# juhotuho10/rust_GPU_raytracing

Hardware: AMD Instinct MI355X
Metric: Mray/s (primary+bounce) at 1920x1080, 8 bounces; 1/2/4/8-GPU scaling (higher is better)
Workload: dtype f32

## Files before the change

rust_gpu_raytracing_amd/csrc/pathtrace.hip:

```cpp
#include <hip/hip_runtime.h>
#include <stdint.h>

#include <algorithm>

#include "rt_launch.h"
#include "rt_path_common.h"
#include "rt_sphere_walk.h"
#include "rt_walk.h"

#ifdef RT_ISA_MARKS
#define RT_ISA_MARK(name) asm volatile("; RT_MARK " name)
#else
#define RT_ISA_MARK(name)
#endif

#pragma clang fp contract(off)

using namespace rtk;

typedef const __attribute__((address_space(4))) unsigned char* KernargPtr;
__device__ __forceinline__ KernargPtr kernarg_fresh(KernargPtr kp) {
    asm volatile("" : "+s"(kp));
    return kp;
}
#define RT_KERNARG(kp, field)                                                                        \
    (*reinterpret_cast<const __attribute__((address_space(4))) decltype(KernelArgs::field)*>(        \
        (kp) + __builtin_offsetof(KernelArgs, field)))
__device__ __forceinline__ ShadeArgs load_shade_args(KernargPtr kp) {
    return ShadeArgs{RT_KERNARG(kp, textures),        RT_KERNARG(kp, env),           RT_KERNARG(kp, texture_width),
                     RT_KERNARG(kp, texture_height),  RT_KERNARG(kp, env_map_width), RT_KERNARG(kp, env_map_height),
                     RT_KERNARG(kp, material_count),  RT_KERNARG(kp, tex_w),         RT_KERNARG(kp, tex_h),
                     RT_KERNARG(kp, tex_layers),      RT_KERNARG(kp, env_w),         RT_KERNARG(kp, env_h),
                     RT_KERNARG(kp, env_uniform),     RT_KERNARG(kp, bounces)};
}

constexpr uint32_t kPrimaryThreads = 1024;


__device__ __forceinline__ uint32_t* sched_orders(const KernelArgs& ka) { return ka.sched + 2u * ka.owned_tiles; }
__device__ __forceinline__ uint32_t* sched_flags(const KernelArgs& ka) { return ka.sched + 4u * ka.owned_tiles; }

__device__ __forceinline__ uint32_t xcc_id() {
    return __builtin_amdgcn_s_getreg((3 << 11) | (0 << 6) | 20);
}

struct TileQueue {
    uint32_t stripe;
    uint32_t empty;
};

__device__ __forceinline__ uint32_t claim_tile(const KernelArgs& ka, TileQueue& q) {
    const uint32_t n_str = ka.queue_stripes;
    const uint32_t lane = threadIdx.x & 63u;
    if (q.empty) return 0xffffffffu;
    uint32_t old = 0;
    if (lane == 0) old = atomicAdd(ka.queue + q.stripe * kQueueStride, 1u);
    uint64_t pos = (uint64_t)__builtin_amdgcn_readlane(old, 0) * n_str + q.stripe;
    if (pos < ka.queue_units) return (uint32_t)pos;
    while (true) {
        bool open = false;
        if (lane < n_str) {
            uint32_t st = q.stripe + 1u + lane;
            st = st >= n_str ? st - n_str : st;
            const uint32_t v = __hip_atomic_load(ka.queue + st * kQueueStride, __ATOMIC_RELAXED, __HIP_MEMORY_SCOPE_AGENT);
            open = (uint64_t)v * n_str + st < ka.queue_units;
        }
        const uint64_t m = __ballot(open);
        if (m == 0) {
            q.empty = 1u;
            return 0xffffffffu;
        }
        uint32_t st = q.stripe + 1u + (uint32_t)__builtin_ctzll(m);
        q.stripe = st >= n_str ? st - n_str : st;
        if (lane == 0) old = atomicAdd(ka.queue + q.stripe * kQueueStride, 1u);
        pos = (uint64_t)__builtin_amdgcn_readlane(old, 0) * n_str + q.stripe;
        if (pos < ka.queue_units) return (uint32_t)pos;
    }
}

template <bool kFramePar>
__device__ __forceinline__ uint32_t unit_tile(const KernelArgs& ka, uint32_t pos, uint32_t& frame) {
    if (pos == 0xffffffffu) return pos;
    uint32_t q;
    if (!kFramePar && !ka.frame_light) {
        frame = 0u;
        q = pos;
    } else if (ka.unit_tile_major) {
        q = pos / ka.frames;
        frame = pos - q * ka.frames;
    } else {
        frame = pos / ka.owned_tiles;
        q = pos - frame * ka.owned_tiles;
    }
    return ka.tile_order ? ka.tile_order[q] : q;
}

__device__ __forceinline__ void record_tile_cost(uint32_t* cost, bool fin, uint32_t tile, uint32_t n) {
    uint64_t m = __ballot(fin);
    while (m) {
        const uint32_t t = __builtin_amdgcn_readlane(tile, (uint32_t)__builtin_ctzll(m));
        const bool mine = fin && tile == t;
        uint32_t v = mine ? n : 0u;
        for (int o = 32; o > 0; o >>= 1) v += __shfl_xor(v, o);
        if ((threadIdx.x & 63u) == 0) atomicAdd(cost + t, v);
        m &= ~__ballot(mine);
    }
}


template <uint32_t kThreads>
__device__ void sort_tiles_by_cost(uint32_t* __restrict__ cost, uint32_t* __restrict__ order, uint32_t n,
                                   uint32_t* scratch) {
    constexpr uint32_t kWaves = kThreads / 64;
    static_assert(kWaves <= 16 && kOrderBuckets * kWaves <= kThreads, "scratch layout / one scan entry per thread");
    uint32_t* slots = scratch;
    uint32_t* max_cost = scratch + kOrderBuckets * 16;
    const uint32_t tid = threadIdx.x, wave = tid >> 6, lane = tid & 63u;
    if (tid == 0) *max_cost = 0;
    __syncthreads();
    uint32_t m = 0;
    for (uint32_t i = tid; i < n; i += kThreads) m = max(m, cost[i]);
    for (int o = 32; o > 0; o >>= 1) m = max(m, (uint32_t)__shfl_xor(m, o));
    if (lane == 0) atomicMax(max_cost, m);
    __syncthreads();
    const uint32_t mx = *max_cost;
    if (mx == 0) {
        for (uint32_t i = tid; i < n; i += kThreads) order[i] = i;
        return;
    }
    const uint64_t mc = (uint64_t)mx + 1u;
    const uint32_t span = ((n + kWaves - 1u) / kWaves + 63u) & ~63u;
    const uint32_t lo = min(n, wave * span), hi = min(n, lo + span);
    auto key = [&](uint32_t i) {
        return i < hi ? kOrderBuckets - 1u - (uint32_t)(((uint64_t)cost[i] * kOrderBuckets) / mc) : kOrderBuckets;
    };
    uint32_t cnt = 0;
    for (uint32_t base = lo; base < hi; base += 64u) {
        const uint32_t k = key(base + lane);
        for (uint32_t b = 0; b < kOrderBuckets; ++b) {
            const uint32_t c = (uint32_t)__popcll(__ballot(k == b));
            if (lane == b) cnt += c;
        }
    }
    if (lane < kOrderBuckets) slots[lane * kWaves + wave] = cnt;
    __syncthreads();
    constexpr uint32_t kEntries = kOrderBuckets * kWaves;
    uint32_t v = tid < kEntries ? slots[tid] : 0u;
    const uint32_t own = v;
    for (uint32_t off = 1; off < kEntries; off <<= 1) {
        __syncthreads();
        const uint32_t add = (tid < kEntries && tid >= off) ? slots[tid - off] : 0u;
        __syncthreads();
        v += add;
        if (tid < kEntries) slots[tid] = v;
    }
    __syncthreads();
    if (tid < kEntries) slots[tid] = v - own;
    __syncthreads();
    uint32_t next = lane < kOrderBuckets ? slots[lane * kWaves + wave] : 0u;
    for (uint32_t base = lo; base < hi; base += 64u) {
        const uint32_t i = base + lane;
        const uint32_t k = key(i);
        uint32_t pos = 0;
        for (uint32_t b = 0; b < kOrderBuckets; ++b) {
            const uint64_t mb = __ballot(k == b);
            const uint32_t first = __builtin_amdgcn_readlane(next, b);
            if (k == b) pos = first + __builtin_amdgcn_mbcnt_hi((uint32_t)(mb >> 32), __builtin_amdgcn_mbcnt_lo((uint32_t)mb, 0u));
            if (lane == b) next += (uint32_t)__popcll(mb);
        }
        if (i < hi) {
            order[pos] = i;
            cost[i] = 0;
        }
    }
}

#ifdef RT_DIAG_TAIL
__device__ __forceinline__ unsigned long long realtime() {
    unsigned long long t;
    asm volatile("s_memrealtime %0\n\ts_waitcnt lgkmcnt(0)" : "=s"(t)::"memory");
    return t;
}
#endif

#ifdef RT_DIAG
__device__ __forceinline__ unsigned long long stamp() {
    unsigned long long t;
    asm volatile("s_memtime %0\n\ts_waitcnt lgkmcnt(0)" : "=s"(t)::"memory");
    return t;
}
struct RootPassCount {
    unsigned long long* diag;
    __device__ __forceinline__ void operator()() const {
        const uint64_t pm = __ballot(true);
        if ((threadIdx.x & 63u) == (uint32_t)__builtin_ctzll(pm)) {
            atomicAdd(diag + 28, 1ull);
            atomicAdd(diag + 29, (unsigned long long)__popcll(pm));
        }
    }
};
struct WalkStepCount {
    unsigned long long* diag;
    __device__ __forceinline__ void operator()(bool walk, bool at_leaf, uint32_t) const {
        const uint64_t act = __ballot(walk), lf = __ballot(at_leaf);
        if (act && (threadIdx.x & 63u) == (uint32_t)__builtin_ctzll(__ballot(true))) {
            atomicAdd(diag + 22, 1ull);
            atomicAdd(diag + 23, (unsigned long long)__popcll(act));
            if (lf) {
                atomicAdd(diag + 24, 1ull);
                atomicAdd(diag + 25, (unsigned long long)__popcll(lf));
            }
        }
    }
};
#endif

template <int kMode, bool kTris>
constexpr bool kLinkedWalk = kBlockLeaves<kTris> && kMode >= 1;

__device__ __forceinline__ uint32_t lds_address(const void* p) {
    return (uint32_t)(uintptr_t)(const __attribute__((address_space(3))) void*)p;
}

template <int kMode, uint32_t kThreads, bool kTris, bool kFramePar>
__global__ void __launch_bounds__(kThreads, 1) rt_pathtrace_kernel(KernelArgs ka) {
    extern __shared__ __attribute__((aligned(16))) unsigned char lds[];
    __shared__ uint32_t block_rays;

    const uint32_t tid = threadIdx.x;
    const KernargPtr kernarg = (KernargPtr)__builtin_amdgcn_kernarg_segment_ptr();
    if (ka.launch_clock && tid == 0) atomicMax(ka.launch_clock, ~(unsigned long long)wall_clock64());
    float* l_srgb = reinterpret_cast<float*>(lds + ka.lds_srgb_offset);
    SceneView sv{ka.sphere_slots, ka.sphere_orig, ka.sphere_material, ka.sphere_bvh, ka.materials, nullptr,
                 ka.objects,      l_srgb,         ka.tri_bvh,     ka.tri_prims, kTris ? *ka.tri_extent : 0.0f,
                 ka.sub_objects};
    if constexpr (kTris && kMode <= 1) {
        if (ka.tri_qnodes) {
            const float4 g0 = ka.tri_qgrid[0], g1 = ka.tri_qgrid[1];
            if (g0.w != 0.0f) {
                sv.tri_q = ka.tri_qnodes;
                sv.qox = g0.x;
                sv.qoy = g0.y;
                sv.qoz = g0.z;
                sv.qsx = g1.x;
                sv.qsy = g1.y;
                sv.qsz = g1.z;
            }
        }
    }
    if (tid == 0) block_rays = 0;
    if constexpr (kMode >= 1) {
        float4* l_sph = reinterpret_cast<float4*>(lds);
        RtMaterial* l_mat = reinterpret_cast<RtMaterial*>(lds + ka.lds_mat_offset);
        RtObject* l_obj = reinterpret_cast<RtObject*>(lds + ka.lds_obj_offset);
        uint32_t* l_orig = reinterpret_cast<uint32_t*>(lds + ka.lds_orig_offset);
        uint32_t* l_smat = reinterpret_cast<uint32_t*>(lds + ka.lds_smat_offset);
        float4* l_nodes = reinterpret_cast<float4*>(lds + ka.lds_nodes_offset);
        for (uint32_t i = tid; i < ka.sphere_slot_count; i += kThreads) {
            l_sph[i] = ka.sphere_slots[i];
            l_orig[i] = ka.sphere_orig[i];
        }
        for (uint32_t i = tid; i < ka.sphere_count; i += kThreads) l_smat[i] = ka.sphere_material[i];
        if constexpr (kLinkedWalk<kMode, kTris>) {
            const uint32_t base = lds_address(l_nodes);
            for (uint32_t i = tid; i < 2u * ka.sphere_nodes; i += kThreads)
                l_nodes[i] = sphere_links_stage(ka.sphere_bvh[i], i, base, ka.sphere_nodes);
            if (tid < 2u) l_nodes[2u * ka.sphere_nodes + tid] = sphere_links_sentinel<float4>(tid, base, ka.sphere_nodes);
        } else {
            for (uint32_t i = tid; i < 2u * ka.sphere_nodes; i += kThreads) l_nodes[i] = ka.sphere_bvh[i];
        }
        float4* l_aux = reinterpret_cast<float4*>(lds + ka.lds_mat_aux_offset);
        for (uint32_t i = tid; i < ka.material_count; i += kThreads) {
            const RtMaterial m = ka.materials[i];
            l_mat[i] = m;
            const float ior_front = 1.0f / m.refraction_index;
            float r0f = (1.0f - ior_front) / (1.0f + ior_front);
            float r0b = (1.0f - m.refraction_index) / (1.0f + m.refraction_index);
            r0f = r0f * r0f;
            r0b = r0b * r0b;
            l_aux[2u * i] = make_float4(ior_front, r0f, r0b, div_const(m.roughness, 10.0f, kInv10));
            const f4 c = decode_texel(ka.textures[min(m.texture_index, ka.tex_layers - 1u)], ka.srgb);
            l_aux[2u * i + 1u] = make_float4(c.x, c.y, c.z, c.w);
        }
        sv.mat_aux = l_aux;
        if (ka.env_uniform & kEnvLineStaged) {
            float4* l_env = reinterpret_cast<float4*>(l_srgb) + kLdsTailBytes / sizeof(float4);
            const uint32_t n = env_line_texels(ka.env_uniform, ka.env_w, ka.env_h);
            const size_t stride = (ka.env_uniform & 2u) ? 1u : ka.env_w;
            for (uint32_t i = tid; i < n; i += kThreads) {
                const f4 c = decode_texel(ka.env[(size_t)i * stride], ka.srgb);
                l_env[i] = make_float4(c.x, c.y, c.z, c.w);
            }
        }
        if constexpr (kTris)
            for (uint32_t i = tid; i < ka.object_count; i += kThreads) l_obj[i] = ka.objects[i];
        sv.sph = l_sph;
        sv.orig = l_orig;
        sv.sph_mat = l_smat;
        sv.nodes = l_nodes;
        sv.mat = l_mat;
        sv.obj = l_obj;
    }
    if constexpr (kMode == 2) {
        float4* l_tn = reinterpret_cast<float4*>(lds + ka.lds_tri_nodes_offset);
        uint4* l_tp = reinterpret_cast<uint4*>(lds + ka.lds_tri_prims_offset);
        for (uint32_t i = tid; i < 2u * ka.tri_nodes; i += kThreads) l_tn[i] = ka.tri_bvh[i];
        for (uint32_t i = tid; i < ka.tri_prim_count; i += kThreads) l_tp[i] = ka.tri_prims[i];
        sv.tri_nodes = l_tn;
        sv.tri_prims = l_tp;
        if (ka.lds_sub_offset) {
            RtSubObject* l_sub = reinterpret_cast<RtSubObject*>(lds + ka.lds_sub_offset);
            for (uint32_t i = tid; i < ka.sub_object_count; i += kThreads) l_sub[i] = ka.sub_objects[i];
            sv.sub = l_sub;
        }
    }
    for (uint32_t i = tid; i < 256u; i += kThreads) l_srgb[i] = ka.srgb[i];
    float* l_cam = l_srgb + 256;
    if (tid < 16u) {
        l_cam[tid] = ka.inv_proj[tid];
        l_cam[16u + tid] = ka.inv_view[tid];
    }
    if (tid == 0) l_cam[32] = ka.aspect;
    __syncthreads();

    const bool accumulate = kFramePar || ka.accumulate == 1u;
    const uint32_t samples = accumulate ? ka.compute_per_frame : 1u;
    constexpr bool kLinked = kLinkedWalk<kMode, kTris>;
    const uint32_t walk_base = kLinked ? lds_address(lds + ka.lds_nodes_offset) : 0u;
    const uint32_t walk_end = kLinked ? sphere_links_addr(walk_base, ka.sphere_nodes) : ka.sphere_nodes;
    const auto walk_over = [&](uint32_t node) { return kLinked ? node == walk_end : node >= walk_end; };

    constexpr uint32_t kIdle = 0, kSetup = 1, kTrav = 2, kDone = 3, kPrimary = 4;
    uint32_t rays = 0;
    uint32_t lane_tile = 0;
    uint32_t lane_slot = 0;
    const bool frame_par = kFramePar || ka.frame_light != nullptr;
    uint32_t mode = kIdle;
    uint32_t index = 0, sample = 0, frame = 0;
    float4 pix = make_float4(0.f, 0.f, 0.f, 0.f);
    Path p;
    p.o = p.d = mk(0.f, 0.f, 0.f);
    p.light = p.contrib = f4{0.f, 0.f, 0.f, 0.f};
    p.seed = p.bounce = 0;
    TraceState ts;
    ts.inv = mk(0.f, 0.f, 0.f);
    ts.a4 = ts.a2 = 0.f;
    ts.node = 0;
    ts.phase = 2;
    ts.nan_hit = false;
    ts.sph = SphereHit{kF32Max, 0u, 0u};
    ts.tri = TriHit{kF32Max, 0u, 0u, 0u, false};

    auto random_index = [&]() { return ka.accumulation_index + (accumulate ? frame : 0u) + sample; };
    auto primary_start = [&]() -> uint32_t {
        return (kTris && ka.primary && p.bounce < ka.bounces) ? kPrimary : kSetup;
    };

    auto store_frame = [&]() {
        float r, g, b, a;
        if (accumulate) {
            const float div = (float)((ka.accumulation_index + frame) * ka.compute_per_frame);
            r = clamp01(pix.x / div);
            g = clamp01(pix.y / div);
            b = clamp01(pix.z / div);
            a = clamp01(pix.w / div);
        } else {
            r = clamp01(p.light.x);
            g = clamp01(p.light.y);
            b = clamp01(p.light.z);
            a = clamp01(p.light.w);
        }
        if (accumulate) ka.accum[index] = pix;
        ka.output[index] = pack_rgba8(r, g, b, a);
    };
    auto finish_sample_frame_par = [&]() {
        const size_t plane = kFramePar ? (size_t)ka.light_plane : (size_t)ka.owned_tiles * 64u;
        const size_t slot = (size_t)(frame * samples + sample) * plane + (size_t)lane_tile * 64u + lane_slot;
        ka.frame_light[slot] = make_float4(p.light.x, p.light.y, p.light.z, p.light.w);
        sample += 1;
        if (sample < samples) {
            start_sample(ka, index, random_index(), pixel_ray(ka, l_cam, index, index % ka.width, index / ka.width), p);
            mode = primary_start();
        } else {
            mode = kIdle;
        }
    };
    auto finish_sample = [&]() {
        if constexpr (kFramePar) {
            finish_sample_frame_par();
        } else {
            if (frame_par) {
                finish_sample_frame_par();
                return;
            }
            sample += 1;
            if (accumulate) {
                pix.x = pix.x + p.light.x;
                pix.y = pix.y + p.light.y;
                pix.z = pix.z + p.light.z;
                pix.w = pix.w + p.light.w;
            }
            if (sample == samples && frame + 1u < ka.frames) {
                store_frame();
                frame += 1;
                sample = 0;
            }
            if (sample < samples) {
                start_sample(ka, index, random_index(), pixel_ray(ka, l_cam, index, index % ka.width, index / ka.width),
                             p);
                mode = primary_start();
            } else {
                store_frame();
                mode = kIdle;
            }
        }
    };

#ifdef RT_DIAG_TAIL
    const unsigned long long wave_t0 = realtime();
    unsigned long long wave_dry = 0;
#endif
    static_assert(kThreads >= kQueueStripesMax, "one thread per stripe counter");
    if (blockIdx.x == 0 && threadIdx.x < kQueueStripesMax) ka.queue_next[threadIdx.x * kQueueStride] = 0u;
    TileQueue queue{(xcc_id() + 8u * (blockIdx.x >> 3)) % ka.queue_stripes, 0u};
    uint32_t tile_frame = 0;
    uint32_t tile = unit_tile<kFramePar>(ka, claim_tile(ka, queue), tile_frame);
    uint32_t next = 0;
#ifdef RT_DIAG
    unsigned long long iters = 0, trav_cyc = 0, steps = 0, step_lanes = 0, shade_cyc = 0, refill_cyc = 0,
                       setup_cyc = 0, leaf_cyc = 0, leaf_steps = 0;
    unsigned long long shade_passes = 0, shade_lanes = 0, miss_lanes = 0, glass_lanes = 0, spec_lanes = 0,
                       setup_passes = 0, setup_lanes = 0;
    const unsigned long long t_start = stamp();
#endif
    while (true) {
#ifdef RT_DIAG
        ++iters;
        const unsigned long long ts0 = stamp();
#endif
        bool fin = false;
        uint32_t fin_rays = 0;
        if (kTris && mode == kPrimary) {
            const uint4 r = ka.primary[(size_t)(frame * samples + sample) * ((size_t)ka.owned_tiles * 64u) +
                                       (size_t)lane_tile * 64u + lane_slot];
            primary_state(PrimaryRecord{__uint_as_float(r.x), r.y, r.z, r.w}, ts);
            mode = kDone;
        }
#ifdef RT_DIAG
        {
            const uint64_t dm = __ballot(mode == kDone);
            if (dm) {
                ++shade_passes;
                shade_lanes += (unsigned long long)__popcll(dm);
            }
        }
#endif
        if (mode == kDone) {
            const Hit h = trace_end<kTris>(sv, ka, p.o, p.d, ts);
#ifdef RT_DIAG
            {
                const bool miss = h.t == kF32Max;
                const RtMaterial dmat = sv.mat[min(h.material_index, ka.material_count - 1u)];
                miss_lanes += (unsigned long long)__popcll(__ballot(miss));
                glass_lanes += (unsigned long long)__popcll(__ballot(!miss && dmat.glass > 0.0f));
                spec_lanes += (unsigned long long)__popcll(__ballot(!miss && !(dmat.glass > 0.0f) && dmat.specular > 0.0f));
            }
#endif
            ++rays;
            RT_ISA_MARK("shade");
            bool ended;
            uint32_t bounce_limit;
            if constexpr (kFramePar) {
                const ShadeArgs sa = load_shade_args(kernarg_fresh(kernarg));
                ended = shade<(kMode >= 1), (kMode >= 1)>(sv, sa, p, h);
                bounce_limit = sa.bounces;
            } else {
                ended = shade<(kMode >= 1), (kMode >= 1)>(sv, ka, p, h);
                bounce_limit = ka.bounces;
            }
            if (ended) {
                fin = true;
                fin_rays = p.bounce + (p.bounce < bounce_limit ? 1u : 0u);
                finish_sample();
            } else {
                mode = kSetup;
            }
        }
        if (ka.tile_cost) record_tile_cost(ka.tile_cost, fin && (!frame_par || frame == 0u), lane_tile, fin_rays);
#ifdef RT_DIAG
        const unsigned long long ts1 = stamp();
        shade_cyc += ts1 - ts0;
#endif
        RT_ISA_MARK("refill");
        while (true) {
            const uint64_t need = __ballot(mode == kIdle);
            if (need == 0 || tile >= ka.owned_tiles) break;
            const uint32_t avail = 64u - next;
            if (mode == kIdle) {
                const uint32_t rank =
                    __builtin_amdgcn_mbcnt_hi((uint32_t)(need >> 32), __builtin_amdgcn_mbcnt_lo((uint32_t)need, 0u));
                if (rank < avail) {
                    const uint32_t slot = next + rank;
                    const uint32_t gt = tile * ka.world_size + ka.rank;
                    const uint32_t x = (gt % ka.tiles_x) * 8u + (slot & 7u);
                    const uint32_t y = (gt / ka.tiles_x) * 8u + (slot >> 3);
                    if (x < ka.width && y < ka.height) {
                        index = y * ka.width + x;
                        lane_tile = tile;
                        lane_slot = slot;
                        sample = 0;
                        frame = tile_frame;
                        mode = kSetup;
                        if (!kFramePar && accumulate && !frame_par) pix = ka.accum[index];
                        start_sample(ka, index, random_index(), pixel_ray(ka, l_cam, index, x, y), p);
                        mode = primary_start();
                    }
                }
            }
            next += min((uint32_t)__popcll(need), avail);
            if (next == 64u) {
                tile = unit_tile<kFramePar>(ka, claim_tile(ka, queue), tile_frame);
                next = 0;
            #ifdef RT_DIAG_TAIL
                if (tile >= ka.owned_tiles && wave_dry == 0) wave_dry = realtime();
#endif
            }
        }
#ifdef RT_DIAG
        const unsigned long long ts2 = stamp();
        refill_cyc += ts2 - ts1;
#endif
#ifdef RT_DIAG
        {
            const uint64_t sm = __ballot(mode == kSetup);
            if (sm) {
                ++setup_passes;
                setup_lanes += (unsigned long long)__popcll(sm);
            }
        }
#endif
        RT_ISA_MARK("setup");
        if (mode == kSetup) {
            if constexpr (!kFramePar)
                while (mode == kSetup && p.bounce >= ka.bounces) finish_sample();
            if (kFramePar || mode == kSetup) {
                trace_begin<kTris>(sv, ka, p.o, p.d, ts);
                if constexpr (kLinkedWalk<kMode, kTris>) ts.node = sphere_links_addr(walk_base, ts.node);
                mode = ts.phase == 2 ? kDone : kTrav;
            }
        }
#ifdef RT_DIAG
        setup_cyc += stamp() - ts2;
#endif
        if (__ballot(mode != kIdle) == 0 && tile >= ka.owned_tiles) break;
        const bool draining = tile >= ka.owned_tiles;
        uint32_t thresh = draining ? 0u : ka.trav_threshold;
        uint32_t n_active = 64u, min_steps = 0u;
        if constexpr (kDrainDecouple<kMode, kTris>) {
            if (draining) {
                thresh = ka.drain_threshold;
                n_active = (uint32_t)__popcll(__ballot(mode == kTrav || mode == kDone));
                min_steps = ka.drain_min_steps;
            }
        }
#ifdef RT_DIAG
        const unsigned long long t0 = stamp();
#endif
        while (true) {
            const uint64_t trav = __ballot(mode == kTrav);
            const uint32_t n_trav = (uint32_t)__popcll(trav);
            if constexpr (kDrainDecouple<kMode, kTris>) {
                if (trav == 0 || (n_trav <= thresh && n_trav < n_active && min_steps == 0)) break;
                min_steps -= min_steps != 0;
            } else {
                if (n_trav <= thresh || trav == 0) break;
            }
#ifdef RT_DIAG
            ++steps;
            step_lanes += (unsigned long long)n_trav;
#endif
            RT_ISA_MARK("traversal");
            bool leaves = false;
            if constexpr (kDeferLeaves<kTris> && !kFusedLeaves<kMode, kTris>) {
                const uint32_t n_pend = (uint32_t)__popcll(__ballot(mode == kTrav && ts.pending != kNoLeaf));
                leaves = 8u * n_pend >= ka.leaf_batch * n_trav;
            }
#ifdef RT_DIAG
            const unsigned long long tl0 = stamp();
#endif
            bool batched = false;
            if constexpr (kCoopLeaves<kMode, kTris>) {
                if (leaves && ka.tri_leaftris) {
                    RT_ISA_MARK("coop_leaf_batch");
                    const bool act = mode == kTrav && ts.pending != kNoLeaf;
                    coop_leaf_batch(sv, ka, p.o, p.d, ts, act, lds);
                    if (act) {
                        phase_end<kTris>(sv, ka, p.o, p.d, ts);
                        if (ts.phase == 2) mode = kDone;
                    }
                    batched = true;
                }
            }
            if constexpr (kBlockLeaves<kTris>) {
                if (mode == kTrav) {
                    RT_ISA_MARK("node_step");
                    RT_ISA_MARK("walk_block");
#ifdef RT_DIAG
                    const WalkStepCount hook{ka.diag};
#else
                    const SphereWalkNoHook hook{};
#endif
                    constexpr int kSteps = kTravUnroll<kMode, kTris>;
                    if constexpr (kLinkedWalk<kMode, kTris>) {
                        if (ka.sphere_boxes_ordered)
                            sphere_links_block<kSteps, true, float4>(lds, walk_end, ts.slab, ts.slack, ts.limit, ts.node,
                                                                     ts.pending, hook);
                        else
                            sphere_links_block<kSteps, false, float4>(lds, walk_end, ts.slab, ts.slack, ts.limit, ts.node,
                                                                      ts.pending, hook);
                    } else {
                        if (ka.sphere_boxes_ordered)
                            sphere_walk_block<kSteps, true>(sv.nodes, ka.sphere_nodes, ts.slab, ts.slack, ts.limit,
                                                            ts.node, ts.pending, hook);
                        else
                            sphere_walk_block<kSteps, false>(sv.nodes, ka.sphere_nodes, ts.slab, ts.slack, ts.limit,
                                                             ts.node, ts.pending, hook);
                    }
                    RT_ISA_MARK("walk_block_end");
                    if (ts.pending == kNoLeaf && walk_over(ts.node)) {
                        ts.phase = 2;
                        mode = kDone;
                    }
                    const uint32_t n_wait = (uint32_t)__popcll(__ballot(ts.pending != kNoLeaf));
                    const uint32_t n_tr = (uint32_t)__popcll(__ballot(true));
#ifdef RT_DIAG
                    if (8u * n_wait >= kBlockLeafShare * n_tr) {
                        const uint64_t gm = __ballot(mode == kTrav && ts.pending != kNoLeaf);
                        if (gm && (threadIdx.x & 63u) == (uint32_t)__builtin_ctzll(gm)) {
                            atomicAdd(ka.diag + 26, 1ull);
                            atomicAdd(ka.diag + 27, (unsigned long long)__popcll(gm));
                        }
                    }
#endif
                    if (8u * n_wait >= kBlockLeafShare * n_tr && mode == kTrav && ts.pending != kNoLeaf) {
                        RT_ISA_MARK("sphere_leaves");
#ifdef RT_DIAG
                        test_sphere_group<false>(sv, ts.pending, p.o, p.d, ts.a4, ts.a2, ts.sph, RootPassCount{ka.diag});
#else
                        test_sphere_group(sv, ts.pending, p.o, p.d, ts.a4, ts.a2, ts.sph);
#endif
                        ts.limit = prune_limit(ts);
                        ts.pending = kNoLeaf;
                        if (walk_over(ts.node)) {
                            ts.phase = 2;
                            mode = kDone;
                        }
                    }
                }
            } else if (!batched && mode == kTrav && (!leaves || ts.pending != kNoLeaf)) {
                if (kDeferLeaves<kTris> && leaves) {
                    RT_ISA_MARK("leaf_batch");
                    leaf_step<kTris, (kMode <= 1)>(sv, ka, p.o, p.d, ts);
                } else {
                    RT_ISA_MARK("node_step");
                    node_step<kTris, kCertWalk<kMode>>(sv, ka, p.o, p.d, ts);
                }
                phase_end<kTris>(sv, ka, p.o, p.d, ts);
                if (ts.phase == 2) mode = kDone;
                if (!(kDeferLeaves<kTris> && leaves)) {
#pragma unroll
                    for (int k = 1; k < kTravUnroll<kMode, kTris>; ++k) {
                        if (mode == kTrav) {
                            node_step<kTris, kCertWalk<kMode>>(sv, ka, p.o, p.d, ts);
                            phase_end<kTris>(sv, ka, p.o, p.d, ts);
                            if (ts.phase == 2) mode = kDone;
                        }
                    }
                }
                if constexpr (kFusedLeaves<kMode, kTris>) {
                    const uint64_t mt = __ballot(mode == kTrav && ts.pending != kNoLeaf && ts.phase == 0);
                    const uint64_t ms = __ballot(mode == kTrav && ts.pending != kNoLeaf && ts.phase != 0);
                    const uint32_t n_p = (uint32_t)__popcll(mt | ms);
                    const uint32_t n_t = (uint32_t)__popcll(__ballot(mode == kTrav));
                    const bool tri_first = __popcll(mt) >= __popcll(ms);
                    if (8u * n_p >= ka.leaf_batch * n_t && mode == kTrav && ts.pending != kNoLeaf &&
                        (ts.phase == 0) == tri_first) {
                        RT_ISA_MARK("leaf_batch");
                        leaf_step<kTris, (kMode <= 1)>(sv, ka, p.o, p.d, ts);
                        phase_end<kTris>(sv, ka, p.o, p.d, ts);
                        if (ts.phase == 2) mode = kDone;
                    }
                }
            }
#ifdef RT_DIAG
            if (leaves) {
                leaf_cyc += stamp() - tl0;
                ++leaf_steps;
            }
#endif
        }
#ifdef RT_DIAG
        trav_cyc += stamp() - t0;
#endif
    }
#ifdef RT_DIAG
    if ((threadIdx.x & 63u) == 0) {
        atomicAdd(ka.diag + 0, stamp() - t_start);
        atomicAdd(ka.diag + 1, trav_cyc);
        atomicAdd(ka.diag + 2, steps);
        atomicAdd(ka.diag + 3, iters);
        atomicAdd(ka.diag + 4, step_lanes);
        atomicAdd(ka.diag + 5, shade_cyc);
        atomicAdd(ka.diag + 6, refill_cyc);
        atomicAdd(ka.diag + 7, setup_cyc);
        atomicAdd(ka.diag + 8, leaf_cyc);
        atomicAdd(ka.diag + 9, leaf_steps);
        atomicAdd(ka.diag + 12, shade_passes);
        atomicAdd(ka.diag + 13, shade_lanes);
        atomicAdd(ka.diag + 14, miss_lanes);
        atomicAdd(ka.diag + 15, glass_lanes);
        atomicAdd(ka.diag + 16, spec_lanes);
        atomicAdd(ka.diag + 17, setup_passes);
        atomicAdd(ka.diag + 18, setup_lanes);
    }
#endif
#ifdef RT_DIAG_TAIL
    if ((threadIdx.x & 63u) == 0) {
        const unsigned long long wave_t1 = realtime();
        atomicAdd(ka.diag + 0, wave_t1);
        atomicMax(ka.diag + 1, wave_t1);
        atomicMax(ka.diag + 2, ~wave_t0);
        atomicAdd(ka.diag + 3, 1ull);
        atomicAdd(ka.diag + 4, wave_t0);
        atomicMax(ka.diag + 5, wave_t0);
        atomicMax(ka.diag + 7, wave_t1 - wave_t0);
        const uint32_t w = blockIdx.x * (kThreads / 64u) + (threadIdx.x >> 6);
        if (w < 65536u) {
            ka.diag[kDiagHeaderWords + 2 * w] = wave_dry ? wave_dry : wave_t1;
            ka.diag[kDiagHeaderWords + 2 * w + 1] = wave_t1;
        }
    }
#endif
    atomicAdd(&block_rays, rays);
    __syncthreads();
    if (tid == 0 && block_rays != 0) atomicAdd(ka.ray_counter, (unsigned long long)block_rays);
    if (ka.sched) {
        const uint32_t par = ka.sched_bits & 1u, n = ka.owned_tiles;
        __shared__ uint32_t sorter;
        if (tid == 0) {
            sorter = atomicAdd(sched_flags(ka) + par, 1u);
            if (blockIdx.x == 0) sched_flags(ka)[par ^ 1u] = 0u;
        }
        __syncthreads();
        if (sorter == 0)
            sort_tiles_by_cost<kThreads>(ka.sched + (par ^ 1u) * n, sched_orders(ka) + (par ^ 1u) * n, n,
                                         reinterpret_cast<uint32_t*>(lds + ka.lds_srgb_offset));
    }
    if (ka.launch_clock) {
        __syncthreads();
        if (tid == 0) atomicMax(ka.launch_clock + 1, (unsigned long long)wall_clock64());
    }
}

#define RT_FOR_EACH_SHAPE(X, FP)                                                                                \
    X(0, 256, true, FP) X(0, 512, true, FP) X(0, 1024, true, FP) X(1, 256, true, FP) X(1, 512, true, FP)       \
    X(1, 1024, true, FP) X(2, 256, true, FP) X(2, 512, true, FP) X(2, 1024, true, FP) X(0, 256, false, FP)     \
    X(0, 512, false, FP) X(0, 1024, false, FP) X(1, 256, false, FP) X(1, 512, false, FP) X(1, 1024, false, FP)
#define RT_FOR_EACH_CONFIG(X) RT_FOR_EACH_SHAPE(X, false) RT_FOR_EACH_SHAPE(X, true)

constexpr uint32_t kBruteThreads = 256;

__device__ __forceinline__ void brute_sub_triangles(const KernelArgs& ka, f3 o, f3 d, uint32_t first_tri,
                                                    uint32_t count, uint32_t oi, float& closest, TriHit& best) {
    for (uint32_t j = 0; j < count; ++j) {
        const uint32_t ti = min(first_tri + j, ka.triangle_count - 1u);
        const TriGeom g = load_tri(ka.triangles, ti);
        const float det = -dot(d, g.cn);
        const float inv_det = 1.0f / det;
        const f3 ao = o - g.a;
        const float dist = dot(ao, g.cn) * inv_det;
        if (dist < 0.0f || dist >= closest) continue;
        const f3 dao = cross(ao, d);
        const float v = -dot(g.ab, dao) * inv_det;
        if (v < 0.0f) continue;
        const float u = dot(g.ac, dao) * inv_det;
        if (u < 0.0f) continue;
        const float w = 1.0f - u - v;
        if (w < 0.0f) continue;
        closest = dist;
        best = TriHit{dist, 0u, ti, oi, det > 0.0f};
    }
}

constexpr uint32_t kBruteGroup = 4;
constexpr uint32_t kBruteWfTileSubs = 512;
constexpr uint32_t kBruteWfLoads = 2u * kBruteWfTileSubs / kBruteThreads;
static_assert(kBruteWfLoads * kBruteThreads == 2u * kBruteWfTileSubs, "tile = whole 16-B loads per thread");
static_assert(kBruteWfLoads == 4u, "the sweep's tile loads are written out for 4 per thread");
constexpr uint32_t kBruteRays = 1;
constexpr uint32_t kBruteChunk = kBruteRays * kBruteThreads;
constexpr uint32_t kBruteHits = 8;
static_assert(kBruteHits >= kBruteGroup, "a group's hits fit a drained list");
constexpr int kBruteWaves = 4, kBruteStreamWaves = 8;

struct BruteSlot {
    uint32_t s, index, x, y;
    bool valid;
};
__device__ __forceinline__ BruteSlot brute_slot(const KernelArgs& ka, const uint32_t* q_in, uint32_t level,
                                                uint32_t qi, uint32_t n_in) {
    BruteSlot r;
    const bool have = qi < n_in;
    r.s = have ? (level == 0u ? qi : q_in[qi]) : 0u;
    const uint32_t local_tile = r.s >> 6, lane_slot = r.s & 63u;
    const uint32_t gt = local_tile * ka.world_size + ka.rank;
    r.x = (gt % ka.tiles_x) * 8u + (lane_slot & 7u);
    r.y = (gt / ka.tiles_x) * 8u + (lane_slot >> 3);
    r.valid = have && local_tile < ka.owned_tiles && r.x < ka.width && r.y < ka.height;
    r.index = r.valid ? r.y * ka.width + r.x : 0u;
    return r;
}

__device__ __forceinline__ void brute_load_path(const float4* pl, uint32_t n_slots, uint32_t s, Path& p) {
    const float4 a = pl[s], b = pl[n_slots + s], l = pl[2u * n_slots + s], k = pl[3u * n_slots + s];
    p.o = mk(a.x, a.y, a.z);
    p.seed = __float_as_uint(a.w);
    p.d = mk(b.x, b.y, b.z);
    p.bounce = __float_as_uint(b.w);
    p.light = f4{l.x, l.y, l.z, l.w};
    p.contrib = f4{k.x, k.y, k.z, k.w};
}
__device__ __forceinline__ void brute_store_path(float4* pl, uint32_t n_slots, uint32_t s, const Path& p) {
    pl[s] = make_float4(p.o.x, p.o.y, p.o.z, __uint_as_float(p.seed));
    pl[n_slots + s] = make_float4(p.d.x, p.d.y, p.d.z, __uint_as_float(p.bounce));
    pl[2u * n_slots + s] = make_float4(p.light.x, p.light.y, p.light.z, p.light.w);
    pl[3u * n_slots + s] = make_float4(p.contrib.x, p.contrib.y, p.contrib.z, p.contrib.w);
}

template <bool kTris, bool kStream>
__global__ void __launch_bounds__(kBruteThreads, kStream ? kBruteStreamWaves : kBruteWaves)
    rt_brute_wf_kernel(KernelArgs ka) {
    extern __shared__ __attribute__((aligned(16))) unsigned char lds[];
    __shared__ uint32_t block_rays;
    const uint32_t tid = threadIdx.x;
    if (ka.launch_clock && tid == 0) atomicMax(ka.launch_clock, ~(unsigned long long)wall_clock64());
    const uint32_t n_slots = ka.owned_tiles * 64u;
    const uint32_t level = ka.brute_level;
    uint32_t* counts = ka.brute_counts + (size_t)ka.brute_pass * ka.brute_levels;
    const uint32_t n_in = level == 0u ? n_slots : counts[level];
    if (blockIdx.x * kBruteChunk >= n_in) {
        if (ka.launch_clock && tid == 0) atomicMax(ka.launch_clock + 1, (unsigned long long)wall_clock64());
        return;
    }
    float* l_cam;
    const SceneView sv = brute_stage<kTris, kBruteThreads>(ka, lds, tid, l_cam);
    uint4* l_tile = reinterpret_cast<uint4*>(lds + ka.lds_stack_offset);
    uint16_t* l_hits = reinterpret_cast<uint16_t*>(l_tile + 4u * kBruteWfTileSubs);
    if (tid == 0) block_rays = 0;
    __syncthreads();

    const bool accumulate = ka.accumulate == 1u;
    const uint32_t samples = accumulate ? ka.compute_per_frame : 1u;
    const uint32_t frame = ka.brute_pass / samples, sample = ka.brute_pass % samples;
    const bool last_pass = ka.brute_pass + 1u == ka.frames * samples;
    const uint32_t random_index = ka.accumulation_index + (accumulate ? frame : 0u) + sample;
    const uint32_t* q_in = ka.brute_queue + (size_t)(level & 1u) * n_slots;
    uint32_t* q_out = ka.brute_queue + (size_t)((level + 1u) & 1u) * n_slots;
    float4* pl = ka.brute_paths;
    uint32_t rays = 0;
    uint64_t streamed = 0;
    uint32_t chunks = 0;
    for (uint32_t c = blockIdx.x; c * kBruteChunk < n_in; c += gridDim.x) {
        ++chunks;
        f3 o[kBruteRays], d[kBruteRays], inv[kBruteRays];
        bool alive[kBruteRays];
        SphereHit sph[kBruteRays];
        TriHit tri[kBruteRays];
        float closest[kBruteRays];
#pragma unroll
        for (uint32_t k = 0; k < kBruteRays; ++k) {
            const BruteSlot bs = brute_slot(ka, q_in, level, c * kBruteChunk + k * kBruteThreads + tid, n_in);
            Path p;
            if (level == 0u) {
                if (bs.valid) {
                    start_sample(ka, bs.index, random_index, pixel_ray(ka, l_cam, bs.index, bs.x, bs.y), p);
                    brute_store_path(pl, n_slots, bs.s, p);
                }
            } else if (bs.valid) {
                brute_load_path(pl, n_slots, bs.s, p);
            }
            alive[k] = bs.valid && p.bounce < ka.bounces;
            o[k] = alive[k] ? p.o : mk(0.f, 0.f, 0.f);
            d[k] = alive[k] ? p.d : mk(0.f, 0.f, 1.f);
            inv[k] = mk(1.0f / d[k].x, 1.0f / d[k].y, 1.0f / d[k].z);
            sph[k] = SphereHit{kF32Max, 0u, 0u};
            tri[k] = TriHit{kF32Max, 0u, 0u, 0u, false};
            closest[k] = kF32Max;
            if (alive[k]) {
                const float a = dot(d[k], d[k]);
                for (uint32_t i = 0; i < ka.sphere_slot_count; i += 4u)
                    test_sphere_group<true>(sv, i, o[k], d[k], 4.0f * a, 2.0f * a, sph[k]);
            }
        }
        if constexpr (kTris && kStream) {
            static_assert(kBruteRays == 1, "the streamed sweep carries one ray per thread");
            uint32_t* l_hits32 = reinterpret_cast<uint32_t*>(l_tile);
            typedef float rt_v4 __attribute__((ext_vector_type(4)));
            typedef __attribute__((address_space(4))) const rt_v4 rt_cf4;
            auto ldc = [](rt_cf4* p_, uint32_t i_) {
                const rt_v4 v_ = p_[i_];
                return make_float4(v_.x, v_.y, v_.z, v_.w);
            };
            for (uint32_t oi = 0; oi < ka.object_count; ++oi) {
                const RtObject& ob = sv.obj[oi];
                const bool in_obj = alive[0] && ray_in_bounds(o[0], inv[0], ob.min_bounds, ob.max_bounds);
                if (__ballot(in_obj) == 0ull) continue;
                const uint32_t first = ob.first_sub_object_index, n_sub = ob.sub_object_count;
                const uint32_t last_sub = ka.sub_object_count - 1u;
                rt_cf4* recs = (rt_cf4*)(const void*)ka.sub_objects;
                if ((tid & 63u) == 0u) streamed += n_sub;
                uint32_t cnt = 0u;
                auto drain = [&]() {
                    for (uint32_t e = 0; __builtin_amdgcn_ballot_w64(e < cnt) != 0ull; ++e) {
                        if (e < cnt) {
                            const uint32_t si = l_hits32[e * kBruteThreads + tid];
                            const float4 lo = reinterpret_cast<const float4*>(ka.sub_objects)[2u * si];
                            const float4 hi = reinterpret_cast<const float4*>(ka.sub_objects)[2u * si + 1u];
                            brute_sub_triangles(ka, o[0], d[0], __float_as_uint(lo.w), __float_as_uint(hi.w), oi,
                                                closest[0], tri[0]);
                        }
                    }
                    cnt = 0u;
                };
                float4 l0, l1, l2, l3, h0, h1, h2, h3;
#define RT_BRUTE_SLOAD(j_)                                                                              \
    {                                                                                                   \
        const uint32_t s0_ = 2u * min(first + (j_), last_sub), s1_ = 2u * min(first + (j_) + 1u, last_sub); \
        const uint32_t s2_ = 2u * min(first + (j_) + 2u, last_sub), s3_ = 2u * min(first + (j_) + 3u, last_sub); \
        n0 = ldc(recs, s0_); m0 = ldc(recs, s0_ + 1u); n1 = ldc(recs, s1_); m1 = ldc(recs, s1_ + 1u);   \
        n2 = ldc(recs, s2_); m2 = ldc(recs, s2_ + 1u); n3 = ldc(recs, s3_); m3 = ldc(recs, s3_ + 1u);   \
    }
                {
                    float4 n0, n1, n2, n3, m0, m1, m2, m3;
                    RT_BRUTE_SLOAD(0u)
                    l0 = n0; l1 = n1; l2 = n2; l3 = n3; h0 = m0; h1 = m1; h2 = m2; h3 = m3;
                }
                uint32_t j0 = 0;
                for (; j0 + 4u <= n_sub; j0 += 4u) {
                    RT_ISA_MARK("brute_box");
                    float4 n0, n1, n2, n3, m0, m1, m2, m3;
                    RT_BRUTE_SLOAD(j0 + 4u)
                    uint32_t bits = 0u;
                    if (in_obj) {
                        bits |= ray_in_box4(o[0], inv[0], l0, h0) ? 1u : 0u;
                        bits |= ray_in_box4(o[0], inv[0], l1, h1) ? 2u : 0u;
                        bits |= ray_in_box4(o[0], inv[0], l2, h2) ? 4u : 0u;
                        bits |= ray_in_box4(o[0], inv[0], l3, h3) ? 8u : 0u;
                    }
                    if (__ballot(bits != 0u) != 0ull) {
                        while (bits) {
                            const uint32_t j = __builtin_ctz(bits);
                            bits &= bits - 1u;
                            l_hits32[cnt * kBruteThreads + tid] = first + j0 + j;
                            cnt += 1u;
                        }
                        if (__ballot(cnt + 4u > kBruteHits) != 0ull) drain();
                    }
                    l0 = n0; l1 = n1; l2 = n2; l3 = n3; h0 = m0; h1 = m1; h2 = m2; h3 = m3;
                }
#undef RT_BRUTE_SLOAD
                for (; j0 < n_sub; ++j0) {
                    const uint32_t si = min(first + j0, last_sub);
                    const float4 lo = ldc(recs, 2u * si), hi = ldc(recs, 2u * si + 1u);
                    if (in_obj && ray_in_box4(o[0], inv[0], lo, hi)) {
                        l_hits32[cnt * kBruteThreads + tid] = si;
                        cnt += 1u;
                    }
                    if (__ballot(cnt + 1u > kBruteHits) != 0ull) drain();
                }
                drain();
            }
        } else if constexpr (kTris) {
            for (uint32_t oi = 0; oi < ka.object_count; ++oi) {
                const RtObject& ob = sv.obj[oi];
                bool in_obj[kBruteRays];
                bool any_in = false;
#pragma unroll
                for (uint32_t k = 0; k < kBruteRays; ++k) {
                    in_obj[k] = alive[k] && ray_in_bounds(o[k], inv[k], ob.min_bounds, ob.max_bounds);
                    any_in |= in_obj[k];
                }
                if (!__syncthreads_or(any_in)) continue;
                const uint32_t first = ob.first_sub_object_index, n_sub = ob.sub_object_count;
                const uint32_t n_tiles = (n_sub + kBruteWfTileSubs - 1u) / kBruteWfTileSubs;
                const uint4* src = reinterpret_cast<const uint4*>(ka.sub_objects);
                const uint32_t last_sub = ka.sub_object_count - 1u;
                uint4 r0, r1, r2, r3;
#define RT_BRUTE_LOAD1(k_, rk)                                                                          \
    {                                                                                                   \
        const uint32_t q_ = tid + (k_) * kBruteThreads;                                                 \
        rk = src[2u * min(first + base_ + (min(q_, 2u * nt_ - 1u) >> 1), last_sub) + (q_ & 1u)];       \
    }
#define RT_BRUTE_LOAD_TILE(t)                                                                           \
    {                                                                                                   \
        const uint32_t base_ = (t) * kBruteWfTileSubs, nt_ = min(kBruteWfTileSubs, n_sub - base_);     \
        RT_BRUTE_LOAD1(0u, r0) RT_BRUTE_LOAD1(1u, r1) RT_BRUTE_LOAD1(2u, r2) RT_BRUTE_LOAD1(3u, r3)     \
    }
#define RT_BRUTE_STORE1(k_, rk)                                                                         \
    {                                                                                                   \
        const uint32_t q_ = tid + (k_) * kBruteThreads;                                                 \
        if (q_ < 2u * nt_) dst_[q_] = rk;                                                               \
    }
#define RT_BRUTE_STORE_TILE(t)                                                                          \
    {                                                                                                   \
        uint4* dst_ = l_tile + (size_t)((t) & 1u) * 2u * kBruteWfTileSubs;                             \
        const uint32_t nt_ = min(kBruteWfTileSubs, n_sub - (t) * kBruteWfTileSubs);                     \
        RT_BRUTE_STORE1(0u, r0) RT_BRUTE_STORE1(1u, r1) RT_BRUTE_STORE1(2u, r2) RT_BRUTE_STORE1(3u, r3) \
    }
                if (n_tiles) {
                    RT_BRUTE_LOAD_TILE(0u)
                    RT_BRUTE_STORE_TILE(0u)
                }
                for (uint32_t t = 0; t < n_tiles; ++t) {
                    __syncthreads();
                    const uint32_t nt = min(kBruteWfTileSubs, n_sub - t * kBruteWfTileSubs);
                    if (tid == 0) streamed += nt;
                    const bool more = t + 1u < n_tiles;
                    if (more) RT_BRUTE_LOAD_TILE(t + 1u)
                    if (any_in) {
                        const float4* tile = reinterpret_cast<const float4*>(l_tile + (size_t)(t & 1u) * 2u * kBruteWfTileSubs);
                        uint32_t cnt[kBruteRays];
#pragma unroll
                        for (uint32_t k = 0; k < kBruteRays; ++k) cnt[k] = 0u;
                        auto drain = [&]() {
#pragma unroll
                            for (uint32_t k = 0; k < kBruteRays; ++k) {
                                for (uint32_t e = 0; __builtin_amdgcn_ballot_w64(e < cnt[k]) != 0ull; ++e) {
                                    if (e < cnt[k]) {
                                        const uint32_t j = l_hits[(k * kBruteHits + e) * kBruteThreads + tid];
                                        const float4 lo = tile[2u * j], hi = tile[2u * j + 1u];
                                        brute_sub_triangles(ka, o[k], d[k], __float_as_uint(lo.w), __float_as_uint(hi.w),
                                                            oi, closest[k], tri[k]);
                                    }
                                }
                                cnt[k] = 0u;
                            }
                        };
                        uint32_t j0 = 0;
                        for (; j0 + kBruteGroup <= nt; j0 += kBruteGroup) {
                            RT_ISA_MARK("brute_box");
                            uint32_t bits[kBruteRays];
                            uint32_t any = 0u;
#pragma unroll
                            for (uint32_t k = 0; k < kBruteRays; ++k) bits[k] = 0u;
#pragma unroll
                            for (uint32_t j = 0; j < kBruteGroup; ++j) {
                                const float4 lo = tile[2u * (j0 + j)], hi = tile[2u * (j0 + j) + 1u];
#pragma unroll
                                for (uint32_t k = 0; k < kBruteRays; ++k)
                                    bits[k] |= (in_obj[k] & ray_in_box4(o[k], inv[k], lo, hi)) ? 1u << j : 0u;
                            }
#pragma unroll
                            for (uint32_t k = 0; k < kBruteRays; ++k) any |= bits[k];
                            if (any) {
                                bool full = false;
#pragma unroll
                                for (uint32_t k = 0; k < kBruteRays; ++k) {
                                    while (bits[k]) {
                                        const uint32_t j = __builtin_ctz(bits[k]);
                                        bits[k] &= bits[k] - 1u;
                                        l_hits[(k * kBruteHits + cnt[k]) * kBruteThreads + tid] = (uint16_t)(j0 + j);
                                        cnt[k] += 1u;
                                    }
                                    full |= cnt[k] + kBruteGroup > kBruteHits;
                                }
                                if (__builtin_amdgcn_ballot_w64(full) != 0ull) drain();
                            }
                        }
                        for (; j0 < nt; ++j0) {
                            const float4 lo = tile[2u * j0], hi = tile[2u * j0 + 1u];
#pragma unroll
                            for (uint32_t k = 0; k < kBruteRays; ++k) {
                                if (in_obj[k] && ray_in_box4(o[k], inv[k], lo, hi)) {
                                    l_hits[(k * kBruteHits + cnt[k]) * kBruteThreads + tid] = (uint16_t)j0;
                                    cnt[k] += 1u;
                                }
                            }
                            bool full = false;
#pragma unroll
                            for (uint32_t k = 0; k < kBruteRays; ++k) full |= cnt[k] + 1u > kBruteHits;
                            if (__builtin_amdgcn_ballot_w64(full) != 0ull) drain();
                        }
                        drain();
                    }
                    if (more) RT_BRUTE_STORE_TILE(t + 1u)
                }
#undef RT_BRUTE_LOAD1
#undef RT_BRUTE_LOAD_TILE
#undef RT_BRUTE_STORE1
#undef RT_BRUTE_STORE_TILE
            }
        }
#pragma unroll
        for (uint32_t k = 0; k < kBruteRays; ++k) {
            const BruteSlot bs = brute_slot(ka, q_in, level, c * kBruteChunk + k * kBruteThreads + tid, n_in);
            Path p;
            if (bs.valid) brute_load_path(pl, n_slots, bs.s, p);
            bool done = bs.valid && !alive[k];
            if (alive[k]) {
                ++rays;
                TraceState ts;
                ts.sph = sph[k];
                ts.tri = tri[k];
                const Hit h = trace_end<kTris>(sv, ka, o[k], d[k], ts);
                done = shade<true>(sv, ka, p, h);
            }
            const bool cont = alive[k] && !done;
            if (cont) brute_store_path(pl, n_slots, bs.s, p);
            const uint64_t m = __ballot(cont);
            if (m) {
                const uint32_t lane = __builtin_amdgcn_mbcnt_hi((uint32_t)(m >> 32), __builtin_amdgcn_mbcnt_lo((uint32_t)m, 0u));
                uint32_t base = 0u;
                if ((tid & 63u) == (uint32_t)__builtin_ctzll(m)) base = atomicAdd(counts + level + 1u, (uint32_t)__popcll(m));
                base = __builtin_amdgcn_readlane(base, (uint32_t)__builtin_ctzll(m));
                if (cont) q_out[base + lane] = bs.s;
            }
            if (done) {
                float r, g, b, al;
                if (accumulate) {
                    float4 pix = ka.accum[bs.index];
                    pix.x = pix.x + p.light.x;
                    pix.y = pix.y + p.light.y;
                    pix.z = pix.z + p.light.z;
                    pix.w = pix.w + p.light.w;
                    ka.accum[bs.index] = pix;
                    const float div = (float)((ka.accumulation_index + ka.frames - 1u) * ka.compute_per_frame);
                    r = clamp01(pix.x / div);
                    g = clamp01(pix.y / div);
                    b = clamp01(pix.z / div);
                    al = clamp01(pix.w / div);
                } else {
                    r = clamp01(p.light.x);
                    g = clamp01(p.light.y);
                    b = clamp01(p.light.z);
                    al = clamp01(p.light.w);
                }
                if (last_pass) ka.output[bs.index] = pack_rgba8(r, g, b, al);
            }
        }
    }
    atomicAdd(&block_rays, rays);
    __syncthreads();
    if (tid == 0 && block_rays) atomicAdd(ka.ray_counter, (unsigned long long)block_rays);
    if (tid == 0 && ka.stream_bytes && kTris && chunks) {
        uint64_t n_sub = 0;
        for (uint32_t oi = 0; oi < ka.object_count; ++oi) n_sub += sv.obj[oi].sub_object_count;
        atomicAdd(ka.stream_bytes, (unsigned long long)(chunks * n_sub * 32ull));
    }
    if (streamed && ka.l2_stream_bytes) atomicAdd(ka.l2_stream_bytes, (unsigned long long)streamed * 32ull);
    if (ka.launch_clock) {
        __syncthreads();
        if (tid == 0) atomicMax(ka.launch_clock + 1, (unsigned long long)wall_clock64());
    }
}

template <int kMode, bool kTris, uint32_t kThreads, uint32_t kMinWaves>
__global__ void __launch_bounds__(kThreads, kMinWaves) rt_primary_kernel(KernelArgs ka) {
    extern __shared__ __attribute__((aligned(16))) unsigned char lds[];
    const uint32_t tid = threadIdx.x;
    if (ka.launch_clock && tid == 0) atomicMax(ka.launch_clock, ~(unsigned long long)wall_clock64());
    float* l_srgb = reinterpret_cast<float*>(lds + ka.lds_srgb_offset);
    float* l_cam = l_srgb + 256;
    SceneView sv{ka.sphere_slots, ka.sphere_orig, ka.sphere_material, ka.sphere_bvh, ka.materials, nullptr,
                 ka.objects,      l_srgb,         ka.tri_bvh,     ka.tri_prims, kTris ? *ka.tri_extent : 0.0f,
                 ka.sub_objects};
    if constexpr (kMode >= 1) {
        float4* l_sph = reinterpret_cast<float4*>(lds);
        RtObject* l_obj = reinterpret_cast<RtObject*>(lds + ka.lds_obj_offset);
        uint32_t* l_orig = reinterpret_cast<uint32_t*>(lds + ka.lds_orig_offset);
        float4* l_nodes = reinterpret_cast<float4*>(lds + ka.lds_nodes_offset);
        for (uint32_t i = tid; i < ka.sphere_slot_count; i += kThreads) {
            l_sph[i] = ka.sphere_slots[i];
            l_orig[i] = ka.sphere_orig[i];
        }
        for (uint32_t i = tid; i < 2u * ka.sphere_nodes; i += kThreads) l_nodes[i] = ka.sphere_bvh[i];
        if constexpr (kTris)
            for (uint32_t i = tid; i < ka.object_count; i += kThreads) l_obj[i] = ka.objects[i];
        sv.sph = l_sph;
        sv.orig = l_orig;
        sv.nodes = l_nodes;
        sv.obj = l_obj;
    }
    if constexpr (kMode == 2) {
        float4* l_tn = reinterpret_cast<float4*>(lds + ka.lds_tri_nodes_offset);
        uint4* l_tp = reinterpret_cast<uint4*>(lds + ka.lds_tri_prims_offset);
        for (uint32_t i = tid; i < 2u * ka.tri_nodes; i += kThreads) l_tn[i] = ka.tri_bvh[i];
        for (uint32_t i = tid; i < ka.tri_prim_count; i += kThreads) l_tp[i] = ka.tri_prims[i];
        sv.tri_nodes = l_tn;
        sv.tri_prims = l_tp;
        if (ka.lds_sub_offset) {
            RtSubObject* l_sub = reinterpret_cast<RtSubObject*>(lds + ka.lds_sub_offset);
            for (uint32_t i = tid; i < ka.sub_object_count; i += kThreads) l_sub[i] = ka.sub_objects[i];
            sv.sub = l_sub;
        }
    }
    if (tid < 16u) {
        l_cam[tid] = ka.inv_proj[tid];
        l_cam[16u + tid] = ka.inv_view[tid];
    }
    if (tid == 0) l_cam[32] = ka.aspect;
    __syncthreads();

    const uint32_t unit = __builtin_amdgcn_readfirstlane(blockIdx.x * (kThreads / 64u) + (tid >> 6));
    if (unit >= ka.queue_units) return;
    const uint32_t n_frames = ka.queue_units / ka.owned_tiles;
    const uint32_t frame = ka.primary_tile_major ? unit % n_frames : unit / ka.owned_tiles;
    const uint32_t local_tile = ka.primary_tile_major ? unit / n_frames : unit - frame * ka.owned_tiles;
    const uint32_t slot = tid & 63u;
    const uint32_t gt = local_tile * ka.world_size + ka.rank;
    const uint32_t x = (gt % ka.tiles_x) * 8u + (slot & 7u);
    const uint32_t y = (gt / ka.tiles_x) * 8u + (slot >> 3);
    const bool valid = x < ka.width && y < ka.height;
    const uint32_t index = valid ? y * ka.width + x : 0u;
    const bool accumulate = ka.accumulate == 1u;
    const uint32_t samples = accumulate ? ka.compute_per_frame : 1u;
    const size_t owned_px = (size_t)ka.owned_tiles * 64u;
    const f3 cam = pixel_ray(ka, l_cam, index, x, y);
    for (uint32_t sample = 0; sample < samples; ++sample) {
        Path p;
        start_sample(ka, index, ka.accumulation_index + (accumulate ? frame : 0u) + sample, cam, p);
        const f3 o = p.o, d = p.d;
        TraceState ts;
        trace_begin<kTris>(sv, ka, o, d, ts);
        if constexpr (kTris) {
            if (ts.phase == 0) {
                uint32_t node = __builtin_amdgcn_readfirstlane(ts.node);
                while (node < ka.tri_nodes) {
                    const float4 lo = sv.tri_nodes[2u * node], hi = sv.tri_nodes[2u * node + 1u];
                    float near_t, far_t;
                    slab_hit(ts.slab, lo.x, lo.y, lo.z, hi.x, hi.y, hi.z, near_t, far_t);
                    bool hit = valid && near_t <= far_t && far_t >= 0.0f && near_t <= ts.limit;
                    const uint32_t leaf = __float_as_uint(hi.w);
                    uint32_t skip = 0u;
                    if (kCertWalk<kMode> && hit && leaf != 0xffffffffu && ka.tri_leafcert && near_t > ts.tri.t &&
                        ts.tri.t != kF32Max) {
                        skip = tri_leaf_skips(ka, leaf & 0xffffffu, ts.slab, o, d, ts.tri.t, lo, hi);
                        if (skip == kLeafCertAll) hit = false;
                    }
                    const bool any = __ballot(hit) != 0;
                    if (any && leaf != 0xffffffffu && hit) {
                        tri_leaf<(kMode <= 1)>(sv, ka, o, d, ts, leaf & 0xffffffu);
                        ts.limit = tri_limit(sv, ka, o, ts);
                    }
                    node = (any && leaf == 0xffffffffu) ? node + 1u : __float_as_uint(lo.w);
                }
                if (ts.nan_hit) ts.tri = sweep_triangles(sv, ka, o, d);
                ts.phase = ka.sphere_nodes != 0 ? 1u : 2u;
                ts.node = 0;
                if (ts.phase == 1) phase_setup<kTris>(sv, ka, o, ts.a2 * 0.5f, 1, ts);
            }
        }
        if (ts.phase == 1) {
            const uint32_t n0 = ka.sphere_octant_stride ? ka.sphere_octant_stride : ka.sphere_nodes;
            SlabRay sr = slab_ray(o.x, o.y, o.z, ts.inv.x, ts.inv.y, ts.inv.z, 0.0f);
            {
                const float r = sqrt_up(dot(o, o));
                float m, slack;
                sphere_cull_bounds(r, ka.sphere_extent, ka.sphere_rmin, ka.sphere_rmax,
                                   __builtin_amdgcn_rsqf(ts.a2 * 0.5f), m, slack);
                sr = slab_ray(o.x, o.y, o.z, ts.inv.x, ts.inv.y, ts.inv.z, m);
                ts.slack = slack;
                ts.limit = prune_limit(ts);
            }
            uint32_t node = 0;
            while (node < n0) {
                const float4 lo = sv.nodes[2u * node], hi = sv.nodes[2u * node + 1u];
                float near_t, far_t;
                slab_hit(sr, lo.x, lo.y, lo.z, hi.x, hi.y, hi.z, near_t, far_t);
                const bool hit = valid && near_t <= far_t && far_t >= -ts.slack && near_t <= ts.limit;
                const bool any = __ballot(hit) != 0;
                const uint32_t leaf = __float_as_uint(hi.w);
                if (any && leaf != 0xffffffffu && hit) {
                    test_sphere_group(sv, leaf & 0xffffffu, o, d, ts.a4, ts.a2, ts.sph);
                    ts.limit = prune_limit(ts);
                }
                node = (any && leaf == 0xffffffffu) ? node + 1u : __float_as_uint(lo.w);
            }
        }
        if (valid)
            reinterpret_cast<uint4*>(ka.primary)[(size_t)(frame * samples + sample) * owned_px +
                                                 (size_t)local_tile * 64u + slot] = [&] {
                const PrimaryRecord r = primary_record<kTris>(ts);
                return make_uint4(__float_as_uint(r.t), r.id, r.meta, r.orig);
            }();
    }
}

namespace {
hipError_t allow_big_lds(const void* fn) {
    int dev = 0, max_optin = 0;
    hipError_t e = hipGetDevice(&dev);
    if (e != hipSuccess) return e;
    e = hipDeviceGetAttribute(&max_optin, hipDeviceAttributeSharedMemPerBlockOptin, dev);
    if (e != hipSuccess || max_optin <= 0) return hipSuccess;
    return hipFuncSetAttribute(fn, hipFuncAttributeMaxDynamicSharedMemorySize, max_optin - 256);
}
}

hipError_t rt_launch_pathtrace(const KernelArgs& ka, int mode, bool tris, bool frame_par, uint32_t threads,
                               size_t lds_bytes, uint32_t blocks, hipStream_t stream) {
    if (frame_par && (!ka.frame_light || ka.accumulate != 1u || ka.bounces == 0)) return hipErrorInvalidValue;
#define RT_LAUNCH(M, T, TR, FP)                                                                                \
    if (mode == M && threads == T && tris == TR && frame_par == FP) {                                         \
        hipLaunchKernelGGL((rt_pathtrace_kernel<M, T, TR, FP>), dim3(blocks), dim3(T), lds_bytes, stream, ka); \
        return hipGetLastError();                                                                             \
    }
    RT_FOR_EACH_CONFIG(RT_LAUNCH)
#undef RT_LAUNCH
    return hipErrorInvalidValue;
}

size_t rt_brute_wf_tile_bytes(bool stream) {
    if (stream) return (size_t)kBruteThreads * kBruteHits * 4u;
    return 2u * (size_t)kBruteWfTileSubs * sizeof(RtSubObject) + (size_t)kBruteThreads * kBruteRays * kBruteHits * 2u;
}

uint32_t rt_brute_wf_chunk() { return kBruteChunk; }

hipError_t rt_launch_brute_wf(const KernelArgs& ka, bool tris, bool scalar_stream, size_t lds_bytes, uint32_t blocks,
                              hipStream_t stream) {
    if (blocks == 0) return hipSuccess;
    const void* fn = tris ? (scalar_stream ? reinterpret_cast<const void*>(&rt_brute_wf_kernel<true, true>)
                                           : reinterpret_cast<const void*>(&rt_brute_wf_kernel<true, false>))
                          : reinterpret_cast<const void*>(&rt_brute_wf_kernel<false, false>);
    if (lds_bytes > 64u * 1024u) {
        hipError_t e = hipFuncSetAttribute(fn, hipFuncAttributeMaxDynamicSharedMemorySize, (int)lds_bytes);
        if (e != hipSuccess) return hipErrorInvalidConfiguration;
    }
    if (tris && scalar_stream)
        hipLaunchKernelGGL((rt_brute_wf_kernel<true, true>), dim3(blocks), dim3(kBruteThreads), lds_bytes, stream, ka);
    else if (tris)
        hipLaunchKernelGGL((rt_brute_wf_kernel<true, false>), dim3(blocks), dim3(kBruteThreads), lds_bytes, stream, ka);
    else
        hipLaunchKernelGGL((rt_brute_wf_kernel<false, false>), dim3(blocks), dim3(kBruteThreads), lds_bytes, stream, ka);
    return hipGetLastError();
}

hipError_t rt_launch_primary(const KernelArgs& ka, int mode, bool tris, size_t lds_bytes, uint32_t threads,
                             uint32_t min_waves, hipStream_t stream) {
    if (threads == 0) threads = kPrimaryThreads;
    const uint32_t per = threads / 64u;
    const uint32_t blocks = (ka.queue_units + per - 1u) / per;
    if (blocks == 0) return hipSuccess;
#define RT_PRIMARY(M, TR, T, W)                                                                                \
    if (mode == M && tris == TR && threads == T && min_waves == W) {                                           \
        if (lds_bytes > 64u * 1024u) {                                                                         \
            hipError_t e = allow_big_lds(reinterpret_cast<const void*>(&rt_primary_kernel<M, TR, T, W>));     \
            if (e != hipSuccess) return e;                                                                     \
        }                                                                                                      \
        hipLaunchKernelGGL((rt_primary_kernel<M, TR, T, W>), dim3(blocks), dim3(T), lds_bytes, stream, ka);   \
        return hipGetLastError();                                                                              \
    }
    RT_PRIMARY(1, true, 64, 0) RT_PRIMARY(1, true, 128, 0) RT_PRIMARY(1, true, 256, 0) RT_PRIMARY(1, true, 256, 8)
    RT_PRIMARY(1, true, 512, 0) RT_PRIMARY(1, true, 1024, 0) RT_PRIMARY(2, true, 1024, 0)
#undef RT_PRIMARY
    return hipErrorInvalidValue;
}

constexpr int kDefaultWavesPerCu = 16;

hipError_t rt_pathtrace_pick_config(int mode, bool tris, bool frame_par, size_t lds_bytes,
                                    size_t lds_bytes_per_thread, uint32_t force_threads, uint32_t waves_cap,
                                    uint32_t* threads, int* blocks_per_cu) {
    const int kTargetWavesPerCu = waves_cap ? (int)waves_cap : kDefaultWavesPerCu;
    int best_waves = -1;
#define RT_OCC(M, T, TR, FP)                                                                              \
    if (mode == M && tris == TR && frame_par == FP) {                                                     \
        int n = 0;                                                                                        \
        hipError_t e = allow_big_lds(reinterpret_cast<const void*>(&rt_pathtrace_kernel<M, T, TR, FP>)); \
        if (e != hipSuccess) return e;                                                                    \
        e = hipOccupancyMaxActiveBlocksPerMultiprocessor(&n, rt_pathtrace_kernel<M, T, TR, FP>, T,       \
                                                         lds_bytes + (size_t)T * lds_bytes_per_thread);  \
        if (e != hipSuccess) return e;                                                                    \
        const int waves = std::min(n * (int)(T / 64), kTargetWavesPerCu);                                 \
        if (n > 0 && (force_threads ? force_threads == T : waves > best_waves)) {                         \
            best_waves = waves;                                                                           \
            *threads = T;                                                                                 \
            *blocks_per_cu = force_threads ? n : std::max(1, std::min(n, kTargetWavesPerCu / (int)(T / 64))); \
        }                                                                                                 \
    }
    RT_FOR_EACH_CONFIG(RT_OCC)
#undef RT_OCC
    if (best_waves <= 0) return hipErrorInvalidConfiguration;
    return hipSuccess;
}

extern "C" __global__ void __launch_bounds__(256) rt_pack_tiles_kernel(const float4* __restrict__ accum,
                                                                      float4* __restrict__ dst, uint32_t width,
                                                                      uint32_t height, uint32_t tiles_x,
                                                                      uint32_t owned_tiles, uint32_t rank,
                                                                      uint32_t world) {
    const uint64_t gid = (uint64_t)blockIdx.x * blockDim.x + threadIdx.x;
    const uint64_t local_tile = gid >> 6;
    if (local_tile >= owned_tiles) return;
    const uint32_t lane = (uint32_t)(gid & 63u);
    const uint32_t tile = (uint32_t)local_tile * world + rank;
    const uint32_t x = (tile % tiles_x) * 8u + (lane & 7u);
    const uint32_t y = (tile / tiles_x) * 8u + (lane >> 3);
    float4 v = make_float4(0.f, 0.f, 0.f, 0.f);
    if (x < width && y < height) v = accum[(size_t)y * width + x];
    dst[gid] = v;
}

__device__ __forceinline__ uint32_t owned_tiles_of(uint32_t n_tiles, uint32_t rank, uint32_t world) {
    return rank < n_tiles ? (n_tiles - rank + world - 1u) / world : 0u;
}

extern "C" __global__ void __launch_bounds__(256) rt_unpack_tiles_kernel(
    const float4* __restrict__ src, float4* __restrict__ accum, uint32_t* __restrict__ output, uint32_t width,
    uint32_t height, uint32_t tiles_x, uint32_t n_tiles, uint32_t first_rank, uint32_t world, uint64_t stride_px,
    uint32_t skip_rank, float divisor) {
    const uint32_t rank = first_rank + blockIdx.y;
    if (rank == skip_rank) return;
    src += (uint64_t)blockIdx.y * stride_px;
    const uint64_t gid = (uint64_t)blockIdx.x * blockDim.x + threadIdx.x;
    const uint64_t local_tile = gid >> 6;
    if (local_tile >= owned_tiles_of(n_tiles, rank, world)) return;
    const uint32_t lane = (uint32_t)(gid & 63u);
    const uint32_t tile = (uint32_t)local_tile * world + rank;
    const uint32_t x = (tile % tiles_x) * 8u + (lane & 7u);
    const uint32_t y = (tile / tiles_x) * 8u + (lane >> 3);
    if (x >= width || y >= height) return;
    const float4 v = src[gid];
    const size_t idx = (size_t)y * width + x;
    accum[idx] = v;
    output[idx] = pack_rgba8(clamp01(v.x / divisor), clamp01(v.y / divisor), clamp01(v.z / divisor),
                             clamp01(v.w / divisor));
}

typedef float StreamF4 __attribute__((ext_vector_type(4)));
__device__ __forceinline__ float4 ld_stream(const float4* p) {
    const StreamF4 v = __builtin_nontemporal_load(reinterpret_cast<const StreamF4*>(p));
    return make_float4(v.x, v.y, v.z, v.w);
}

__device__ __forceinline__ void resolve_pixel(float4* __restrict__ accum, uint32_t* __restrict__ output,
                                              const float4* __restrict__ light, uint32_t width, uint32_t height,
                                              uint32_t tiles_x, uint32_t owned_tiles, uint32_t rank, uint32_t world,
                                              uint32_t k0, uint32_t samples, uint32_t frames) {
    const uint64_t gid = (uint64_t)blockIdx.x * blockDim.x + threadIdx.x;
    const uint64_t owned_px = (uint64_t)owned_tiles * 64u;
    if (gid >= owned_px) return;
    const uint32_t lane = (uint32_t)(gid & 63u);
    const uint32_t tile = (uint32_t)(gid >> 6) * world + rank;
    const uint32_t x = (tile % tiles_x) * 8u + (lane & 7u);
    const uint32_t y = (tile / tiles_x) * 8u + (lane >> 3);
    if (x >= width || y >= height) return;
    const size_t idx = (size_t)y * width + x;
    float4 pix = accum[idx];
    const uint32_t n = frames * samples;
    constexpr uint32_t kGroup = 8;
    const float4* src = light + gid;
    uint32_t i = 0;
    for (; i + kGroup <= n; i += kGroup) {
        float4 l[kGroup];
#pragma unroll
        for (uint32_t k = 0; k < kGroup; k++) l[k] = ld_stream(src + (size_t)(i + k) * owned_px);
#pragma unroll
        for (uint32_t k = 0; k < kGroup; k++) {
            pix.x = pix.x + l[k].x;
            pix.y = pix.y + l[k].y;
            pix.z = pix.z + l[k].z;
            pix.w = pix.w + l[k].w;
        }
    }
    for (; i < n; i++) {
        const float4 l = ld_stream(src + (size_t)i * owned_px);
        pix.x = pix.x + l.x;
        pix.y = pix.y + l.y;
        pix.z = pix.z + l.z;
        pix.w = pix.w + l.w;
    }
    accum[idx] = pix;
    const float div = (float)((k0 + frames - 1u) * samples);
    output[idx] = pack_rgba8(clamp01(pix.x / div), clamp01(pix.y / div), clamp01(pix.z / div), clamp01(pix.w / div));
}

extern "C" __global__ void __launch_bounds__(256) rt_resolve_frames_kernel(
    float4* __restrict__ accum, uint32_t* __restrict__ output, const float4* __restrict__ light, uint32_t width,
    uint32_t height, uint32_t tiles_x, uint32_t owned_tiles, uint32_t rank, uint32_t world, uint32_t k0,
    uint32_t samples, uint32_t frames, unsigned long long* __restrict__ clock) {
    constexpr uint32_t kResolveStampBlocks = 64;
    const bool first = blockIdx.x < kResolveStampBlocks;
    const bool last = blockIdx.x + kResolveStampBlocks >= gridDim.x;
    if (clock && first && threadIdx.x == 0) atomicMax(clock, ~(unsigned long long)wall_clock64());
    resolve_pixel(accum, output, light, width, height, tiles_x, owned_tiles, rank, world, k0, samples, frames);
    if (clock && last) {
        __syncthreads();
        if (threadIdx.x == 0) atomicMax(clock + 1, (unsigned long long)wall_clock64());
    }
}

hipError_t rt_launch_resolve(float4* accum, uint32_t* output, const float4* light, uint32_t width, uint32_t height,
                             uint32_t tiles_x, uint32_t owned_tiles, uint32_t rank, uint32_t world, uint32_t k0,
                             uint32_t samples, uint32_t frames, unsigned long long* clock, hipStream_t stream) {
    const uint64_t threads = (uint64_t)owned_tiles * 64u;
    const uint32_t blocks = (uint32_t)((threads + 255u) / 256u);
    hipLaunchKernelGGL(rt_resolve_frames_kernel, dim3(blocks), dim3(256), 0, stream, accum, output, light, width,
                       height, tiles_x, owned_tiles, rank, world, k0, samples, frames, clock);
    return hipGetLastError();
}

extern "C" __global__ void __launch_bounds__(256) rt_pack_output_kernel(
    const uint32_t* __restrict__ output, uint32_t* __restrict__ dst, uint32_t width, uint32_t height,
    uint32_t tiles_x, uint32_t n_tiles, uint32_t first_rank, uint32_t world, uint64_t stride_px, uint32_t skip_rank,
    uint32_t unpack) {
    const uint32_t rank = first_rank + blockIdx.y;
    if (rank == skip_rank) return;
    dst += (uint64_t)blockIdx.y * stride_px;
    const uint64_t gid = (uint64_t)blockIdx.x * blockDim.x + threadIdx.x;
    const uint64_t local_tile = gid >> 6;
    if (local_tile >= owned_tiles_of(n_tiles, rank, world)) return;
    const uint32_t lane = (uint32_t)(gid & 63u);
    const uint32_t tile = (uint32_t)local_tile * world + rank;
    const uint32_t x = (tile % tiles_x) * 8u + (lane & 7u);
    const uint32_t y = (tile / tiles_x) * 8u + (lane >> 3);
    const bool inside = x < width && y < height;
    const size_t idx = (size_t)y * width + x;
    uint32_t* out = const_cast<uint32_t*>(output);
    if (unpack) {
        if (inside) out[idx] = dst[gid];
    } else {
        dst[gid] = inside ? output[idx] : 0u;
    }
}

static uint32_t owned_tiles_host(uint32_t n_tiles, uint32_t rank, uint32_t world) {
    return rank < n_tiles ? (n_tiles - rank + world - 1u) / world : 0u;
}

hipError_t rt_launch_pack_output(uint32_t* output, uint32_t* packed, uint32_t width, uint32_t height, uint32_t tiles_x,
                                 uint32_t n_tiles, uint32_t first_rank, uint32_t ranks, uint32_t world,
                                 uint64_t stride_px, uint32_t skip_rank, bool unpack, hipStream_t stream) {
    const uint64_t threads = (uint64_t)owned_tiles_host(n_tiles, first_rank, world) * 64u;
    const uint32_t blocks = (uint32_t)((threads + 255u) / 256u);
    if (blocks == 0 || ranks == 0) return hipSuccess;
    hipLaunchKernelGGL(rt_pack_output_kernel, dim3(blocks, ranks), dim3(256), 0, stream, output, packed, width, height,
                       tiles_x, n_tiles, first_rank, world, stride_px, skip_rank, unpack ? 1u : 0u);
    return hipGetLastError();
}

hipError_t rt_launch_pack(const float4* accum, float4* dst, uint32_t width, uint32_t height, uint32_t tiles_x,
                          uint32_t owned_tiles, uint32_t rank, uint32_t world, hipStream_t stream) {
    const uint64_t threads = (uint64_t)owned_tiles * 64u;
    const uint32_t blocks = (uint32_t)((threads + 255u) / 256u);
    hipLaunchKernelGGL(rt_pack_tiles_kernel, dim3(blocks), dim3(256), 0, stream, accum, dst, width, height, tiles_x,
                       owned_tiles, rank, world);
    return hipGetLastError();
}

hipError_t rt_launch_unpack(const float4* src, float4* accum, uint32_t* output, uint32_t width, uint32_t height,
                            uint32_t tiles_x, uint32_t n_tiles, uint32_t first_rank, uint32_t ranks, uint32_t world,
                            uint64_t stride_px, uint32_t skip_rank, float divisor, hipStream_t stream) {
    const uint64_t threads = (uint64_t)owned_tiles_host(n_tiles, first_rank, world) * 64u;
    const uint32_t blocks = (uint32_t)((threads + 255u) / 256u);
    if (blocks == 0 || ranks == 0) return hipSuccess;
    hipLaunchKernelGGL(rt_unpack_tiles_kernel, dim3(blocks, ranks), dim3(256), 0, stream, src, accum, output, width,
                       height, tiles_x, n_tiles, first_rank, world, stride_px, skip_rank, divisor);
    return hipGetLastError();
}

extern "C" __global__ void __launch_bounds__(256) rt_math_selftest_kernel(uint32_t which,
                                                                         unsigned long long* mismatches,
                                                                         uint32_t* first_bad) {
    unsigned long long bad = 0;
    const uint64_t stride = (uint64_t)gridDim.x * blockDim.x;
    for (uint64_t i = (uint64_t)blockIdx.x * blockDim.x + threadIdx.x; i < (1ull << 32); i += stride) {
        const uint32_t bits = (uint32_t)i;
        const float x = __uint_as_float(bits);
        float got, want;
        if (which == 0) {
            const float ax = __builtin_fabsf(x);
            if (ax != 0.0f && ax < 0x1p-96f) continue;
            got = sqrt_rn_nrm(x);
            want = __builtin_sqrtf(x);
        } else if (which == 1) {
            got = div_const(x, kTwoPiWgsl, kInvTwoPiWgsl);
            want = x / kTwoPiWgsl;
        } else if (which == 2) {
            got = div_const(x, kWgslPi, kInvWgslPi);
            want = x / kWgslPi;
        } else if (which == 3) {
            got = div_const(x, 255.0f, kInv255);
            want = x / 255.0f;
        } else if (which == 4) {
            got = div_const(x, 10.0f, kInv10);
            want = x / 10.0f;
        } else {
            const float u = (float)bits / 4294967296.0f;
            if (which == 5) {
                got = logf_u01(u);
                want = logf_c(u);
            } else {
                const float theta = kBoxMullerTwoPi * u;
                got = cosf_box(theta);
                want = cosf_c(theta);
            }
        }
        const bool same = __float_as_uint(got) == __float_as_uint(want) || (got != got && want != want);
        if (!same) {
            ++bad;
            atomicMin(first_bad, bits);
        }
    }
    if (bad) atomicAdd(mismatches, bad);
}

hipError_t rt_launch_math_selftest(uint32_t which, unsigned long long* mismatches, uint32_t* first_bad,
                                   hipStream_t stream) {
    hipLaunchKernelGGL(rt_math_selftest_kernel, dim3(8192), dim3(256), 0, stream, which, mismatches, first_bad);
    return hipGetLastError();
}
```

rust_gpu_raytracing_amd/csrc/rt_frames.cpp:

```cpp
#include <algorithm>

#include "rt_ctx.h"
#include "rt_launch.h"

namespace {

constexpr size_t kLdsSceneBudget = 64 * 1024;
constexpr size_t kLdsAccelBudget = 150 * 1024;
constexpr float kTriPruneRho = 1.0f / 64.0f;
uint32_t trav_threshold_for(int lds_mode, bool tris, bool certified) {
    if (!tris) return 12;
    return lds_mode == 2 ? 24 : certified ? 56 : 48;
}
uint32_t leaf_batch_for(int lds_mode, bool certified) { return lds_mode == 2 ? 6 : certified ? 4 : 5; }
constexpr uint64_t kSchedMinTilesPerWave = 4;
constexpr uint32_t kMaxFrameBatch = 64;
constexpr uint32_t kMaxParallelLights = 64;

}


void rth::scene_base_args(rt_ctx* ctx, KernelArgs& ka) {
    const rt_params& p = ctx->params;
    ka.sphere_slots = ctx->d_slot_sph;
    ka.sphere_orig = ctx->d_slot_orig;
    ka.sphere_material = ctx->d_sph_mat;
    ka.sphere_bvh = reinterpret_cast<const float4*>(ctx->d_bvh);
    ka.sphere_always = ctx->n_always;
    ka.sphere_nodes = ctx->n_nodes;
    ka.sphere_extent = ctx->sphere_extent;
    ka.sphere_rmin = ctx->sphere_rmin;
    ka.sphere_rmax = ctx->sphere_rmax;
    ka.tri_accel = (ctx->use_tri_bvh && p.object_count != 0) ? 1u : 0u;
    ka.tri_nodes = ka.tri_accel ? ctx->tri_nodes : 0u;
    ka.tri_prim_count = ka.tri_accel ? ctx->tri_prim_count : 0u;
    ka.tri_extent = ctx->d_tri_extent;
    ka.tri_bvh = reinterpret_cast<const float4*>(ctx->d_tri_bvh);
    ka.tri_prims = reinterpret_cast<const uint4*>(ctx->d_tri_prims);
    ka.materials = ctx->d_mat;
    ka.objects = ctx->d_obj;
    ka.sub_objects = ctx->d_sub;
    ka.triangles = ctx->d_tri;
    ka.textures = ctx->d_tex;
    ka.env = ctx->d_env;
    ka.srgb = ctx->d_srgb;
    ka.camera_origin[0] = ctx->camera.origin[0];
    ka.camera_origin[1] = ctx->camera.origin[1];
    ka.camera_origin[2] = ctx->camera.origin[2];
    ka.width = ctx->width;
    ka.accumulation_index = p.accumulation_index;
    ka.accumulate = p.accumulate;
    ka.sphere_count = p.sphere_count;
    ka.sphere_slot_count = ctx->n_slots;
    ka.object_count = p.object_count;
    ka.compute_per_frame = p.compute_per_frame;
    ka.texture_width = p.texture_width;
    ka.texture_height = p.texture_height;
    ka.env_map_width = p.env_map_width;
    ka.env_map_height = p.env_map_height;
    ka.material_count = ctx->n_mat_dev;
    ka.sub_object_count = ctx->n_sub_dev;
    ka.triangle_count = ctx->n_tri_dev;
    ka.tex_w = ctx->tex_w;
    ka.tex_h = ctx->tex_h;
    ka.tex_layers = ctx->tex_layers;
    ka.env_w = ctx->env_w;
    ka.env_h = ctx->env_h;
    ka.env_uniform = ctx->env_uniform;
    ka.height = ctx->height;
    ka.gen_rays = ctx->gen_rays ? 1u : 0u;
    ka.aspect = (float)ctx->width / (float)ctx->height;
    std::memcpy(ka.inv_proj, ctx->inv_proj, sizeof(ka.inv_proj));
    std::memcpy(ka.inv_view, ctx->inv_view, sizeof(ka.inv_view));
}

static int scene_carve_layouts(rt_ctx* ctx, KernelArgs& ka, uint32_t layouts, size_t mode1_budget, int max_mode,
                               SceneLaunch& sl) {
    const rt_params& p = ctx->params;
    size_t off = al16((size_t)ctx->n_slots * 16);
    ka.lds_mat_offset = (uint32_t)off;
    off = al16(off + (size_t)ctx->n_mat_dev * sizeof(RtMaterial));
    ka.lds_mat_aux_offset = (uint32_t)off;
    off = al16(off + (size_t)ctx->n_mat_dev * 32);
    ka.lds_obj_offset = (uint32_t)off;
    off = al16(off + (size_t)p.object_count * sizeof(RtObject));
    ka.lds_orig_offset = (uint32_t)off;
    off = al16(off + (size_t)ctx->n_slots * 4);
    ka.lds_smat_offset = (uint32_t)off;
    off = al16(off + (size_t)p.sphere_count * 4);
    ka.lds_nodes_offset = (uint32_t)off;
    off = al16(off + (size_t)layouts * ctx->n_nodes * sizeof(SphereBvhNode));
    if (p.object_count == 0) off += sizeof(SphereBvhNode);
    sl.mode1_bytes = off + kLdsTailBytes;
    ka.lds_tri_nodes_offset = (uint32_t)off;
    off = al16(off + (size_t)ka.tri_nodes * sizeof(SphereBvhNode));
    ka.lds_tri_prims_offset = (uint32_t)off;
    off = al16(off + (size_t)ka.tri_prim_count * sizeof(SubObjectPrim));
    ka.lds_sub_offset = 0;
    if (ctx->stage_subs && ka.sub_object_count != 0) {
        const size_t with = al16(off + (size_t)ka.sub_object_count * sizeof(RtSubObject));
        if (with + kLdsTailBytes <= kLdsAccelBudget) {
            ka.lds_sub_offset = (uint32_t)off;
            off = with;
        }
    }
    sl.mode2_bytes = off + kLdsTailBytes;
    if (ka.tri_accel && ka.tri_nodes != 0 && sl.mode2_bytes <= kLdsAccelBudget && max_mode >= 2)
        return 2;
    if (sl.mode1_bytes <= mode1_budget && max_mode >= 1) return 1;
    return 0;
}

void rth::scene_carve(rt_ctx* ctx, KernelArgs& ka, int max_mode, SceneLaunch& sl) {
    sl.tris = ctx->params.object_count != 0;
    sl.mode = scene_carve_layouts(ctx, ka, 1, kLdsSceneBudget, max_mode, sl);
    sl.layouts = 1;
    if (ctx->sphere_octants && ctx->n_nodes != 0) {
        if (scene_carve_layouts(ctx, ka, 8, kLdsAccelBudget, max_mode, sl) == sl.mode)
            sl.layouts = 8;
        else
            scene_carve_layouts(ctx, ka, 1, kLdsSceneBudget, max_mode, sl);
    }
}

int rth::scene_accel_args(rt_ctx* ctx, KernelArgs& ka, SceneLaunch& sl) {
    ka.sphere_nodes = sl.layouts * ctx->n_nodes;
    ka.sphere_octant_stride = sl.layouts == 8 ? ctx->n_nodes : 0u;
    ka.sphere_boxes_ordered = (sl.layouts == 8 && ctx->sphere_boxes_ordered && !sl.tris) ? 1u : 0u;
    const bool certified = sl.tris && sl.mode <= 1 && ka.tri_accel && ctx->tri_prune_mode == 1;
    ka.trav_threshold = ctx->trav_threshold ? ctx->trav_threshold : trav_threshold_for(sl.mode, sl.tris, certified);
    ka.leaf_batch = ctx->leaf_batch ? ctx->leaf_batch : leaf_batch_for(sl.mode, certified);
    ka.tri_qnodes = nullptr;
    ka.tri_qgrid = nullptr;
    ka.tri_octant_stride = 0;
    const bool global_walk = sl.tris && sl.mode <= 1 && ka.tri_accel && ka.tri_nodes != 0;
    const bool octants = global_walk && ctx->tri_octants_built;
    const bool qnodes = global_walk && ctx->use_qnodes;
    int rc;
    if (octants || qnodes) {
        const uint32_t n_out = octants ? 8u * ka.tri_nodes : ka.tri_nodes;
        if (qnodes && (rc = grow_buffer(ctx, "quantized triangle nodes", &ctx->d_tri_qnodes, &ctx->qnodes_cap,
                                        (size_t)n_out * sizeof(uint4), &ctx->qnodes_dirty)))
            return rc;
        if (!ctx->d_tri_qgrid) RT_HIP(ctx, hipMalloc(reinterpret_cast<void**>(&ctx->d_tri_qgrid), 2 * sizeof(float4)));
        if (ctx->qnodes_dirty || ctx->derived_octants != octants || ctx->derived_qnodes != qnodes) {
            RT_HIP(ctx, rt_launch_quantize_tri_nodes(reinterpret_cast<const SphereBvhNode*>(ctx->d_tri_bvh),
                                                     ka.tri_nodes, octants ? ctx->d_tri_src8 : nullptr,
                                                     octants ? ctx->d_tri_skip8 : nullptr, n_out,
                                                     octants ? ctx->d_tri_bvh8 : nullptr,
                                                     qnodes ? ctx->d_tri_qnodes : nullptr, ctx->d_tri_qgrid,
                                                     ctx->stream));
            ctx->qnodes_dirty = false;
            ctx->derived_octants = octants;
            ctx->derived_qnodes = qnodes;
            ctx->primary_dirty = true;
        }
        if (qnodes) {
            ka.tri_qnodes = ctx->d_tri_qnodes;
            ka.tri_qgrid = ctx->d_tri_qgrid;
        }
        if (octants) {
            ka.tri_bvh = reinterpret_cast<const float4*>(ctx->d_tri_bvh8);
            ka.tri_octant_stride = ka.tri_nodes;
            ka.tri_nodes = n_out;
        }
    }
    ka.tri_prune_mode = (sl.tris && ka.tri_accel && ka.tri_nodes != 0) ? (uint32_t)ctx->tri_prune_mode : 0u;
    ka.tri_prune = ka.tri_prune_mode == 2u ? kTriPruneRho : 0.0f;
    ka.tri_leafcert = nullptr;
    if (ka.tri_prune_mode == 1u && ka.tri_prim_count != 0 && sl.mode <= 1) {
        if ((rc = grow_buffer(ctx, "leaf certificates", &ctx->d_tri_lcert, &ctx->tri_lcert_cap,
                              (size_t)ka.tri_prim_count * sizeof(TriLeafCert), &ctx->cones_dirty)))
            return rc;
        if (ctx->cones_dirty) {
            RT_HIP(ctx, rt_launch_tri_leafcert(ctx->d_tri_prims, ka.tri_prim_count, ctx->d_sub, ctx->d_tri,
                                               ctx->n_tri_dev, ctx->d_tri_lcert, ctx->stream));
            ctx->cones_dirty = false;
            ctx->primary_dirty = true;
        }
        ka.tri_leafcert = ctx->d_tri_lcert;
    }
    ka.tri_leaftris = nullptr;
    sl.coop = sl.tris && sl.mode <= 1 && ka.tri_accel && ka.tri_nodes != 0 && ka.tri_prim_count != 0 &&
                      ctx->use_coop_leaves;
    if (sl.coop) {
        if ((rc = grow_buffer(ctx, "leaf triangle blocks", &ctx->d_tri_ltris, &ctx->tri_ltris_cap,
                              (size_t)ka.tri_prim_count * kLeafTriWords * sizeof(uint4), &ctx->ltris_dirty)))
            return rc;
        if (ctx->ltris_dirty) {
            RT_HIP(ctx, rt_launch_tri_leaftris(ctx->d_tri_prims, ka.tri_prim_count, ctx->d_tri, ctx->n_tri_dev,
                                               ctx->d_tri_ltris, ctx->stream));
            ctx->ltris_dirty = false;
            ctx->primary_dirty = true;
        }
        ka.tri_leaftris = ctx->d_tri_ltris;
    }
    if (sl.mode == 2) {
        ka.lds_srgb_offset = (uint32_t)(sl.mode2_bytes - kLdsTailBytes);
        sl.lds_bytes = sl.mode2_bytes;
    } else if (sl.mode == 1) {
        ka.lds_srgb_offset = (uint32_t)(sl.mode1_bytes - kLdsTailBytes);
        sl.lds_bytes = sl.mode1_bytes;
    } else {
        ka.lds_srgb_offset = 0;
        sl.lds_bytes = kLdsTailBytes;
    }
    return RT_OK;
}

static bool rt_path_frame_par_instance(bool frame_par_batch, uint32_t accumulate, uint32_t bounces, bool enabled) {
    return enabled && frame_par_batch && accumulate == 1u && bounces >= 1u;
}


struct BatchLaunch {
    uint32_t bounces = 0, frames = 0;
    uint64_t owned_px = 0;
    bool frame_par = false;
    bool fp_instance = false;
    SceneLaunch sl;
    const rt_ctx::OccEntry* occ = nullptr;
    size_t lds_bytes = 0;
    uint32_t blocks = 0;
    bool sched = false;
    int si = 0;
    hipStream_t S = nullptr;
    bool primary = false;
};

static void batch_base_args(rt_ctx* ctx, const BatchLaunch& b, KernelArgs& ka) {
    ka.camera_rays = ctx->d_rays;
    ka.accum = ctx->d_accum;
    ka.output = ctx->d_out;
    ka.ray_counter = ctx->d_counter;
    ka.diag = ctx->d_counter + 1;
    ka.queue_stripes = ctx->queue_stripes;
    scene_base_args(ctx, ka);
    ka.bounces = b.bounces;
    ka.tiles_x = ctx->tiles_x;
    ka.owned_tiles = ctx->owned_tiles;
    ka.rank = ctx->rank;
    ka.world_size = ctx->world;
    ka.drain_threshold = ctx->drain_threshold;
    ka.drain_min_steps = ctx->drain_min_steps;
    ka.frames = b.frames;
}

static int plan_batch(rt_ctx* ctx, BatchLaunch& b, KernelArgs& ka) {
    const rt_params& p = ctx->params;
    b.owned_px = (uint64_t)ctx->owned_tiles * 64u;
    b.frame_par = b.frames > 1 && p.accumulate == 1u && ctx->frame_parallel &&
                  (uint64_t)b.frames * p.compute_per_frame <= kMaxParallelLights && p.compute_per_frame > 0;
    ka.frame_light = nullptr;
    ka.queue_units = ctx->owned_tiles;
    if (b.frame_par) {
        const size_t need = (size_t)b.owned_px * b.frames * p.compute_per_frame;
        if (need * sizeof(float4) > ctx->frame_light_cap) {
            const size_t want = std::max<size_t>(
                need, std::min<size_t>(ctx->batch_budget / (2 * sizeof(float4)),
                                       (size_t)b.owned_px * std::min<uint64_t>((uint64_t)ctx->frame_batch *
                                                                                   p.compute_per_frame,
                                                                               kMaxParallelLights)));
            const int rc = grow_buffer(ctx, "frame lights", ctx->d_frame_light, &ctx->frame_light_cap,
                                       want * sizeof(float4), nullptr, 2);
            if (rc) return rc;
        }
        ka.queue_units = ctx->owned_tiles * b.frames;
        ka.unit_tile_major = ctx->unit_tile_major ? 1u : 0u;
        ka.light_plane = (uint32_t)b.owned_px;
    }
    b.fp_instance = rt_path_frame_par_instance(b.frame_par, p.accumulate, b.bounces, ctx->frame_par_instance);
    return RT_OK;
}

static int launch_brute(rt_ctx* ctx, BatchLaunch& b, KernelArgs& ka) {
    SceneLaunch& sl = b.sl;
    scene_carve_layouts(ctx, ka, 1, kLdsSceneBudget, ctx->force_global_scene ? 0 : ctx->max_lds_mode, sl);
    ka.lds_srgb_offset = (uint32_t)(sl.mode1_bytes - kLdsTailBytes);
    ka.lds_stack_offset = (uint32_t)al16(sl.mode1_bytes);
    const uint32_t samples = ka.accumulate == 1u ? ka.compute_per_frame : 1u;
    const uint64_t passes = (uint64_t)b.frames * samples;
    const bool scalar_stream = sl.tris && ctx->brute == 2;
    const size_t lds = ka.lds_stack_offset + rt_brute_wf_tile_bytes(scalar_stream);
    int dev = 0, max_optin = 0;
    RT_HIP(ctx, hipGetDevice(&dev));
    RT_HIP(ctx, hipDeviceGetAttribute(&max_optin, hipDeviceAttributeSharedMemPerBlockOptin, dev));
    if (lds > (size_t)max_optin - 256)
        return fail(ctx, RT_E_CAPACITY, "brute-force mode: spheres, materials and objects must fit in LDS");
    ka.sphere_octant_stride = 0;
    ka.sphere_boxes_ordered = 0;
    ka.stream_bytes = ctx->d_stream;
    ka.l2_stream_bytes = ctx->d_stream + 1;
    ka.frame_light = nullptr;
    RT_HIP(ctx, join_aux(ctx));
    int rc = claim_clock_slot(ctx, ctx->stream, ka);
    if (rc) return rc;
    const size_t n_slots = (size_t)ctx->owned_tiles * 64u;
    ka.brute_levels = std::max(1u, b.bounces) + 1u;
    const size_t n_counts = (size_t)passes * ka.brute_levels;
    if ((rc = grow_buffer(ctx, "brute-force paths", &ctx->d_brute_paths, &ctx->brute_paths_cap,
                          4 * n_slots * sizeof(float4))) ||
        (rc = grow_buffer(ctx, "brute-force queue", &ctx->d_brute_queue, &ctx->brute_queue_cap,
                          2 * n_slots * sizeof(uint32_t))) ||
        (rc = grow_buffer(ctx, "brute-force counters", &ctx->d_brute_counts, &ctx->brute_counts_cap,
                          n_counts * sizeof(uint32_t))))
        return rc;
    RT_HIP(ctx, hipMemsetAsync(ctx->d_brute_counts, 0, n_counts * sizeof(uint32_t), ctx->stream));
    ka.brute_paths = ctx->d_brute_paths;
    ka.brute_queue = ctx->d_brute_queue;
    ka.brute_counts = ctx->d_brute_counts;
    const uint32_t chunks = (uint32_t)((n_slots + rt_brute_wf_chunk() - 1u) / rt_brute_wf_chunk());
    const uint32_t blocks = std::min<uint32_t>(chunks, 16u * (uint32_t)std::max<int>(1, (int)ctx->n_cu));
    for (uint64_t pass = 0; pass < passes; ++pass)
        for (uint32_t level = 0; level < std::max(1u, b.bounces); ++level) {
            ka.brute_pass = (uint32_t)pass;
            ka.brute_level = level;
            RT_HIP(ctx, rt_launch_brute_wf(ka, sl.tris, scalar_stream, lds, blocks, ctx->stream));
        }
    ctx->last_blocks = blocks;
    ctx->last_passes = RT_PASS_BRUTE | (scalar_stream ? RT_PASS_BRUTE_STREAM : 0u);
    ctx->last_lds = (uint32_t)lds;
    ctx->last_threads = 256;
    ctx->primary_dirty = true;
    return RT_OK;
}

static int path_occupancy(rt_ctx* ctx, BatchLaunch& b, KernelArgs& ka) {
    const SceneLaunch& sl = b.sl;
    const size_t lane_pt = sl.coop ? (size_t)kLeafBatchWaveBytes / 64u : 0u;
    size_t line_bytes = 0;
    if (sl.mode >= 1) {
        const uint32_t n = env_line_texels(ka.env_uniform, ka.env_w, ka.env_h);
        if (n != 0 && n <= kEnvLineMax) line_bytes = (size_t)n * sizeof(float4);
    }
    const rt_ctx::OccKey key{sl.lds_bytes, lane_pt, line_bytes, sl.mode, sl.tris ? 1u : 0u, ctx->force_threads,
                             ctx->waves_cap};
    rt_ctx::OccEntry& oc = ctx->occ_cache[b.fp_instance ? 1 : 0];
    if (oc.blocks_per_cu == 0 || !same_key(oc.key, key)) {
        int per_cu = 0;
        uint32_t threads = 0;
        hipError_t oe = rt_pathtrace_pick_config(sl.mode, sl.tris, b.fp_instance, sl.lds_bytes, lane_pt,
                                                 ctx->force_threads, ctx->waves_cap, &threads, &per_cu);
        if (oe != hipSuccess) return hip_fail(ctx, "rt_pathtrace_pick_config (occupancy query)", oe);
        oc.env_line = false;
        if (line_bytes != 0) {
            int per_cu_line = 0;
            uint32_t threads_line = 0;
            oe = rt_pathtrace_pick_config(sl.mode, sl.tris, b.fp_instance, sl.lds_bytes + line_bytes, lane_pt,
                                          ctx->force_threads, ctx->waves_cap, &threads_line, &per_cu_line);
            if (oe != hipSuccess) (void)hipGetLastError();
            oc.env_line = oe == hipSuccess && threads_line == threads && per_cu_line == per_cu;
        }
        oc.key = key;
        oc.blocks_per_cu = per_cu;
        oc.threads = threads;
    }
    b.occ = &oc;
    ctx->last_threads = oc.threads;
    ctx->last_mode = sl.mode;
    b.lds_bytes = sl.lds_bytes;
    if (oc.env_line) {
        ka.env_uniform |= kEnvLineStaged;
        b.lds_bytes += line_bytes;
    }
    ka.lds_leafbatch_offset = (uint32_t)al16(b.lds_bytes);
    if (sl.coop) b.lds_bytes = ka.lds_leafbatch_offset + (size_t)oc.threads * lane_pt;
    const uint32_t waves_per_block = oc.threads / 64;
    const uint64_t resident = (uint64_t)oc.blocks_per_cu * (uint64_t)(ctx->n_cu > 0 ? ctx->n_cu : 1);
    const uint64_t wanted = ((uint64_t)ka.queue_units + waves_per_block - 1) / waves_per_block;
    b.blocks = (uint32_t)(wanted < resident ? wanted : resident);
    return RT_OK;
}

static int select_stream(rt_ctx* ctx, BatchLaunch& b, KernelArgs& ka) {
    b.si = (b.frame_par && ctx->batch_overlap) ? (int)(ctx->batches & 1u) : 0;
    b.S = b.si ? ctx->aux_stream : ctx->stream;
    if (!b.frame_par) RT_HIP(ctx, join_aux(ctx));
    if (b.si && ctx->primary_dirty) {
        RT_HIP(ctx, follow_primary(ctx, b.S));
        ctx->primary_dirty = false;
    }
    const uint32_t parity = ctx->queue_parity[b.si];
    ka.queue = ctx->d_queue + (size_t)(2 * b.si + parity) * kQueueStripesMax * kQueueStride;
    ka.queue_next = ctx->d_queue + (size_t)(2 * b.si + (parity ^ 1u)) * kQueueStripesMax * kQueueStride;
    if (b.frame_par) ka.frame_light = ctx->d_frame_light[ctx->batches & 1u];
    return RT_OK;
}

static int schedule_state(rt_ctx* ctx, BatchLaunch& b, KernelArgs& ka) {
    const uint32_t waves_per_block = b.occ->threads / 64;
    b.sched = ctx->tile_schedule && (!b.frame_par || ctx->batch_schedule) &&
              (uint64_t)ka.queue_units >= kSchedMinTilesPerWave * b.blocks * waves_per_block;
    if (!b.sched) return RT_OK;
    const size_t n = ctx->owned_tiles;
    uint32_t*& state = ctx->d_tile_sched[b.si];
    if (!state) {
        int rc = dev_alloc(ctx, &state, 4 * n + 2);
        if (rc) return rc;
        RT_HIP(ctx, hipMemsetAsync(state, 0, (4 * n + 2) * 4, ctx->stream));
        ctx->primary_dirty = true;
        RT_HIP(ctx, follow_primary(ctx, b.S));
        ctx->sched_launches[b.si] = 0;
    }
    ka.sched = state;
    ka.sched_bits = (uint32_t)(ctx->sched_launches[b.si] & 1u);
    ka.tile_cost = ka.sched + ka.sched_bits * (size_t)n;
    ka.tile_order = ctx->sched_launches[b.si] ? ka.sched + (2u + ka.sched_bits) * (size_t)n : nullptr;
    return RT_OK;
}

static int primary_prepass(rt_ctx* ctx, BatchLaunch& b, KernelArgs& ka) {
    const rt_params& p = ctx->params;
    const SceneLaunch& sl = b.sl;
    const size_t need =
        (size_t)b.owned_px * b.frames * std::max<uint32_t>(1u, p.accumulate == 1u ? p.compute_per_frame : 1u);
    b.primary = b.bounces > 0 && sl.mode >= 1 && sl.tris && ka.compute_per_frame > 0 &&
                (ctx->primary_pass == 1 || (ctx->primary_pass == -1 && sl.mode == 1)) &&
                2 * need * sizeof(uint4) <= ctx->batch_budget;
    ka.primary = nullptr;
    if (!b.primary) return RT_OK;
    if (need * sizeof(uint4) > ctx->primary_cap) {
        const size_t want = std::max<size_t>(
            need, std::min<size_t>(ctx->batch_budget / (2 * sizeof(uint4)), (size_t)b.owned_px * ctx->frame_batch));
        const int rc = grow_buffer(ctx, "primary records", ctx->d_primary, &ctx->primary_cap, want * sizeof(uint4),
                                   nullptr, 2);
        if (rc) return rc;
    }
    KernelArgs pka = ka;
    pka.primary = ctx->d_primary[ctx->batches & 1u];
    pka.queue_units = ctx->owned_tiles * b.frames;
    pka.primary_tile_major = ctx->primary_tile_major ? 1u : 0u;
    const size_t image = sl.mode == 2 ? sl.mode2_bytes : sl.mode1_bytes;
    const uint32_t min_waves = (sl.mode == 2 || ctx->primary_threads != 256u) ? 0u : ctx->primary_min_waves;
    RT_HIP(ctx, rt_launch_primary(pka, sl.mode, sl.tris, image, sl.mode == 2 ? 1024u : ctx->primary_threads, min_waves,
                                  b.S));
    ka.primary = pka.primary;
    return RT_OK;
}

static int launch_path_and_resolve(rt_ctx* ctx, const BatchLaunch& b, const KernelArgs& ka) {
    const rt_params& p = ctx->params;
    hipError_t e = rt_launch_pathtrace(ka, b.sl.mode, b.sl.tris, b.fp_instance, b.occ->threads, b.lds_bytes, b.blocks,
                                       b.S);
    ctx->last_blocks = b.blocks;
    ctx->last_passes = RT_PASS_PATH | (b.primary ? RT_PASS_PRIMARY : 0u) | (b.frame_par ? RT_PASS_RESOLVE : 0u) |
                       (b.fp_instance ? RT_PASS_PATH_FRAME_PAR : 0u);
    ctx->last_lds = (uint32_t)b.lds_bytes;
    if (e != hipSuccess) return hip_fail(ctx, "rt_pathtrace_kernel launch", e);
    if (b.frame_par) {
        if (ctx->batches > 0) RT_HIP(ctx, hipStreamWaitEvent(b.S, ctx->ev_resolved[(ctx->batches - 1) & 1u], 0));
        e = rt_launch_resolve(ctx->d_accum, ctx->d_out, ka.frame_light, ctx->width, ctx->height, ctx->tiles_x,
                              ctx->owned_tiles, ctx->rank, ctx->world, p.accumulation_index, p.compute_per_frame,
                              b.frames, ka.launch_clock ? ka.launch_clock + 2 : nullptr, b.S);
        if (e != hipSuccess) return hip_fail(ctx, "rt_resolve_frames_kernel launch", e);
        RT_HIP(ctx, hipEventRecord(ctx->ev_resolved[ctx->batches & 1u], b.S));
        ctx->batches += 1;
    }
    ctx->queue_parity[b.si] ^= 1u;
    if (b.si) {
        RT_HIP(ctx, hipEventRecord(ctx->ev_aux_done, b.S));
        ctx->aux_outstanding = true;
    }
    if (!b.frame_par) ctx->primary_dirty = true;
    if (b.sched) ++ctx->sched_launches[b.si];
    return RT_OK;
}

static int dispatch_batch(rt_ctx* ctx, uint32_t bounces, uint32_t frames) {
    const rt_params& p = ctx->params;
    int rc;
    if ((rc = refresh_sphere_slots(ctx, p.sphere_count, p.object_count == 0)) ||
        (rc = refresh_tri_accel(ctx, p.object_count)))
        return rc;
    KernelArgs ka{};
    BatchLaunch b;
    b.bounces = bounces;
    b.frames = frames;
    batch_base_args(ctx, b, ka);
    if ((rc = plan_batch(ctx, b, ka))) return rc;
    scene_carve(ctx, ka, ctx->force_global_scene ? 0 : ctx->max_lds_mode, b.sl);
    if (ctx->brute) return launch_brute(ctx, b, ka);
    if ((rc = scene_accel_args(ctx, ka, b.sl)) || (rc = path_occupancy(ctx, b, ka))) return rc;
    if (b.blocks == 0) return RT_OK;
    if ((rc = select_stream(ctx, b, ka)) || (rc = schedule_state(ctx, b, ka)) ||
        (rc = claim_clock_slot(ctx, b.S, ka)) || (rc = primary_prepass(ctx, b, ka)))
        return rc;
    return launch_path_and_resolve(ctx, b, ka);
}

static int dispatch_frames(rt_ctx* ctx, uint32_t bounces, uint32_t frames) {
    const rt_params& p = ctx->params;
    const uint64_t samples = std::max<uint32_t>(1u, p.accumulate == 1u ? p.compute_per_frame : 1u);
    const uint64_t per_frame = (uint64_t)ctx->owned_tiles * 64u * samples * 2u * 2u * sizeof(float4);
    const uint64_t fit = std::max<uint64_t>(1u, ctx->batch_budget / std::max<uint64_t>(1u, per_frame));
    if (frames <= fit) return dispatch_batch(ctx, bounces, frames);
    const uint32_t k0 = ctx->params.accumulation_index;
    int rc = RT_OK;
    for (uint32_t done = 0; done < frames && rc == RT_OK;) {
        const uint32_t n = (uint32_t)std::min<uint64_t>(fit, frames - done);
        if (p.accumulate == 1u) ctx->params.accumulation_index = k0 + done;
        rc = dispatch_batch(ctx, bounces, n);
        done += n;
    }
    ctx->params.accumulation_index = k0;
    return rc;
}

int rth::flush_frames(rt_ctx* ctx) {
    if (ctx->pending_frames == 0) return RT_OK;
    const uint32_t n = ctx->pending_frames;
    ctx->pending_frames = 0;
    return dispatch_frames(ctx, ctx->pending_bounces, n);
}

int rt_dispatch(rt_ctx* ctx, uint32_t bounces) {
    RT_ENTER(ctx);
    return dispatch_frames(ctx, bounces, 1);
}

int rt_compute_frame(rt_ctx* ctx, uint32_t bounces) {
    if (!ctx || ctx->frame_batch <= 1) return rt_compute_frames(ctx, bounces, 1);
    if (ctx->pending_frames && bounces != ctx->pending_bounces) {
        RT_ENTER_NOFLUSH(ctx);
        const int rc = flush_frames(ctx);
        if (rc) return rc;
    }
    if (ctx->pending_frames == 0) {
        ctx->pending_bounces = bounces;
        if (ctx->params.accumulate) ctx->params.accumulation_index = ctx->k;
    }
    if (ctx->params.accumulate) ctx->k += 1;
    ctx->pending_frames += 1;
    if (ctx->pending_frames < ctx->frame_batch) return RT_OK;
    RT_ENTER_NOFLUSH(ctx);
    return flush_frames(ctx);
}

int rt_submit_frames(rt_ctx* ctx, uint32_t bounces, uint32_t count) {
    if (!ctx) return RT_E_INVALID;
    for (uint32_t i = 0; i < count; i++) {
        const int rc = rt_compute_frame(ctx, bounces);
        if (rc) return rc;
    }
    return RT_OK;
}

int rt_set_frame_batch(rt_ctx* ctx, uint32_t max_frames) {
    RT_ENTER(ctx);
    if (max_frames == 0 || max_frames > kMaxFrameBatch)
        return fail(ctx, RT_E_INVALID, "frame batch must be in [1, " + std::to_string(kMaxFrameBatch) + "]");
    ctx->frame_batch = max_frames;
    return RT_OK;
}

int rt_frame_batch(const rt_ctx* ctx, uint32_t* max_frames, uint32_t* pending) {
    if (!ctx || !max_frames || !pending) return RT_E_INVALID;
    *max_frames = ctx->frame_batch;
    *pending = ctx->pending_frames;
    return RT_OK;
}

int rt_flush(rt_ctx* ctx) {
    RT_ENTER(ctx);
    return RT_OK;
}

int rt_compute_frames(rt_ctx* ctx, uint32_t bounces, uint32_t frames) {
    RT_ENTER(ctx);
    if (frames == 0) return fail(ctx, RT_E_INVALID, "frames must be >= 1");
    if (ctx->params.accumulate) {
        ctx->params.accumulation_index = ctx->k;
        ctx->k += frames;
    }
    return dispatch_frames(ctx, bounces, frames);
}

int rt_synchronize(rt_ctx* ctx) {
    RT_ENTER(ctx);
    RT_HIP(ctx, hipStreamSynchronize(ctx->stream));
    return RT_OK;
}

int rth::copy_plane_to_device(rt_ctx* ctx, const char* entry, const uint32_t* src, const char* missing,
                         void* dst_device, uint32_t bytes_per_row) {
    if (dst_device && missing) return fail(ctx, RT_E_INVALID, std::string(entry) + ": " + missing);
    const int rc = check_device_ptrs(ctx, entry, {{dst_device, "dst_device", 1, false}});
    if (rc) return rc;
    if ((uint64_t)bytes_per_row < 4ull * ctx->width)
        return fail(ctx, RT_E_INVALID, std::string(entry) + ": bytes_per_row < 4 * width");
    RT_HIP(ctx, hipMemcpy2DAsync(dst_device, bytes_per_row, src, 4u * (size_t)ctx->width, 4u * (size_t)ctx->width,
                                 ctx->height, hipMemcpyDeviceToDevice, ctx->stream));
    return RT_OK;
}

int rt_copy_output_to_device(rt_ctx* ctx, void* dst_device, uint32_t bytes_per_row) {
    RT_ENTER(ctx);
    return copy_plane_to_device(ctx, "rt_copy_output_to_device", ctx->d_out,
                                ctx->world > 1 ? "a rank context (world_size > 1) has no full frame" : nullptr,
                                dst_device, bytes_per_row);
}

int rt_owned_pixel_count(const rt_ctx* ctx, uint32_t rank, uint32_t world_size, uint64_t* out) {
    if (!ctx || !out || world_size == 0 || rank >= world_size) return RT_E_INVALID;
    *out = (uint64_t)owned_tile_count(ctx->tiles_x * ctx->tiles_y, rank, world_size) * 64u;
    return RT_OK;
}

int rt_pack_owned_accumulation(rt_ctx* ctx, void* dst_device) {
    RT_ENTER(ctx);
    if (!dst_device) return fail(ctx, RT_E_INVALID, "dst is NULL");
    if (ctx->owned_tiles == 0) return RT_OK;
    hipError_t e = rt_launch_pack(ctx->d_accum, static_cast<float4*>(dst_device), ctx->width, ctx->height,
                                  ctx->tiles_x, ctx->owned_tiles, ctx->rank, ctx->world, ctx->stream);
    if (e != hipSuccess) return hip_fail(ctx, "rt_pack_tiles_kernel launch", e);
    return RT_OK;
}

int rt_unpack_accumulation(rt_ctx* ctx, const void* src_device, uint32_t src_rank, uint32_t world_size,
                           uint32_t divisor) {
    RT_ENTER(ctx);
    if (!src_device || world_size == 0 || src_rank >= world_size || divisor == 0)
        return fail(ctx, RT_E_INVALID, "unpack: bad arguments");
    hipError_t e = rt_launch_unpack(static_cast<const float4*>(src_device), ctx->d_accum, ctx->d_out, ctx->width,
                                    ctx->height, ctx->tiles_x, ctx->tiles_x * ctx->tiles_y, src_rank, 1, world_size,
                                    0, 0xffffffffu, (float)divisor, ctx->stream);
    if (e != hipSuccess) return hip_fail(ctx, "rt_unpack_tiles_kernel launch", e);
    return RT_OK;
}

int rt_unpack_accumulation_ranks(rt_ctx* ctx, const void* src_device, uint64_t stride_px, uint32_t world_size,
                                 uint32_t skip_rank, uint32_t divisor) {
    RT_ENTER(ctx);
    const uint64_t cap = (uint64_t)owned_tile_count(ctx->tiles_x * ctx->tiles_y, 0, world_size ? world_size : 1) * 64u;
    if (!src_device || world_size == 0 || divisor == 0 || stride_px < cap)
        return fail(ctx, RT_E_INVALID, "unpack: bad arguments (stride below the largest rank's block?)");
    hipError_t e = rt_launch_unpack(static_cast<const float4*>(src_device), ctx->d_accum, ctx->d_out, ctx->width,
                                    ctx->height, ctx->tiles_x, ctx->tiles_x * ctx->tiles_y, 0, world_size, world_size,
                                    stride_px, skip_rank, (float)divisor, ctx->stream);
    if (e != hipSuccess) return hip_fail(ctx, "rt_unpack_tiles_kernel launch", e);
    return RT_OK;
}

int rt_pack_owned_output(rt_ctx* ctx, void* dst_device) {
    RT_ENTER(ctx);
    if (!dst_device) return fail(ctx, RT_E_INVALID, "dst is NULL");
    if (ctx->owned_tiles == 0) return RT_OK;
    hipError_t e = rt_launch_pack_output(ctx->d_out, static_cast<uint32_t*>(dst_device), ctx->width, ctx->height,
                                         ctx->tiles_x, ctx->tiles_x * ctx->tiles_y, ctx->rank, 1, ctx->world, 0,
                                         0xffffffffu, false, ctx->stream);
    if (e != hipSuccess) return hip_fail(ctx, "rt_pack_output_kernel launch", e);
    return RT_OK;
}

int rt_unpack_output(rt_ctx* ctx, const void* src_device, uint32_t src_rank, uint32_t world_size) {
    RT_ENTER(ctx);
    if (!src_device || world_size == 0 || src_rank >= world_size) return fail(ctx, RT_E_INVALID, "unpack: bad arguments");
    hipError_t e = rt_launch_pack_output(ctx->d_out, const_cast<uint32_t*>(static_cast<const uint32_t*>(src_device)),
                                         ctx->width, ctx->height, ctx->tiles_x, ctx->tiles_x * ctx->tiles_y, src_rank, 1,
                                         world_size, 0, 0xffffffffu, true, ctx->stream);
    if (e != hipSuccess) return hip_fail(ctx, "rt_pack_output_kernel launch", e);
    return RT_OK;
}

int rt_unpack_output_ranks(rt_ctx* ctx, const void* src_device, uint64_t stride_px, uint32_t world_size,
                           uint32_t skip_rank) {
    RT_ENTER(ctx);
    const uint64_t cap = (uint64_t)owned_tile_count(ctx->tiles_x * ctx->tiles_y, 0, world_size ? world_size : 1) * 64u;
    if (!src_device || world_size == 0 || stride_px < cap)
        return fail(ctx, RT_E_INVALID, "unpack: bad arguments (stride below the largest rank's block?)");
    hipError_t e = rt_launch_pack_output(ctx->d_out, const_cast<uint32_t*>(static_cast<const uint32_t*>(src_device)),
                                         ctx->width, ctx->height, ctx->tiles_x, ctx->tiles_x * ctx->tiles_y, 0,
                                         world_size, world_size, stride_px, skip_rank, true, ctx->stream);
    if (e != hipSuccess) return hip_fail(ctx, "rt_pack_output_kernel launch", e);
    return RT_OK;
}
```

rust_gpu_raytracing_amd/csrc/rt_kernel_args.h:

```cpp
#pragma once
#include <hip/hip_runtime.h>
#include <stdint.h>

#include "tri_cone.h"

struct RtSphere {
    float position[3];
    float radius;
    uint32_t material_index;
    uint32_t _pad[3];
};

struct RtMaterial {
    uint32_t texture_index;
    float roughness;
    float emission_power;
    float specular;
    float specular_scatter;
    float glass;
    float refraction_index;
    uint32_t _pad;
};

struct RtObject {
    float min_bounds[3];
    uint32_t first_sub_object_index;
    float max_bounds[3];
    uint32_t sub_object_count;
    uint32_t material_index;
    uint32_t _pad[3];
};

struct RtSubObject {
    float min_bounds[3];
    uint32_t first_triangle_index;
    float max_bounds[3];
    uint32_t triangle_count;
};

struct RtTriangleHot {
    float4 p0;
    float4 p1;
    float4 p2;
    float4 fn;
};

__host__ __device__ inline RtTriangleHot pack_triangle(const float* a, const float* ab, const float* ac,
                                                       const float* cn, const float* fn) {
    RtTriangleHot h;
    h.p0 = make_float4(a[0], a[1], a[2], ab[0]);
    h.p1 = make_float4(ab[1], ab[2], ac[0], ac[1]);
    h.p2 = make_float4(ac[2], cn[0], cn[1], cn[2]);
    h.fn = make_float4(fn[0], fn[1], fn[2], 0.f);
    return h;
}

__host__ __device__ inline void unpack_triangle(const RtTriangleHot& h, float* a, float* ab, float* ac, float* cn,
                                                float* fn) {
    a[0] = h.p0.x, a[1] = h.p0.y, a[2] = h.p0.z;
    ab[0] = h.p0.w, ab[1] = h.p1.x, ab[2] = h.p1.y;
    ac[0] = h.p1.z, ac[1] = h.p1.w, ac[2] = h.p2.x;
    cn[0] = h.p2.y, cn[1] = h.p2.z, cn[2] = h.p2.w;
    fn[0] = h.fn.x, fn[1] = h.fn.y, fn[2] = h.fn.z;
}

static_assert(sizeof(RtSphere) == 32, "SceneSphere layout");
static_assert(sizeof(RtMaterial) == 32, "SceneMaterial layout");
static_assert(sizeof(RtObject) == 48, "ObjectInfo layout");
static_assert(sizeof(RtSubObject) == 32, "SubObjectInfo layout");
static_assert(sizeof(RtTriangleHot) == 64, "hot triangle layout");

#ifndef RT_ORDER_BUCKETS
#define RT_ORDER_BUCKETS 16
#endif
constexpr uint32_t kOrderBuckets = RT_ORDER_BUCKETS;
constexpr size_t kLdsTailBytes = 1024 + 160;
static_assert(kLdsTailBytes >= (kOrderBuckets * 16 + 1) * 4, "sort scratch fits the LDS tail");

constexpr uint32_t kEnvLineMax = 512;
constexpr uint32_t kEnvLineStaged = 4u;
static_assert(kLdsTailBytes % 16 == 0, "the environment line after the tail is 16-byte aligned");
__host__ __device__ inline uint32_t env_line_texels(uint32_t env_uniform, uint32_t env_w, uint32_t env_h) {
    switch (env_uniform & 3u) {
        case 3u: return 1u;
        case 1u: return env_h;
        case 2u: return env_w;
        default: return 0u;
    }
}

constexpr uint32_t kLeafTriSlots = 8;
constexpr uint32_t kLeafTriWords = 3 * kLeafTriSlots;
constexpr uint32_t kLeafBatchWaveBytes = 64 * 48;

constexpr uint32_t kQueueStripesMax = 64;
constexpr uint32_t kQueueStride = 64;

constexpr uint32_t kDiagHeaderWords = 32;

struct KernelArgs {
    const float4* __restrict__ camera_rays;
    float4* __restrict__ accum;
    uint32_t* __restrict__ output;
    unsigned long long* __restrict__ ray_counter;
    unsigned long long* __restrict__ diag;
    uint32_t* __restrict__ queue;
    uint32_t* __restrict__ queue_next;
    uint32_t* __restrict__ sched;
    const uint32_t* __restrict__ tile_order;
    uint32_t* __restrict__ tile_cost;
    const float4* __restrict__ sphere_slots;
    const uint32_t* __restrict__ sphere_orig;
    const uint32_t* __restrict__ sphere_material;
    const float4* __restrict__ sphere_bvh;
    const RtMaterial* __restrict__ materials;
    const RtObject* __restrict__ objects;
    const RtSubObject* __restrict__ sub_objects;
    const RtTriangleHot* __restrict__ triangles;
    const float4* __restrict__ tri_bvh;
    const uint4* __restrict__ tri_prims;
    const uint4* __restrict__ tri_qnodes;
    const float4* __restrict__ tri_qgrid;
    const uint32_t* __restrict__ textures;
    const uint32_t* __restrict__ env;
    const float* __restrict__ srgb;
    float camera_origin[3];
    float inv_proj[16];
    float inv_view[16];
    float aspect;
    uint32_t gen_rays;
    uint32_t width;
    uint32_t accumulation_index;
    uint32_t accumulate;
    uint32_t sphere_count;
    uint32_t object_count;
    uint32_t sphere_slot_count;
    uint32_t sphere_always;
    uint32_t sphere_nodes;
    uint32_t sphere_octant_stride;
    uint32_t sphere_boxes_ordered;
    float sphere_extent;
    float sphere_rmin, sphere_rmax;
    uint32_t tri_nodes;
    uint32_t tri_prim_count;
    uint32_t tri_accel;
    const float* __restrict__ tri_extent;
    uint32_t tri_octant_stride;
    uint32_t tri_prune_mode;
    float tri_prune;
    const TriLeafCert* __restrict__ tri_leafcert;
    const uint4* __restrict__ tri_leaftris;
    uint32_t lds_leafbatch_offset;
    uint32_t compute_per_frame;
    uint32_t frames;
    float4* __restrict__ frame_light;
    uint32_t queue_units;
    uint32_t unit_tile_major;
    unsigned long long* __restrict__ launch_clock;
    uint4* __restrict__ primary;
    uint32_t primary_tile_major;
    unsigned long long* __restrict__ stream_bytes;
    unsigned long long* __restrict__ l2_stream_bytes;
    float4* __restrict__ brute_paths;
    uint32_t* __restrict__ brute_queue;
    uint32_t* __restrict__ brute_counts;
    uint32_t brute_levels;
    uint32_t brute_pass;
    uint32_t brute_level;
    uint32_t texture_width;
    uint32_t texture_height;
    uint32_t env_map_width;
    uint32_t env_map_height;
    uint32_t material_count;
    uint32_t sub_object_count;
    uint32_t triangle_count;
    uint32_t tex_w, tex_h, tex_layers;
    uint32_t env_w, env_h;
    uint32_t env_uniform;
    uint32_t height;
    uint32_t bounces;
    uint32_t tiles_x;
    uint32_t owned_tiles;
    uint32_t rank;
    uint32_t world_size;
    uint32_t trav_threshold;
    uint32_t drain_threshold;
    uint32_t drain_min_steps;
    uint32_t leaf_batch;
    uint32_t queue_stripes;
    uint32_t sched_bits;
    uint32_t lds_mat_offset;
    uint32_t lds_mat_aux_offset;
    uint32_t lds_obj_offset;
    uint32_t lds_orig_offset;
    uint32_t lds_smat_offset;
    uint32_t lds_nodes_offset;
    uint32_t lds_tri_nodes_offset;
    uint32_t lds_tri_prims_offset;
    uint32_t lds_sub_offset;
    uint32_t lds_stack_offset;
    uint32_t lds_srgb_offset;
    uint32_t light_plane;
};
```

rust_gpu_raytracing_amd/csrc/rt_path_common.h:

```cpp
#pragma once
#include <hip/hip_runtime.h>
#include <stdint.h>

#include "rt_bvh_slab.h"
#include "rt_device_math.h"
#include "rt_kernel_args.h"
#include "rt_sphere_roots.h"
#include "tri_qnode.h"

#pragma clang fp contract(off)

using namespace rtk;

namespace {

struct Hit {
    float t;
    f3 p;
    f3 n;
    uint32_t material_index;
    bool front_face;
    float u, v;
};

struct SceneView {
    const float4* sph;
    const uint32_t* orig;
    const uint32_t* sph_mat;
    const float4* nodes;
    const RtMaterial* mat;
    const float4* mat_aux;
    const RtObject* obj;
    const float* srgb;
    const float4* tri_nodes;
    const uint4* tri_prims;
    float tri_extent;
    const RtSubObject* sub;
    const uint4* tri_q;
    float qox, qoy, qoz, qsx, qsy, qsz;
};

__device__ __forceinline__ f3 ld3(const float4& v) { return mk(v.x, v.y, v.z); }

__device__ __forceinline__ int texel_coord(float c, uint32_t size) {
    if (!(c >= 0.0f)) return 0;
    if (c >= (float)size) return (int)size - 1;
    const int i = (int)c;
    return i > (int)size - 1 ? (int)size - 1 : i;
}

__device__ __forceinline__ f4 decode_texel(uint32_t texel, const float* srgb) {
    return f4{srgb[texel & 0xffu], srgb[(texel >> 8) & 0xffu], srgb[(texel >> 16) & 0xffu],
              div_const((float)(texel >> 24), 255.0f, kInv255)};
}


__device__ __forceinline__ float sphere_disc(const float4 s, f3 o, f3 d, float four_a, float& b) {
    const f3 oc = o - ld3(s);
    b = 2.0f * dot(d, oc);
    const float c = dot(oc, oc) - s.w;
    return b * b - four_a * c;
}

template <bool kBySlot = false, class PassHook = SphereRootsNoHook>
__device__ __forceinline__ void test_sphere_group(const SceneView& sv, uint32_t slot, f3 o, f3 d, float four_a,
                                                  float two_a, SphereHit& best, PassHook pass = PassHook{}) {
    const float4 s0 = sv.sph[slot], s1 = sv.sph[slot + 1u], s2 = sv.sph[slot + 2u], s3 = sv.sph[slot + 3u];
    const uint4 og = *reinterpret_cast<const uint4*>(sv.orig + slot);
    float b[4], disc[4];
    disc[0] = sphere_disc(s0, o, d, four_a, b[0]);
    disc[1] = sphere_disc(s1, o, d, four_a, b[1]);
    disc[2] = sphere_disc(s2, o, d, four_a, b[2]);
    disc[3] = sphere_disc(s3, o, d, four_a, b[3]);
    const uint32_t orig[4] = {og.x, og.y, og.z, og.w};
    if constexpr (kBySlot)
        sphere_group_roots_by_slot(disc, b, orig, slot, two_a, best);
    else
        sphere_group_roots(disc, b, orig, slot, two_a, best, pass);
}

constexpr float kTriMarginScale = 1.0e-5f;

__device__ __forceinline__ bool ray_in_bounds(f3 o, f3 inv, const float* mn, const float* mx) {
    const float tminx = (mn[0] - o.x) * inv.x, tmaxx = (mx[0] - o.x) * inv.x;
    const float tminy = (mn[1] - o.y) * inv.y, tmaxy = (mx[1] - o.y) * inv.y;
    const float tminz = (mn[2] - o.z) * inv.z, tmaxz = (mx[2] - o.z) * inv.z;
    const float near_t = fmax_nn(fmax_nn(fmin_nn(tminx, tmaxx), fmin_nn(tminy, tmaxy)), fmin_nn(tminz, tmaxz));
    const float far_t = fmin_nn(fmin_nn(fmax_nn(tminx, tmaxx), fmax_nn(tminy, tmaxy)), fmax_nn(tminz, tmaxz));
    return near_t <= far_t && far_t >= 0.0f;
}

__device__ __forceinline__ bool ray_in_box4(f3 o, f3 inv, float4 lo, float4 hi) {
    const float mn[3] = {lo.x, lo.y, lo.z}, mx[3] = {hi.x, hi.y, hi.z};
    return ray_in_bounds(o, inv, mn, mx);
}

struct TriHit {
    float t;
    uint32_t seq, tri, obj;
    bool front;
};

struct TriGeom {
    f3 a, ab, ac, cn;
};
__device__ __forceinline__ TriGeom load_tri(const RtTriangleHot* __restrict__ t, uint32_t i) {
    const float4 p0 = t[i].p0, p1 = t[i].p1, p2 = t[i].p2;
    return TriGeom{mk(p0.x, p0.y, p0.z), mk(p0.w, p1.x, p1.y), mk(p1.z, p1.w, p2.x), mk(p2.y, p2.z, p2.w)};
}


__device__ __forceinline__ TriHit sweep_triangles(const SceneView& sv, const KernelArgs& ka, f3 o, f3 d) {
    TriHit th{kF32Max, 0u, 0u, 0u, false};
    float closest = kF32Max;
    const f3 inv = mk(1.0f / d.x, 1.0f / d.y, 1.0f / d.z);
    const uint32_t n_obj = ka.object_count;
    for (uint32_t oi = 0; oi < n_obj; ++oi) {
        const RtObject& ob = sv.obj[oi];
        if (!ray_in_bounds(o, inv, ob.min_bounds, ob.max_bounds)) continue;
        const uint32_t first_sub = ob.first_sub_object_index;
        const uint32_t n_sub = ob.sub_object_count;
        for (uint32_t i = 0; i < n_sub; ++i) {
            const uint32_t si = min(first_sub + i, ka.sub_object_count - 1u);
            const RtSubObject sub = sv.sub[si];
            if (!ray_in_bounds(o, inv, sub.min_bounds, sub.max_bounds)) continue;
            for (uint32_t j = 0; j < sub.triangle_count; ++j) {
                const uint32_t ti = min(sub.first_triangle_index + j, ka.triangle_count - 1u);
                const TriGeom g = load_tri(ka.triangles, ti);
                const float det = -dot(d, g.cn);
                const float inv_det = 1.0f / det;
                const f3 ao = o - g.a;
                const float dist = dot(ao, g.cn) * inv_det;
                if (dist < 0.0f || dist >= closest) continue;
                const f3 dao = cross(ao, d);
                const float v = -dot(g.ab, dao) * inv_det;
                if (v < 0.0f) continue;
                const float u = dot(g.ac, dao) * inv_det;
                if (u < 0.0f) continue;
                const float w = 1.0f - u - v;
                if (w < 0.0f) continue;
                closest = dist;
                th.t = dist;
                th.tri = ti;
                th.obj = oi;
                th.front = det > 0.0f;
            }
        }
    }
    return th;
}

constexpr uint32_t kNoLeaf = 0xffffffffu;

struct TraceState {
    f3 inv;
    float a4, a2;
    SlabRay slab;
    float slack;
    float limit;
    uint32_t node;
    uint32_t phase;
    uint32_t pending;
    float cert_gap;
    bool nan_hit;
    SphereHit sph;
    TriHit tri;
};

__device__ __forceinline__ float prune_limit(const TraceState& ts) {
    return fmin_nn(ts.sph.t, ts.tri.t) * 1.00001f + ts.slack;
}

constexpr float kTriPruneAbs = 0x1p-10f;
__device__ __forceinline__ float tri_limit(const SceneView& sv, const KernelArgs& ka, f3 o, const TraceState& ts) {
    if (ka.tri_prune == 0.0f || ts.tri.t == kF32Max) return __builtin_inff();
    const float r = sqrt_up(dot(o, o));
    const float sig = kTriPruneAbs * (r + sv.tri_extent) * (__builtin_amdgcn_rsqf(ts.a2 * 0.5f) * 1.001f);
    return ts.tri.t * (1.0f + ka.tri_prune) + sig;
}

__device__ __forceinline__ uint32_t tri_leaf_skips(const KernelArgs& ka, uint32_t prim, const SlabRay& sr, f3 o, f3 d,
                                                   float tb, float4 lo, float4 hi) {
    const uint4* rec = reinterpret_cast<const uint4*>(ka.tri_leafcert + prim);
    const uint4 c0 = rec[0], c1 = rec[1];
    const uint32_t w[8] = {c0.x, c0.y, c0.z, c0.w, c1.x, c1.y, c1.z, c1.w};
    const float t1x = fminf(fmaf(lo.x, sr.ix, sr.lx), fmaf(hi.x, sr.ix, sr.hx));
    const float t1y = fminf(fmaf(lo.y, sr.iy, sr.ly), fmaf(hi.y, sr.iy, sr.hy));
    const float t1z = fminf(fmaf(lo.z, sr.iz, sr.lz), fmaf(hi.z, sr.iz, sr.hz));
    return tri_leafcert_skips(w, tri_cone_ray(o.x, o.y, o.z, d.x, d.y, d.z), tb, t1x, t1y, t1z, fabsf(sr.ix),
                              fabsf(sr.iy), fabsf(sr.iz));
}


template <bool kLazySub = false>
__device__ __forceinline__ void tri_leaf(const SceneView& sv, const KernelArgs& ka, f3 o, f3 d, TraceState& ts,
                                         uint32_t pending) {
    const uint32_t prim = pending & 0xffffffu;
    uint32_t skip = 0u;
    if ((pending >> 24) & 1u) {
        const uint4* rec = reinterpret_cast<const uint4*>(ka.tri_leafcert + prim);
        const uint4 c0 = rec[0], c1 = rec[1];
        const uint32_t w[8] = {c0.x, c0.y, c0.z, c0.w, c1.x, c1.y, c1.z, c1.w};
        skip = tri_leafcert_skips_gap(w, tri_cone_ray(o.x, o.y, o.z, d.x, d.y, d.z), ts.tri.t, ts.cert_gap);
        if (skip == kLeafCertAll) return;
    }
    const uint4 pr = sv.tri_prims[prim];
    const RtObject& ob = sv.obj[pr.x];
    if (!ray_in_bounds(o, ts.inv, ob.min_bounds, ob.max_bounds)) return;
    uint32_t first, count;
    int sub_state;
    if (kLazySub && pr.w != 0xffffffffu) {
        first = pr.w & ((1u << 27) - 1u);
        count = pr.w >> 27;
        sub_state = 0;
    } else {
        const RtSubObject sub = sv.sub[pr.y];
        if (!ray_in_bounds(o, ts.inv, sub.min_bounds, sub.max_bounds)) return;
        first = sub.first_triangle_index;
        count = sub.triangle_count;
        sub_state = 1;
    }
    for (uint32_t j = 0; j < count; ++j) {
        if ((skip >> j) & 1u) continue;
        const uint32_t ti = min(first + j, ka.triangle_count - 1u);
        const uint32_t seq = pr.z + j;
        const TriGeom g = load_tri(ka.triangles, ti);
        const float det = -dot(d, g.cn);
        const float inv_det = 1.0f / det;
        const f3 ao = o - g.a;
        const float dist = dot(ao, g.cn) * inv_det;
        const bool nan_dist = dist != dist;
        if (dist < 0.0f) continue;
        if (!nan_dist && !(dist < ts.tri.t || (dist == ts.tri.t && seq < ts.tri.seq))) continue;
        const f3 dao = cross(ao, d);
        const float v = -dot(g.ab, dao) * inv_det;
        if (v < 0.0f) continue;
        const float u = dot(g.ac, dao) * inv_det;
        if (u < 0.0f) continue;
        const float w = 1.0f - u - v;
        if (w < 0.0f) continue;
        if (kLazySub && sub_state == 0) {
            const RtSubObject sub = sv.sub[pr.y];
            if (!ray_in_bounds(o, ts.inv, sub.min_bounds, sub.max_bounds)) return;
            sub_state = 1;
        }
        if (nan_dist) {
            ts.nan_hit = true;
            continue;
        }
        ts.tri = TriHit{dist, seq, ti, pr.x, det > 0.0f};
    }
}

template <bool kTris, bool kAlwaysUv = false>
__device__ __forceinline__ Hit trace_end(const SceneView& sv, const KernelArgs& ka, f3 o, f3 d, const TraceState& ts) {
    Hit h;
    h.t = kF32Max;
    h.p = mk(0.f, 0.f, 0.f);
    h.n = mk(0.f, 0.f, 0.f);
    h.material_index = 0;
    h.front_face = false;
    h.u = 0.f;
    h.v = 0.f;
    if (kTris && ts.tri.t != kF32Max) {
        const RtObject& ob = sv.obj[ts.tri.obj];
        const f3 fn = ld3(ka.triangles[ts.tri.tri].fn);
        h.front_face = ts.tri.front;
        h.n = ts.tri.front ? fn : -fn;
        h.t = ts.tri.t;
        h.p = o + d * ts.tri.t;
        if (kAlwaysUv || ka.tex_w != 1u || ka.tex_h != 1u) {
            h.u = (h.p.x - ob.min_bounds[0]) / (ob.max_bounds[0] - ob.min_bounds[0]);
            h.v = (h.p.z - ob.min_bounds[2]) / (ob.max_bounds[2] - ob.min_bounds[2]);
        }
        h.material_index = ob.material_index;
    }
    if (ts.sph.t < h.t) {
        const float4 s = sv.sph[ts.sph.slot];
        const float t = ts.sph.t;
        const f3 p = o + d * t;
        const f3 outward = normalize(p - ld3(s));
        h.t = t;
        h.p = p;
        if (kAlwaysUv || ka.tex_w != 1u || ka.tex_h != 1u) {
            const float theta = acosf_c(-outward.y);
            const float phi = atan2f_c(-outward.z, outward.x) + kWgslPi;
            h.u = div_const(phi, kTwoPiWgsl, kInvTwoPiWgsl);
            h.v = div_const(theta, kWgslPi, kInvWgslPi);
        }
        h.front_face = dot(d, outward) < 0.0f;
        h.n = h.front_face ? outward : -outward;
        h.material_index = sv.sph_mat[ts.sph.orig];
    }
    return h;
}

struct HitId {
    uint32_t kind, index, triangle;
};
template <bool kTris>
__device__ __forceinline__ HitId trace_end_id(const TraceState& ts) {
    const float tt = (kTris && ts.tri.t != kF32Max) ? ts.tri.t : kF32Max;
    if (ts.sph.t < tt) return HitId{1u, ts.sph.orig, 0u};
    if (kTris && ts.tri.t != kF32Max) return HitId{2u, ts.tri.obj, ts.tri.tri};
    return HitId{0u, 0u, 0u};
}

struct ShadeArgs {
    const uint32_t* __restrict__ textures;
    const uint32_t* __restrict__ env;
    uint32_t texture_width, texture_height, env_map_width, env_map_height, material_count;
    uint32_t tex_w, tex_h, tex_layers, env_w, env_h, env_uniform;
    uint32_t bounces;
};

template <class KA>
__device__ __forceinline__ uint32_t fetch_texture(const KA& ka, uint32_t layer, float u, float v) {
    const int x = texel_coord(u * (float)(int32_t)ka.texture_width, ka.tex_w);
    const int y = texel_coord(v * (float)(int32_t)ka.texture_height, ka.tex_h);
    const uint32_t l = min(layer, ka.tex_layers - 1u);
    const size_t off = ((size_t)l * ka.tex_h + (size_t)y) * ka.tex_w + (size_t)x;
    return ka.textures[off];
}

template <bool kLine = false, class KA>
__device__ __forceinline__ f4 sample_env(const KA& ka, const float* srgb, f3 d) {
    int x = 0, y = 0;
    if (!(ka.env_uniform & 1u)) {
        const float u = 0.5f + div_const(atan2f_c(d.z, d.x), kTwoPiWgsl, kInvTwoPiWgsl);
        x = texel_coord(u * (float)(int32_t)ka.env_map_width, ka.env_w);
    }
    if (!(ka.env_uniform & 2u)) {
        const float v = 0.5f + div_const(asinf_c(d.y), kWgslPi, kInvWgslPi);
        y = texel_coord(v * (float)(int32_t)ka.env_map_height, ka.env_h);
    }
    if (kLine && (ka.env_uniform & kEnvLineStaged)) {
        const float4 c = (reinterpret_cast<const float4*>(srgb) + kLdsTailBytes / sizeof(float4))[x + y];
        return f4{c.x, c.y, c.z, c.w};
    }
    return decode_texel(ka.env[(size_t)y * ka.env_w + (size_t)x], srgb);
}

struct Path {
    f3 o, d;
    f4 light, contrib;
    uint32_t seed;
    uint32_t bounce;
};

__device__ __forceinline__ f3 mat4_mul_xyz(const float* m, float x, float y, float z, float w, float& out_w) {
    const float r0 = ((m[0] * x + m[4] * y) + m[8] * z) + m[12] * w;
    const float r1 = ((m[1] * x + m[5] * y) + m[9] * z) + m[13] * w;
    const float r2 = ((m[2] * x + m[6] * y) + m[10] * z) + m[14] * w;
    out_w = ((m[3] * x + m[7] * y) + m[11] * z) + m[15] * w;
    return mk(r0, r1, r2);
}

__device__ __forceinline__ f3 camera_ray(const KernelArgs& ka, const float* cam, uint32_t x, uint32_t y) {
    const float xc = (float)x / (float)ka.width;
    const float yc = (float)y / (float)ka.height;
    const float nx = xc * 2.0f - 1.0f;
    const float ny = yc * 2.0f - 1.0f;
    const float ax = nx * cam[32];
    float tw;
    const f3 t = mat4_mul_xyz(cam, ax, ny, 1.0f, 1.0f, tw);
    const f3 ws = normalize(mk(t.x / tw, t.y / tw, t.z / tw));
    float unused;
    return mat4_mul_xyz(cam + 16, ws.x, ws.y, ws.z, 0.0f, unused);
}

__device__ __forceinline__ f3 pixel_ray(const KernelArgs& ka, const float* cam, uint32_t index, uint32_t x,
                                        uint32_t y) {
    if (ka.gen_rays) return camera_ray(ka, cam, x, y);
    const float4 cr = ka.camera_rays[index];
    return mk(cr.x, cr.y, cr.z);
}

__device__ __forceinline__ void start_sample(const KernelArgs& ka, uint32_t index, uint32_t random_index, f3 cam,
                                             Path& p) {
    p.o = mk(ka.camera_origin[0], ka.camera_origin[1], ka.camera_origin[2]);
    p.d = cam;
    p.seed = index * random_index * 326624u;
    const float rx = random01(p.seed), ry = random01(p.seed), rz = random01(p.seed);
    const f3 jit = mk(rx * 2.0f - 1.0f, ry * 2.0f - 1.0f, rz * 2.0f - 1.0f);
    p.d = p.d + jit * 0.0005f;
    p.contrib = f4{1.0f, 1.0f, 1.0f, 1.0f};
    p.light = f4{0.0f, 0.0f, 0.0f, 0.0f};
    p.bounce = 0;
}

__device__ __forceinline__ void start_sample_at(f3 origin, uint32_t stream, uint32_t random_index, f3 dir, Path& p) {
    p.o = origin;
    p.d = dir;
    p.seed = stream * random_index * 326624u;
    const float rx = random01(p.seed), ry = random01(p.seed), rz = random01(p.seed);
    const f3 jit = mk(rx * 2.0f - 1.0f, ry * 2.0f - 1.0f, rz * 2.0f - 1.0f);
    p.d = p.d + jit * 0.0005f;
    p.contrib = f4{1.0f, 1.0f, 1.0f, 1.0f};
    p.light = f4{0.0f, 0.0f, 0.0f, 0.0f};
    p.bounce = 0;
}

template <bool kAux, bool kEnvLine = false, class KA>
__device__ __forceinline__ bool shade(const SceneView& sv, const KA& ka, Path& p, const Hit& h) {
    if (h.t == kF32Max) {
        const f4 c = sample_env<kEnvLine>(ka, sv.srgb, p.d);
        p.light.x = p.light.x + c.x * p.contrib.x;
        p.light.y = p.light.y + c.y * p.contrib.y;
        p.light.z = p.light.z + c.z * p.contrib.z;
        p.light.w = p.light.w + c.w * p.contrib.w;
        return true;
    }
    const uint32_t mi = min(h.material_index, ka.material_count - 1u);
    const RtMaterial m = sv.mat[mi];
    const bool tex1 = kAux && ka.tex_w == 1u && ka.tex_h == 1u;
    uint32_t texel = 0;
    if (!tex1) texel = fetch_texture(ka, m.texture_index, h.u, h.v);
    const float gx = normal01(p.seed);
    const float gy = normal01(p.seed);
    const float gz = normal01(p.seed);
    const f3 diffuse = normalize(h.n + mk(gx, gy, gz));
    const f3 specular = p.d - h.n * (2.0f * dot(h.n, p.d));
    f4 color;
    if (tex1) {
        const float4 c = sv.mat_aux[2u * mi + 1u];
        color = f4{c.x, c.y, c.z, c.w};
    } else {
        color = decode_texel(texel, sv.srgb);
    }
    const float e = m.emission_power;
    p.light.x = p.light.x + (color.x * e) * p.contrib.x;
    p.light.y = p.light.y + (color.y * e) * p.contrib.y;
    p.light.z = p.light.z + (color.z * e) * p.contrib.z;
    p.light.w = p.light.w + (color.w * e) * p.contrib.w;
    const bool is_glass = m.glass > random01(p.seed);
    bool tint;
    if (is_glass) {
        float ior, r0, rough10;
        if constexpr (kAux) {
            const float4 ax = sv.mat_aux[2u * mi];
            ior = h.front_face ? ax.x : m.refraction_index;
            r0 = h.front_face ? ax.y : ax.z;
            rough10 = ax.w;
        } else {
            ior = m.refraction_index;
            if (h.front_face) ior = 1.0f / ior;
            r0 = (1.0f - ior) / (1.0f + ior);
            r0 = r0 * r0;
            rough10 = div_const(m.roughness, 10.0f, kInv10);
        }
        const float cos_t = fmin_nn(dot(-p.d, h.n), 1.0f);
        const float sin_t = sqrt_rn_nrm(1.0f - cos_t * cos_t);
        const bool reflects = ior * sin_t > 1.0f;
        const float sp = r0 + (1.0f - r0) * pow5(1.0f - cos_t);
        const bool is_spec = (m.specular * sp) > random01(p.seed);
        if (reflects || is_spec) {
            p.d = lerp(specular, diffuse, m.specular_scatter);
            p.o = h.p + h.n * 0.0001f;
            tint = false;
        } else {
            const f3 perp = (p.d + h.n * cos_t) * ior;
            const float len = sqrt_rn_any(dot(perp, perp));
            const float len_sq = len * len;
            const f3 refr = perp + h.n * (-sqrt_rn_nrm(__builtin_fabsf(1.0f - len_sq)));
            p.d = lerp(refr, diffuse, rough10);
            p.o = h.p - h.n * 0.0001f;
            tint = true;
        }
    } else {
        const bool is_spec = m.specular > random01(p.seed);
        if (is_spec) {
            p.d = lerp(specular, diffuse, m.specular_scatter);
            tint = false;
        } else {
            p.d = lerp(specular, diffuse, m.roughness);
            tint = true;
        }
        p.o = h.p + h.n * 0.0001f;
    }
    if (tint) {
        p.contrib.x = p.contrib.x * color.x;
        p.contrib.y = p.contrib.y * color.y;
        p.contrib.z = p.contrib.z * color.z;
        p.contrib.w = p.contrib.w * color.w;
    }
    p.bounce += 1;
    return p.bounce >= ka.bounces;
}

__device__ __forceinline__ float clamp01(float x) { return fmin_nn(fmax_nn(x, 0.0f), 1.0f); }

__device__ __forceinline__ uint32_t pack_rgba8(float r, float g, float b, float a) {
    const uint32_t br = (uint32_t)(r * 255.0f) & 0xffu;
    const uint32_t bg = (uint32_t)(g * 255.0f) & 0xffu;
    const uint32_t bb = (uint32_t)(b * 255.0f) & 0xffu;
    const uint32_t ba = (uint32_t)(a * 255.0f) & 0xffu;
    return br | (bg << 8) | (bb << 16) | (ba << 24);
}


struct PrimaryRecord {
    float t;
    uint32_t id;
    uint32_t meta;
    uint32_t orig;
};

template <bool kTris>
__device__ __forceinline__ PrimaryRecord primary_record(const TraceState& ts) {
    const float tt = kTris ? ts.tri.t : kF32Max;
    if (ts.sph.t < (tt != kF32Max ? tt : kF32Max))
        return PrimaryRecord{ts.sph.t, ts.sph.slot, 1u << 30, ts.sph.orig};
    return PrimaryRecord{tt, ts.tri.tri, (ts.tri.obj & 0x3fffffffu) | (ts.tri.front ? 0x80000000u : 0u), 0u};
}

__device__ __forceinline__ void primary_state(const PrimaryRecord& r, TraceState& ts) {
    ts.sph = SphereHit{kF32Max, 0u, 0u};
    ts.tri = TriHit{kF32Max, 0u, 0u, 0u, false};
    if (r.meta & (1u << 30)) {
        ts.sph = SphereHit{r.t, r.orig, r.id};
    } else {
        ts.tri = TriHit{r.t, 0u, r.id, r.meta & 0x3fffffffu, (r.meta & 0x80000000u) != 0u};
    }
}

template <bool kTris, uint32_t kThreads>
__device__ __forceinline__ SceneView brute_stage(const KernelArgs& ka, unsigned char* lds, uint32_t tid, float*& l_cam) {
    float4* l_sph = reinterpret_cast<float4*>(lds);
    RtMaterial* l_mat = reinterpret_cast<RtMaterial*>(lds + ka.lds_mat_offset);
    float4* l_aux = reinterpret_cast<float4*>(lds + ka.lds_mat_aux_offset);
    RtObject* l_obj = reinterpret_cast<RtObject*>(lds + ka.lds_obj_offset);
    uint32_t* l_orig = reinterpret_cast<uint32_t*>(lds + ka.lds_orig_offset);
    uint32_t* l_smat = reinterpret_cast<uint32_t*>(lds + ka.lds_smat_offset);
    float* l_srgb = reinterpret_cast<float*>(lds + ka.lds_srgb_offset);
    for (uint32_t i = tid; i < ka.sphere_slot_count; i += kThreads) {
        l_sph[i] = ka.sphere_slots[i];
        l_orig[i] = ka.sphere_orig[i];
    }
    for (uint32_t i = tid; i < ka.sphere_count; i += kThreads) l_smat[i] = ka.sphere_material[i];
    for (uint32_t i = tid; i < ka.material_count; i += kThreads) {
        const RtMaterial m = ka.materials[i];
        l_mat[i] = m;
        const float ior_front = 1.0f / m.refraction_index;
        float r0f = (1.0f - ior_front) / (1.0f + ior_front);
        float r0b = (1.0f - m.refraction_index) / (1.0f + m.refraction_index);
        r0f = r0f * r0f;
        r0b = r0b * r0b;
        l_aux[2u * i] = make_float4(ior_front, r0f, r0b, div_const(m.roughness, 10.0f, kInv10));
        const f4 c = decode_texel(ka.textures[min(m.texture_index, ka.tex_layers - 1u)], ka.srgb);
        l_aux[2u * i + 1u] = make_float4(c.x, c.y, c.z, c.w);
    }
    if constexpr (kTris)
        for (uint32_t i = tid; i < ka.object_count; i += kThreads) l_obj[i] = ka.objects[i];
    for (uint32_t i = tid; i < 256u; i += kThreads) l_srgb[i] = ka.srgb[i];
    l_cam = l_srgb + 256;
    if (tid < 16u) {
        l_cam[tid] = ka.inv_proj[tid];
        l_cam[16u + tid] = ka.inv_view[tid];
    }
    if (tid == 0) l_cam[32] = ka.aspect;
    return SceneView{l_sph, l_orig, l_smat, nullptr, l_mat, l_aux, l_obj, l_srgb, nullptr, nullptr, 0.0f,
                     ka.sub_objects};
}

}
```

rust_gpu_raytracing_amd/csrc/rt_walk.h:

```cpp
#pragma once
#include <hip/hip_runtime.h>
#include <stdint.h>

#include "rt_path_common.h"

#pragma clang fp contract(off)

using namespace rtk;

namespace {

template <bool kTris>
__device__ __forceinline__ void phase_setup(const SceneView& sv, const KernelArgs& ka, f3 o, float a, uint32_t phase,
                                            TraceState& ts) {
    const float r = sqrt_up(dot(o, o));
    float m;
    if (phase == 0) {
        m = kTriMarginScale * (r + sv.tri_extent) + 1.0e-30f;
        ts.slack = 0.0f;
    } else {
        sphere_cull_bounds(r, ka.sphere_extent, ka.sphere_rmin, ka.sphere_rmax, __builtin_amdgcn_rsqf(a), m,
                           ts.slack);
    }
    ts.slab = slab_ray(o.x, o.y, o.z, ts.inv.x, ts.inv.y, ts.inv.z, m);
    ts.limit = phase == 0 ? __builtin_inff() : prune_limit(ts);
    if (kTris && phase == 0) {
        const uint32_t oct = (__float_as_uint(ts.inv.x) >> 31) | ((__float_as_uint(ts.inv.y) >> 31) << 1) |
                             ((__float_as_uint(ts.inv.z) >> 31) << 2);
        ts.node = oct * ka.tri_octant_stride;
    }
    if (phase == 1) {
        const uint32_t oct = (__float_as_uint(ts.inv.x) >> 31) | ((__float_as_uint(ts.inv.y) >> 31) << 1) |
                             ((__float_as_uint(ts.inv.z) >> 31) << 2);
        ts.node = oct * ka.sphere_octant_stride;
        if constexpr (!kTris)
            if (ka.sphere_boxes_ordered) slab_pair_by_octant(ts.slab);
    }
}

template <bool kTris>
__device__ __forceinline__ void trace_begin(const SceneView& sv, const KernelArgs& ka, f3 o, f3 d, TraceState& ts) {
    if constexpr (kTris) {
        ts.inv = mk(1.0f / d.x, 1.0f / d.y, 1.0f / d.z);
    } else {
        ts.inv = mk(__builtin_amdgcn_rcpf(d.x), __builtin_amdgcn_rcpf(d.y), __builtin_amdgcn_rcpf(d.z));
    }
    const float a = dot(d, d);
    ts.a4 = 4.0f * a;
    ts.a2 = 2.0f * a;
    ts.sph = SphereHit{kF32Max, 0u, 0u};
    ts.tri = TriHit{kF32Max, 0u, 0u, 0u, false};
    ts.nan_hit = false;
    ts.node = 0;
    ts.pending = kNoLeaf;
    uint32_t i = 0;
    for (; i + 4u <= ka.sphere_always; i += 4u) test_sphere_group<true>(sv, i, o, d, ts.a4, ts.a2, ts.sph);
    if (ka.sphere_always - i >= 2u) {
        test_sphere_group<true>(sv, i, o, d, ts.a4, ts.a2, ts.sph);
    } else if (ka.sphere_always - i == 1u) {
        float b;
        const float disc = sphere_disc(sv.sph[i], o, d, ts.a4, b);
        sphere_candidate(disc, b, ts.a2, sv.orig[i], i, ts.sph);
    }
    if constexpr (!kTris) {
        ts.phase = 1;
    } else if (!ka.tri_accel) {
        ts.tri = sweep_triangles(sv, ka, o, d);
        ts.phase = 1;
    } else {
        ts.phase = ka.tri_nodes != 0 ? 0u : 1u;
    }
    if (ts.phase == 1 && ka.sphere_nodes == 0) ts.phase = 2;
    phase_setup<kTris>(sv, ka, o, a, ts.phase, ts);
}

__device__ __forceinline__ uint32_t lane_id_here() {
    uint32_t l;
    asm volatile("v_mbcnt_lo_u32_b32 %0, -1, 0\n\tv_mbcnt_hi_u32_b32 %0, -1, %0" : "=v"(l));
    return l;
}

template <bool kTris>
__device__ __forceinline__ void phase_end(const SceneView& sv, const KernelArgs& ka, f3 o, f3 d, TraceState& ts) {
    if (ts.pending != kNoLeaf) return;
    if (kTris && ts.phase == 0) {
        if (ts.node < ka.tri_nodes) return;
#ifdef RT_DIAG_TAIL
        if (ts.nan_hit) atomicAdd(ka.diag + 6, 1ull);
#endif
        if (ts.nan_hit) ts.tri = sweep_triangles(sv, ka, o, d);
        ts.node = 0;
        ts.phase = ka.sphere_nodes != 0 ? 1u : 2u;
        phase_setup<kTris>(sv, ka, o, ts.a2 * 0.5f, 1, ts);
    } else if (ts.node >= ka.sphere_nodes) {
        ts.phase = 2;
    }
}

template <bool kTris>
constexpr bool kDeferLeaves = kTris;
template <bool kTris>
constexpr bool kBlockLeaves = !kTris;
#ifndef RT_BLOCK_LEAF_SHARE
#define RT_BLOCK_LEAF_SHARE 3
#endif
constexpr uint32_t kBlockLeafShare = RT_BLOCK_LEAF_SHARE;
#ifndef RT_SPHERE_TRAV_UNROLL
#define RT_SPHERE_TRAV_UNROLL 4
#endif
template <int kMode, bool kTris>
constexpr int kTravUnroll = !kTris ? RT_SPHERE_TRAV_UNROLL : kMode <= 1 ? 5 : 3;
template <int kMode, bool kTris>
constexpr bool kFusedLeaves = kTris && kMode == 2;

template <int kMode, bool kTris>
constexpr bool kDrainDecouple = kTris && kMode < 2;

template <int kMode>
constexpr bool kCertWalk = kMode <= 1;

__device__ __forceinline__ void qnode_decode(const SceneView& sv, uint4 q, uint32_t node, float4& lo, float4& hi) {
    lo = make_float4(fmaf((float)(q.x & 0xffffu), sv.qsx, sv.qox), fmaf((float)(q.x >> 16), sv.qsy, sv.qoy),
                     fmaf((float)(q.y & 0xffffu), sv.qsz, sv.qoz), 0.0f);
    hi = make_float4(fmaf((float)(q.y >> 16), sv.qsx, sv.qox), fmaf((float)(q.z & 0xffffu), sv.qsy, sv.qoy),
                     fmaf((float)(q.z >> 16), sv.qsz, sv.qoz), 0.0f);
    const bool is_leaf = (q.w & 0x80000000u) != 0u;
    lo.w = __uint_as_float(is_leaf ? ((q.w & kTriQLastLeaf) ? kTriWalkEnd : node + 1u) : q.w);
    hi.w = __uint_as_float(is_leaf ? (q.w & 0xffffffu) : 0xffffffffu);
}

template <bool kTris, bool kCert>
__device__ __forceinline__ void node_visit(const SceneView& sv, const KernelArgs& ka, f3 o, f3 d, TraceState& ts,
                                           bool tri, float4 lo, float4 hi) {
    float near_t, far_t;
    if (!kTris && ka.sphere_boxes_ordered)
        slab_hit_ordered(ts.slab, lo.x, lo.y, lo.z, hi.x, hi.y, hi.z, near_t, far_t);
    else
        slab_hit(ts.slab, lo.x, lo.y, lo.z, hi.x, hi.y, hi.z, near_t, far_t);
    const bool hit = near_t <= far_t && far_t >= -ts.slack && near_t <= ts.limit;
    const uint32_t leaf = __float_as_uint(hi.w);
    uint32_t skip = 0u;
    if constexpr (kTris && kCert) {
        if (tri && hit && leaf != 0xffffffffu && ka.tri_leafcert && near_t > ts.tri.t && ts.tri.t != kF32Max &&
            ts.pending == kNoLeaf) {
            const float tbs = ts.tri.t * (1.0f + 0x1p-20f);
            const SlabRay& sr = ts.slab;
            const float gx = (fminf(fmaf(lo.x, sr.ix, sr.lx), fmaf(hi.x, sr.ix, sr.hx)) - tbs) * fabsf(d.x);
            const float gy = (fminf(fmaf(lo.y, sr.iy, sr.ly), fmaf(hi.y, sr.iy, sr.hy)) - tbs) * fabsf(d.y);
            const float gz = (fminf(fmaf(lo.z, sr.iz, sr.lz), fmaf(hi.z, sr.iz, sr.hz)) - tbs) * fabsf(d.z);
            ts.cert_gap = fmaxf(fmaxf(gx, gy), gz) * (1.0f - 0x1p-20f);
            skip = ts.cert_gap > 0.0f ? 1u : 0u;
        }
    }
    const bool at_leaf = hit && leaf != 0xffffffffu;
#ifdef RT_DIAG
    if constexpr (!kDeferLeaves<kTris>) {
        const uint64_t act = __ballot(true), lf = __ballot(at_leaf);
        if ((threadIdx.x & 63u) == (uint32_t)__builtin_ctzll(act)) {
            atomicAdd(ka.diag + 22, 1ull);
            atomicAdd(ka.diag + 23, (unsigned long long)__popcll(act));
            if (lf) {
                atomicAdd(ka.diag + 24, 1ull);
                atomicAdd(ka.diag + 25, (unsigned long long)__popcll(lf));
            }
        }
    }
#endif
    if (at_leaf && !kDeferLeaves<kTris> && !kBlockLeaves<kTris>) {
        test_sphere_group(sv, leaf & 0xffffffu, o, d, ts.a4, ts.a2, ts.sph);
        ts.limit = prune_limit(ts);
    } else if (at_leaf) {
        if (ts.pending != kNoLeaf) return;
        ts.pending = (leaf & 0xffffffu) | (skip << 24);
    }
    ts.node = (hit && !at_leaf) ? ts.node + 1u : __float_as_uint(lo.w);
}

template <bool kTris, bool kCert = true>
__device__ __forceinline__ void node_step(const SceneView& sv, const KernelArgs& ka, f3 o, f3 d, TraceState& ts) {
    const bool tri = kTris && ts.phase == 0;
    if (kDeferLeaves<kTris> && ts.node >= (tri ? ka.tri_nodes : ka.sphere_nodes))
        return;
    if (kBlockLeaves<kTris> && ts.pending != kNoLeaf) return;
    float4 lo, hi;
    if (kTris && tri && sv.tri_q) {
        qnode_decode(sv, sv.tri_q[ts.node], ts.node, lo, hi);
    } else {
        const float4* nodes = tri ? sv.tri_nodes : sv.nodes;
        lo = nodes[2u * ts.node];
        hi = nodes[2u * ts.node + 1u];
    }
    node_visit<kTris, kCert>(sv, ka, o, d, ts, tri, lo, hi);
}

template <bool kTris, bool kLazySub = false>
__device__ __forceinline__ void leaf_step(const SceneView& sv, const KernelArgs& ka, f3 o, f3 d, TraceState& ts) {
    if (kTris && ts.phase == 0) {
        tri_leaf<kLazySub>(sv, ka, o, d, ts, ts.pending);
        ts.limit = tri_limit(sv, ka, o, ts);
    } else {
        test_sphere_group(sv, ts.pending, o, d, ts.a4, ts.a2, ts.sph);
        ts.limit = prune_limit(ts);
    }
    ts.pending = kNoLeaf;
}

template <int kMode, bool kTris>
constexpr bool kCoopLeaves = kTris && kMode <= 1;

__device__ __forceinline__ void wave_lds_sync() {
    __builtin_amdgcn_fence(__ATOMIC_SEQ_CST, "wavefront");
    __builtin_amdgcn_wave_barrier();
}

template <int kCtrl>
__device__ __forceinline__ void coop_min_step(float& cd, uint32_t& cs, uint32_t& ct) {
    const float od = __int_as_float(__builtin_amdgcn_update_dpp(0, __float_as_int(cd), kCtrl, 0xf, 0xf, false));
    const uint32_t os = (uint32_t)__builtin_amdgcn_update_dpp(0, (int)cs, kCtrl, 0xf, 0xf, false);
    const uint32_t ot = (uint32_t)__builtin_amdgcn_update_dpp(0, (int)ct, kCtrl, 0xf, 0xf, false);
    const bool take = od < cd || (od == cd && os < cs);
    cd = take ? od : cd;
    cs = take ? os : cs;
    ct = take ? ot : ct;
}

__device__ __forceinline__ void coop_leaf_batch(const SceneView& sv, const KernelArgs& ka, f3 o, f3 d, TraceState& ts,
                                                bool active, unsigned char* lds) {
    bool want = false;
    uint32_t prim = 0u, range = 0u, seq0 = 0u, obj = 0u, sub = 0u;
    if (active) {
        if (ts.phase == 0) {
            prim = ts.pending & 0xffffffu;
            uint32_t skip = 0u;
            if ((ts.pending >> 24) & 1u) {
                const uint4* rec = reinterpret_cast<const uint4*>(ka.tri_leafcert + prim);
                const uint4 c0 = rec[0], c1 = rec[1];
                const uint32_t w[8] = {c0.x, c0.y, c0.z, c0.w, c1.x, c1.y, c1.z, c1.w};
                skip = tri_leafcert_skips_gap(w, tri_cone_ray(o.x, o.y, o.z, d.x, d.y, d.z), ts.tri.t, ts.cert_gap);
            }
            if (skip != kLeafCertAll) {
                const uint4 pr = sv.tri_prims[prim];
                const RtObject& ob = sv.obj[pr.x];
                if (ray_in_bounds(o, ts.inv, ob.min_bounds, ob.max_bounds)) {
                    if (pr.w != kPrimRangeNone && (pr.w >> 27) < kLeafTriSlots) {
                        want = true;
                        range = pr.w;
                        seq0 = pr.z;
                        obj = pr.x;
                        sub = pr.y;
                    } else {
                        tri_leaf<true>(sv, ka, o, d, ts, prim);
                        ts.limit = tri_limit(sv, ka, o, ts);
                    }
                }
            }
        } else {
            test_sphere_group(sv, ts.pending, o, d, ts.a4, ts.a2, ts.sph);
            ts.limit = prune_limit(ts);
        }
        ts.pending = kNoLeaf;
    }
    const uint64_t wm = __ballot(want);
    if (wm == 0) return;
    const uint32_t wave = __builtin_amdgcn_readfirstlane(threadIdx.x >> 6);
    float4* const scratch = reinterpret_cast<float4*>(lds + ka.lds_leafbatch_offset + wave * kLeafBatchWaveBytes);
    const uint32_t n = (uint32_t)__popcll(wm);
    const uint32_t rank = __builtin_amdgcn_mbcnt_hi((uint32_t)(wm >> 32), __builtin_amdgcn_mbcnt_lo((uint32_t)wm, 0u));
    if (want) {
        float4* sl = scratch + 3u * rank;
        sl[0] = make_float4(o.x, o.y, o.z, __uint_as_float(prim));
        sl[1] = make_float4(d.x, d.y, d.z, __uint_as_float(range));
        sl[2] = make_float4(__uint_as_float(seq0), __uint_as_float(obj), __uint_as_float(sub), 0.0f);
    }
    wave_lds_sync();
    const uint32_t lane = lane_id_here(), g = lane >> 3, j = lane & 7u;
    for (uint32_t base = 0; base < n; base += 8u) {
        const uint32_t kk = base + g;
        float cd = __builtin_inff();
        uint32_t cs = 0xffffffffu, ct = 0u;
        bool cnan = false;
        if (kk < n) {
            const float4* sl = scratch + 3u * kk;
            const float4 s0 = sl[0], s1 = sl[1];
            const uint32_t rg = __float_as_uint(s1.w);
            if (j < (rg >> 27)) {
                const uint4* blk = ka.tri_leaftris + (size_t)__float_as_uint(s0.w) * kLeafTriWords + j;
                const uint4 q0 = blk[0], q1 = blk[kLeafTriSlots], q2 = blk[2u * kLeafTriSlots];
                const float4 p0 = make_float4(__uint_as_float(q0.x), __uint_as_float(q0.y), __uint_as_float(q0.z),
                                              __uint_as_float(q0.w));
                const float4 p1 = make_float4(__uint_as_float(q1.x), __uint_as_float(q1.y), __uint_as_float(q1.z),
                                              __uint_as_float(q1.w));
                const float4 p2 = make_float4(__uint_as_float(q2.x), __uint_as_float(q2.y), __uint_as_float(q2.z),
                                              __uint_as_float(q2.w));
                const TriGeom tg{mk(p0.x, p0.y, p0.z), mk(p0.w, p1.x, p1.y), mk(p1.z, p1.w, p2.x),
                                 mk(p2.y, p2.z, p2.w)};
                const f3 ro = mk(s0.x, s0.y, s0.z), rd = mk(s1.x, s1.y, s1.z);
                const float det = -dot(rd, tg.cn);
                const float inv_det = 1.0f / det;
                const f3 ao = ro - tg.a;
                const float dist = dot(ao, tg.cn) * inv_det;
                const f3 dao = cross(ao, rd);
                const float v = -dot(tg.ab, dao) * inv_det;
                const float u = dot(tg.ac, dao) * inv_det;
                const float w = 1.0f - u - v;
                if (!(dist < 0.0f) && !(v < 0.0f) && !(u < 0.0f) && !(w < 0.0f)) {
                    if (dist != dist) {
                        cnan = true;
                    } else {
                        cd = dist;
                        cs = __float_as_uint(sl[2].x) + j;
                        ct = min((rg & ((1u << 27) - 1u)) + j, ka.triangle_count - 1u) | (det > 0.0f ? 0x80000000u : 0u);
                    }
                }
            }
        }
        coop_min_step<0xB1>(cd, cs, ct);
        coop_min_step<0x4E>(cd, cs, ct);
        coop_min_step<0x141>(cd, cs, ct);
        const uint64_t nm = __ballot(cnan);
        if (j == 0u && kk < n)
            scratch[3u * kk] = make_float4(cd, __uint_as_float(cs), __uint_as_float(ct),
                                           __uint_as_float(((nm >> (8u * g)) & 0xffu) != 0u ? 1u : 0u));
    }
    wave_lds_sync();
    if (want) {
        const float4 r = scratch[3u * rank];
        const float4 r2 = scratch[3u * rank + 2u];
        obj = __float_as_uint(r2.y);
        sub = __float_as_uint(r2.z);
        const float rd = r.x;
        const uint32_t rs = __float_as_uint(r.y), rt = __float_as_uint(r.z);
        const bool rnan = __float_as_uint(r.w) != 0u;
        const bool beats = rd < ts.tri.t || (rd == ts.tri.t && rs < ts.tri.seq);
        if (rnan || beats) {
            const RtSubObject so = sv.sub[sub];
            if (ray_in_bounds(o, ts.inv, so.min_bounds, so.max_bounds)) {
                if (rnan) ts.nan_hit = true;
                if (beats) ts.tri = TriHit{rd, rs, rt & 0x7fffffffu, obj, (rt >> 31) != 0u};
            }
        }
        ts.limit = tri_limit(sv, ka, o, ts);
    }
}

}
```

Before: 28310.

## Stage per-pass kernel constants in LDS to relieve scalar register pressure

Copies the kernel arguments the persistent loop uses (pointers, sizes, scene counts, LDS addresses) into a PassConstants block in LDS once per workgroup. For kMode>=1 the main loop re-reads them each iteration through an opaque LDS address and readfirstlane, so they do not stay live in SGPRs or VGPRs across the loop. The helper functions are templated on the argument source to support this. The cost is extra LDS reads and readfirstlane instructions per iteration, plus 288 bytes of LDS that shift the environment line's offset.

```diff
diff --git a/rust_gpu_raytracing_amd/csrc/pathtrace.hip b/rust_gpu_raytracing_amd/csrc/pathtrace.hip
--- a/rust_gpu_raytracing_amd/csrc/pathtrace.hip
+++ b/rust_gpu_raytracing_amd/csrc/pathtrace.hip
@@ -2,6 +2,7 @@
 #include <stdint.h>
 
 #include <algorithm>
+#include <type_traits>
 
 #include "rt_launch.h"
 #include "rt_path_common.h"
@@ -34,11 +35,35 @@
                      RT_KERNARG(kp, env_uniform),     RT_KERNARG(kp, bounces)};
 }
 
+__device__ __forceinline__ uint32_t lds_address(const void* p) {
+    return (uint32_t)(uintptr_t)(const __attribute__((address_space(3))) void*)p;
+}
+
+__device__ __forceinline__ LdsPassConstants& pass_constants_fresh(const float* l_srgb) {
+    uint32_t a = lds_address(l_srgb) + (uint32_t)kLdsTailBytes;
+    asm volatile("" : "+v"(a));
+    return *reinterpret_cast<LdsPassConstants*>(a);
+}
+template <class KA, class T>
+__device__ __forceinline__ T* uniform_ptr(T* p) {
+    static_assert(!kInLds<KA>, "the block's pointers are RT_GLOBAL");
+    return p;
+}
+template <class KA, class T>
+__device__ __forceinline__ T* uniform_ptr(RT_GLOBAL T* p) {
+    const uint64_t v = (uint64_t)p;
+    const uint32_t hi = (uint32_t)__builtin_amdgcn_readfirstlane((uint32_t)(v >> 32));
+    const uint32_t lo = (uint32_t)__builtin_amdgcn_readfirstlane((uint32_t)v);
+    return (T*)(RT_GLOBAL T*)(((uint64_t)hi << 32) | (uint64_t)lo);
+}
+template <class T>
+__device__ __forceinline__ const T* lds_object(uint32_t address) {
+    return (const T*)reinterpret_cast<const __attribute__((address_space(3))) T*>(address);
+}
+
 constexpr uint32_t kPrimaryThreads = 1024;
 
 
-__device__ __forceinline__ uint32_t* sched_orders(const KernelArgs& ka) { return ka.sched + 2u * ka.owned_tiles; }
-__device__ __forceinline__ uint32_t* sched_flags(const KernelArgs& ka) { return ka.sched + 4u * ka.owned_tiles; }
 
 __device__ __forceinline__ uint32_t xcc_id() {
     return __builtin_amdgcn_s_getreg((3 << 11) | (0 << 6) | 20);
@@ -49,10 +74,15 @@
     uint32_t empty;
 };
 
-__device__ __forceinline__ uint32_t claim_tile(const KernelArgs& ka, TileQueue& q) {
-    const uint32_t n_str = ka.queue_stripes;
+template <class KA>
+__device__ __forceinline__ uint32_t claim_tile(const KA& ca, TileQueue& q) {
+    if (q.empty) return 0xffffffffu;
+    struct {
+        uint32_t* queue;
+        uint32_t queue_units;
+    } ka{uniform_ptr<KA>(ca.queue), wave_uniform<KA>(ca.queue_units)};
+    const uint32_t n_str = wave_uniform<KA>(ca.queue_stripes);
     const uint32_t lane = threadIdx.x & 63u;
-    if (q.empty) return 0xffffffffu;
     uint32_t old = 0;
     if (lane == 0) old = atomicAdd(ka.queue + q.stripe * kQueueStride, 1u);
     uint64_t pos = (uint64_t)__builtin_amdgcn_readlane(old, 0) * n_str + q.stripe;
@@ -78,21 +108,24 @@
     }
 }
 
-template <bool kFramePar>
-__device__ __forceinline__ uint32_t unit_tile(const KernelArgs& ka, uint32_t pos, uint32_t& frame) {
+template <bool kFramePar, class KA>
+__device__ __forceinline__ uint32_t unit_tile(const KA& ka, uint32_t pos, uint32_t& frame) {
     if (pos == 0xffffffffu) return pos;
     uint32_t q;
-    if (!kFramePar && !ka.frame_light) {
+    if (!kFramePar && !uniform_ptr<KA>(ka.frame_light)) {
         frame = 0u;
         q = pos;
-    } else if (ka.unit_tile_major) {
-        q = pos / ka.frames;
-        frame = pos - q * ka.frames;
+    } else if (wave_uniform<KA>(ka.unit_tile_major)) {
+        const uint32_t frames = wave_uniform<KA>(ka.frames);
+        q = pos / frames;
+        frame = pos - q * frames;
     } else {
-        frame = pos / ka.owned_tiles;
-        q = pos - frame * ka.owned_tiles;
-    }
-    return ka.tile_order ? ka.tile_order[q] : q;
+        const uint32_t owned_tiles = wave_uniform<KA>(ka.owned_tiles);
+        frame = pos / owned_tiles;
+        q = pos - frame * owned_tiles;
+    }
+    const uint32_t* order = uniform_ptr<KA>(ka.tile_order);
+    return order ? order[q] : q;
 }
 
 __device__ __forceinline__ void record_tile_cost(uint32_t* cost, bool fin, uint32_t tile, uint32_t n) {
@@ -218,10 +251,6 @@
 template <int kMode, bool kTris>
 constexpr bool kLinkedWalk = kBlockLeaves<kTris> && kMode >= 1;
 
-__device__ __forceinline__ uint32_t lds_address(const void* p) {
-    return (uint32_t)(uintptr_t)(const __attribute__((address_space(3))) void*)p;
-}
-
 template <int kMode, uint32_t kThreads, bool kTris, bool kFramePar>
 __global__ void __launch_bounds__(kThreads, 1) rt_pathtrace_kernel(KernelArgs ka) {
     extern __shared__ __attribute__((aligned(16))) unsigned char lds[];
@@ -284,7 +313,7 @@
         }
         sv.mat_aux = l_aux;
         if (ka.env_uniform & kEnvLineStaged) {
-            float4* l_env = reinterpret_cast<float4*>(l_srgb) + kLdsTailBytes / sizeof(float4);
+            float4* l_env = reinterpret_cast<float4*>(l_srgb) + kEnvLineOffset / sizeof(float4);
             const uint32_t n = env_line_texels(ka.env_uniform, ka.env_w, ka.env_h);
             const size_t stride = (ka.env_uniform & 2u) ? 1u : ka.env_w;
             for (uint32_t i = tid; i < n; i += kThreads) {
@@ -294,6 +323,32 @@
         }
         if constexpr (kTris)
             for (uint32_t i = tid; i < ka.object_count; i += kThreads) l_obj[i] = ka.objects[i];
+        if (tid == 0) {
+            PassConstants& c = *reinterpret_cast<PassConstants*>(reinterpret_cast<unsigned char*>(l_srgb) + kLdsTailBytes);
+            const auto global = [](auto* p) { return (RT_GLOBAL std::remove_pointer_t<decltype(p)>*)p; };
+            c.textures = global(ka.textures), c.env = global(ka.env), c.triangles = global(ka.triangles);
+            c.camera_rays = global(ka.camera_rays), c.accum = global(ka.accum), c.output = global(ka.output);
+            c.frame_light = global(ka.frame_light), c.primary = global(ka.primary), c.queue = global(ka.queue);
+            c.tile_order = global(ka.tile_order), c.tile_cost = global(ka.tile_cost), c.sched = global(ka.sched);
+            c.ray_counter = global(ka.ray_counter), c.launch_clock = global(ka.launch_clock);
+            c.texture_width = ka.texture_width, c.texture_height = ka.texture_height;
+            c.env_map_width = ka.env_map_width, c.env_map_height = ka.env_map_height;
+            c.material_count = ka.material_count, c.tex_w = ka.tex_w, c.tex_h = ka.tex_h, c.tex_layers = ka.tex_layers;
+            c.env_w = ka.env_w, c.env_h = ka.env_h, c.env_uniform = ka.env_uniform, c.bounces = ka.bounces;
+            c.lds_mat = lds_address(l_mat), c.lds_mat_aux = lds_address(l_aux), c.lds_sph_mat = lds_address(l_smat);
+            c.light_plane = ka.light_plane, c.compute_per_frame = ka.compute_per_frame;
+            c.accumulation_index = ka.accumulation_index, c.accumulate = ka.accumulate, c.frames = ka.frames;
+            c.gen_rays = ka.gen_rays, c.width = ka.width, c.height = ka.height, c.tiles_x = ka.tiles_x;
+            c.owned_tiles = ka.owned_tiles, c.rank = ka.rank, c.world_size = ka.world_size;
+            c.camera_origin[0] = ka.camera_origin[0], c.camera_origin[1] = ka.camera_origin[1];
+            c.camera_origin[2] = ka.camera_origin[2];
+            c.queue_units = ka.queue_units, c.queue_stripes = ka.queue_stripes;
+            c.unit_tile_major = ka.unit_tile_major, c.sched_bits = ka.sched_bits;
+            c.sphere_always = ka.sphere_always, c.sphere_nodes = ka.sphere_nodes;
+            c.sphere_octant_stride = ka.sphere_octant_stride, c.sphere_boxes_ordered = ka.sphere_boxes_ordered;
+            c.sphere_extent = ka.sphere_extent, c.sphere_rmin = ka.sphere_rmin, c.sphere_rmax = ka.sphere_rmax;
+            c.tri_nodes = ka.tri_nodes, c.tri_accel = ka.tri_accel, c.tri_octant_stride = ka.tri_octant_stride;
+        }
         sv.sph = l_sph;
         sv.orig = l_orig;
         sv.sph_mat = l_smat;
@@ -323,8 +378,9 @@
     if (tid == 0) l_cam[32] = ka.aspect;
     __syncthreads();
 
-    const bool accumulate = kFramePar || ka.accumulate == 1u;
-    const uint32_t samples = accumulate ? ka.compute_per_frame : 1u;
+    const auto accumulates = [](const auto& ca) { return kFramePar || ca.accumulate == 1u; };
+    const auto samples_of = [&](const auto& ca) { return accumulates(ca) ? ca.compute_per_frame : 1u; };
+    const auto frame_par_of = [](const auto& ca) { return kFramePar || ca.frame_light != nullptr; };
     constexpr bool kLinked = kLinkedWalk<kMode, kTris>;
     const uint32_t walk_base = kLinked ? lds_address(lds + ka.lds_nodes_offset) : 0u;
     const uint32_t walk_end = kLinked ? sphere_links_addr(walk_base, ka.sphere_nodes) : ka.sphere_nodes;
@@ -334,7 +390,6 @@
     uint32_t rays = 0;
     uint32_t lane_tile = 0;
     uint32_t lane_slot = 0;
-    const bool frame_par = kFramePar || ka.frame_light != nullptr;
     uint32_t mode = kIdle;
     uint32_t index = 0, sample = 0, frame = 0;
     float4 pix = make_float4(0.f, 0.f, 0.f, 0.f);
@@ -351,15 +406,16 @@
     ts.sph = SphereHit{kF32Max, 0u, 0u};
     ts.tri = TriHit{kF32Max, 0u, 0u, 0u, false};
 
-    auto random_index = [&]() { return ka.accumulation_index + (accumulate ? frame : 0u) + sample; };
-    auto primary_start = [&]() -> uint32_t {
-        return (kTris && ka.primary && p.bounce < ka.bounces) ? kPrimary : kSetup;
+    auto random_index = [&](const auto& ca) { return ca.accumulation_index + (accumulates(ca) ? frame : 0u) + sample; };
+    auto primary_start = [&](const auto& ca) -> uint32_t {
+        return (kTris && ca.primary && p.bounce < ca.bounces) ? kPrimary : kSetup;
     };
 
-    auto store_frame = [&]() {
+    auto store_frame = [&](const auto& ca) {
         float r, g, b, a;
+        const bool accumulate = accumulates(ca);
         if (accumulate) {
-            const float div = (float)((ka.accumulation_index + frame) * ka.compute_per_frame);
+            const float div = (float)((ca.accumulation_index + frame) * ca.compute_per_frame);
             r = clamp01(pix.x / div);
             g = clamp01(pix.y / div);
             b = clamp01(pix.z / div);
@@ -370,29 +426,32 @@
             b = clamp01(p.light.z);
             a = clamp01(p.light.w);
         }
-        if (accumulate) ka.accum[index] = pix;
-        ka.output[index] = pack_rgba8(r, g, b, a);
+        if (accumulate) plain_ptr(ca.accum)[index] = pix;
+        plain_ptr(ca.output)[index] = pack_rgba8(r, g, b, a);
     };
-    auto finish_sample_frame_par = [&]() {
-        const size_t plane = kFramePar ? (size_t)ka.light_plane : (size_t)ka.owned_tiles * 64u;
+    auto finish_sample_frame_par = [&](const auto& ca) {
+        const uint32_t samples = samples_of(ca);
+        const size_t plane = kFramePar ? (size_t)ca.light_plane : (size_t)ca.owned_tiles * 64u;
         const size_t slot = (size_t)(frame * samples + sample) * plane + (size_t)lane_tile * 64u + lane_slot;
-        ka.frame_light[slot] = make_float4(p.light.x, p.light.y, p.light.z, p.light.w);
+        plain_ptr(ca.frame_light)[slot] = make_float4(p.light.x, p.light.y, p.light.z, p.light.w);
         sample += 1;
         if (sample < samples) {
-            start_sample(ka, index, random_index(), pixel_ray(ka, l_cam, index, index % ka.width, index / ka.width), p);
-            mode = primary_start();
+            start_sample(ca, index, random_index(ca), pixel_ray(ca, l_cam, index, index % ca.width, index / ca.width), p);
+            mode = primary_start(ca);
         } else {
             mode = kIdle;
         }
     };
-    auto finish_sample = [&]() {
+    auto finish_sample = [&](const auto& ca) {
         if constexpr (kFramePar) {
-            finish_sample_frame_par();
+            finish_sample_frame_par(ca);
         } else {
-            if (frame_par) {
-                finish_sample_frame_par();
+            if (frame_par_of(ca)) {
+                finish_sample_frame_par(ca);
                 return;
             }
+            const uint32_t samples = samples_of(ca);
+            const bool accumulate = accumulates(ca);
             sample += 1;
             if (accumulate) {
                 pix.x = pix.x + p.light.x;
@@ -400,17 +459,17 @@
                 pix.z = pix.z + p.light.z;
                 pix.w = pix.w + p.light.w;
             }
-            if (sample == samples && frame + 1u < ka.frames) {
-                store_frame();
+            if (sample == samples && frame + 1u < ca.frames) {
+                store_frame(ca);
                 frame += 1;
                 sample = 0;
             }
             if (sample < samples) {
-                start_sample(ka, index, random_index(), pixel_ray(ka, l_cam, index, index % ka.width, index / ka.width),
+                start_sample(ca, index, random_index(ca), pixel_ray(ca, l_cam, index, index % ca.width, index / ca.width),
                              p);
-                mode = primary_start();
+                mode = primary_start(ca);
             } else {
-                store_frame();
+                store_frame(ca);
                 mode = kIdle;
             }
         }
@@ -438,10 +497,18 @@
         ++iters;
         const unsigned long long ts0 = stamp();
 #endif
+        decltype(auto) ca = [&]() -> decltype(auto) {
+            if constexpr (kMode >= 1)
+                return pass_constants_fresh(l_srgb);
+            else
+                return (ka);
+        }();
+        using CA = std::remove_reference_t<decltype(ca)>;
+        const uint32_t owned_tiles = wave_uniform<CA>(ca.owned_tiles);
         bool fin = false;
         uint32_t fin_rays = 0;
         if (kTris && mode == kPrimary) {
-            const uint4 r = ka.primary[(size_t)(frame * samples + sample) * ((size_t)ka.owned_tiles * 64u) +
+            const uint4 r = plain_ptr(ca.primary)[(size_t)(frame * samples_of(ca) + sample) * ((size_t)ca.owned_tiles * 64u) +
                                        (size_t)lane_tile * 64u + lane_slot];
             primary_state(PrimaryRecord{__uint_as_float(r.x), r.y, r.z, r.w}, ts);
             mode = kDone;
@@ -456,7 +523,13 @@
         }
 #endif
         if (mode == kDone) {
-            const Hit h = trace_end<kTris>(sv, ka, p.o, p.d, ts);
+            SceneView svs = sv;
+            if constexpr (kMode >= 1) {
+                svs.mat = lds_object<RtMaterial>(ca.lds_mat);
+                svs.mat_aux = lds_object<float4>(ca.lds_mat_aux);
+                svs.sph_mat = lds_object<uint32_t>(ca.lds_sph_mat);
+            }
+            const Hit h = trace_end<kTris>(svs, ca, p.o, p.d, ts);
 #ifdef RT_DIAG
             {
                 const bool miss = h.t == kF32Max;
@@ -470,23 +543,27 @@
             RT_ISA_MARK("shade");
             bool ended;
             uint32_t bounce_limit;
-            if constexpr (kFramePar) {
+            if constexpr (kMode >= 1) {
+                ended = shade<true, true>(svs, ca, p, h);
+                bounce_limit = ca.bounces;
+            } else if constexpr (kFramePar) {
                 const ShadeArgs sa = load_shade_args(kernarg_fresh(kernarg));
-                ended = shade<(kMode >= 1), (kMode >= 1)>(sv, sa, p, h);
+                ended = shade<false, false>(sv, sa, p, h);
                 bounce_limit = sa.bounces;
             } else {
-                ended = shade<(kMode >= 1), (kMode >= 1)>(sv, ka, p, h);
+                ended = shade<false, false>(sv, ka, p, h);
                 bounce_limit = ka.bounces;
             }
             if (ended) {
                 fin = true;
                 fin_rays = p.bounce + (p.bounce < bounce_limit ? 1u : 0u);
-                finish_sample();
+                finish_sample(ca);
             } else {
                 mode = kSetup;
             }
         }
-        if (ka.tile_cost) record_tile_cost(ka.tile_cost, fin && (!frame_par || frame == 0u), lane_tile, fin_rays);
+        if (uint32_t* const tile_cost = uniform_ptr<CA>(ca.tile_cost))
+            record_tile_cost(tile_cost, fin && (!frame_par_of(ca) || frame == 0u), lane_tile, fin_rays);
 #ifdef RT_DIAG
         const unsigned long long ts1 = stamp();
         shade_cyc += ts1 - ts0;
@@ -494,35 +571,35 @@
         RT_ISA_MARK("refill");
         while (true) {
             const uint64_t need = __ballot(mode == kIdle);
-            if (need == 0 || tile >= ka.owned_tiles) break;
+            if (need == 0 || tile >= owned_tiles) break;
             const uint32_t avail = 64u - next;
             if (mode == kIdle) {
                 const uint32_t rank =
                     __builtin_amdgcn_mbcnt_hi((uint32_t)(need >> 32), __builtin_amdgcn_mbcnt_lo((uint32_t)need, 0u));
                 if (rank < avail) {
                     const uint32_t slot = next + rank;
-                    const uint32_t gt = tile * ka.world_size + ka.rank;
-                    const uint32_t x = (gt % ka.tiles_x) * 8u + (slot & 7u);
-                    const uint32_t y = (gt / ka.tiles_x) * 8u + (slot >> 3);
-                    if (x < ka.width && y < ka.height) {
-                        index = y * ka.width + x;
+                    const uint32_t gt = tile * ca.world_size + ca.rank;
+                    const uint32_t x = (gt % ca.tiles_x) * 8u + (slot & 7u);
+                    const uint32_t y = (gt / ca.tiles_x) * 8u + (slot >> 3);
+                    if (x < ca.width && y < ca.height) {
+                        index = y * ca.width + x;
                         lane_tile = tile;
                         lane_slot = slot;
                         sample = 0;
                         frame = tile_frame;
                         mode = kSetup;
-                        if (!kFramePar && accumulate && !frame_par) pix = ka.accum[index];
-                        start_sample(ka, index, random_index(), pixel_ray(ka, l_cam, index, x, y), p);
-                        mode = primary_start();
+                        if (!kFramePar && accumulates(ca) && !frame_par_of(ca)) pix = plain_ptr(ca.accum)[index];
+                        start_sample(ca, index, random_index(ca), pixel_ray(ca, l_cam, index, x, y), p);
+                        mode = primary_start(ca);
                     }
                 }
             }
             next += min((uint32_t)__popcll(need), avail);
             if (next == 64u) {
-                tile = unit_tile<kFramePar>(ka, claim_tile(ka, queue), tile_frame);
+                tile = unit_tile<kFramePar>(ca, claim_tile(ca, queue), tile_frame);
                 next = 0;
             #ifdef RT_DIAG_TAIL
-                if (tile >= ka.owned_tiles && wave_dry == 0) wave_dry = realtime();
+                if (tile >= owned_tiles && wave_dry == 0) wave_dry = realtime();
 #endif
             }
         }
@@ -542,9 +619,9 @@
         RT_ISA_MARK("setup");
         if (mode == kSetup) {
             if constexpr (!kFramePar)
-                while (mode == kSetup && p.bounce >= ka.bounces) finish_sample();
+                while (mode == kSetup && p.bounce >= ca.bounces) finish_sample(ca);
             if (kFramePar || mode == kSetup) {
-                trace_begin<kTris>(sv, ka, p.o, p.d, ts);
+                trace_begin<kTris>(sv, ka, ca, p.o, p.d, ts);
                 if constexpr (kLinkedWalk<kMode, kTris>) ts.node = sphere_links_addr(walk_base, ts.node);
                 mode = ts.phase == 2 ? kDone : kTrav;
             }
@@ -552,8 +629,8 @@
 #ifdef RT_DIAG
         setup_cyc += stamp() - ts2;
 #endif
-        if (__ballot(mode != kIdle) == 0 && tile >= ka.owned_tiles) break;
-        const bool draining = tile >= ka.owned_tiles;
+        if (__ballot(mode != kIdle) == 0 && tile >= owned_tiles) break;
+        const bool draining = tile >= owned_tiles;
         uint32_t thresh = draining ? 0u : ka.trav_threshold;
         uint32_t n_active = 64u, min_steps = 0u;
         if constexpr (kDrainDecouple<kMode, kTris>) {
@@ -741,24 +818,33 @@
         }
     }
 #endif
+    decltype(auto) ca = [&]() -> decltype(auto) {
+        if constexpr (kMode >= 1)
+            return pass_constants_fresh(l_srgb);
+        else
+            return (ka);
+    }();
     atomicAdd(&block_rays, rays);
     __syncthreads();
-    if (tid == 0 && block_rays != 0) atomicAdd(ka.ray_counter, (unsigned long long)block_rays);
-    if (ka.sched) {
-        const uint32_t par = ka.sched_bits & 1u, n = ka.owned_tiles;
+    if (tid == 0 && block_rays != 0) atomicAdd(plain_ptr(ca.ray_counter), (unsigned long long)block_rays);
+    using CA = std::remove_reference_t<decltype(ca)>;
+    if (uint32_t* const sched = uniform_ptr<CA>(ca.sched)) {
+        const uint32_t par = wave_uniform<CA>(ca.sched_bits) & 1u, n = wave_uniform<CA>(ca.owned_tiles);
+        uint32_t* const flags = sched + 4u * n;
+        uint32_t* const orders = sched + 2u * n;
         __shared__ uint32_t sorter;
         if (tid == 0) {
-            sorter = atomicAdd(sched_flags(ka) + par, 1u);
-            if (blockIdx.x == 0) sched_flags(ka)[par ^ 1u] = 0u;
+            sorter = atomicAdd(flags + par, 1u);
+            if (blockIdx.x == 0) flags[par ^ 1u] = 0u;
         }
         __syncthreads();
         if (sorter == 0)
-            sort_tiles_by_cost<kThreads>(ka.sched + (par ^ 1u) * n, sched_orders(ka) + (par ^ 1u) * n, n,
-                                         reinterpret_cast<uint32_t*>(lds + ka.lds_srgb_offset));
-    }
-    if (ka.launch_clock) {
+            sort_tiles_by_cost<kThreads>(sched + (par ^ 1u) * n, orders + (par ^ 1u) * n, n,
+                                         reinterpret_cast<uint32_t*>(l_srgb));
+    }
+    if (unsigned long long* const launch_clock = uniform_ptr<CA>(ca.launch_clock)) {
         __syncthreads();
-        if (tid == 0) atomicMax(ka.launch_clock + 1, (unsigned long long)wall_clock64());
+        if (tid == 0) atomicMax(launch_clock + 1, (unsigned long long)wall_clock64());
     }
 }
 
diff --git a/rust_gpu_raytracing_amd/csrc/rt_frames.cpp b/rust_gpu_raytracing_amd/csrc/rt_frames.cpp
--- a/rust_gpu_raytracing_amd/csrc/rt_frames.cpp
+++ b/rust_gpu_raytracing_amd/csrc/rt_frames.cpp
@@ -333,20 +333,21 @@
         const uint32_t n = env_line_texels(ka.env_uniform, ka.env_w, ka.env_h);
         if (n != 0 && n <= kEnvLineMax) line_bytes = (size_t)n * sizeof(float4);
     }
-    const rt_ctx::OccKey key{sl.lds_bytes, lane_pt, line_bytes, sl.mode, sl.tris ? 1u : 0u, ctx->force_threads,
+    const size_t image_bytes = sl.lds_bytes + (sl.mode >= 1 ? sizeof(PassConstants) : 0u);
+    const rt_ctx::OccKey key{image_bytes, lane_pt, line_bytes, sl.mode, sl.tris ? 1u : 0u, ctx->force_threads,
                              ctx->waves_cap};
     rt_ctx::OccEntry& oc = ctx->occ_cache[b.fp_instance ? 1 : 0];
     if (oc.blocks_per_cu == 0 || !same_key(oc.key, key)) {
         int per_cu = 0;
         uint32_t threads = 0;
-        hipError_t oe = rt_pathtrace_pick_config(sl.mode, sl.tris, b.fp_instance, sl.lds_bytes, lane_pt,
+        hipError_t oe = rt_pathtrace_pick_config(sl.mode, sl.tris, b.fp_instance, image_bytes, lane_pt,
                                                  ctx->force_threads, ctx->waves_cap, &threads, &per_cu);
         if (oe != hipSuccess) return hip_fail(ctx, "rt_pathtrace_pick_config (occupancy query)", oe);
         oc.env_line = false;
         if (line_bytes != 0) {
             int per_cu_line = 0;
             uint32_t threads_line = 0;
-            oe = rt_pathtrace_pick_config(sl.mode, sl.tris, b.fp_instance, sl.lds_bytes + line_bytes, lane_pt,
+            oe = rt_pathtrace_pick_config(sl.mode, sl.tris, b.fp_instance, image_bytes + line_bytes, lane_pt,
                                           ctx->force_threads, ctx->waves_cap, &threads_line, &per_cu_line);
             if (oe != hipSuccess) (void)hipGetLastError();
             oc.env_line = oe == hipSuccess && threads_line == threads && per_cu_line == per_cu;
@@ -358,7 +359,7 @@
     b.occ = &oc;
     ctx->last_threads = oc.threads;
     ctx->last_mode = sl.mode;
-    b.lds_bytes = sl.lds_bytes;
+    b.lds_bytes = image_bytes;
     if (oc.env_line) {
         ka.env_uniform |= kEnvLineStaged;
         b.lds_bytes += line_bytes;
diff --git a/rust_gpu_raytracing_amd/csrc/rt_kernel_args.h b/rust_gpu_raytracing_amd/csrc/rt_kernel_args.h
--- a/rust_gpu_raytracing_amd/csrc/rt_kernel_args.h
+++ b/rust_gpu_raytracing_amd/csrc/rt_kernel_args.h
@@ -79,7 +79,37 @@
 
 constexpr uint32_t kEnvLineMax = 512;
 constexpr uint32_t kEnvLineStaged = 4u;
-static_assert(kLdsTailBytes % 16 == 0, "the environment line after the tail is 16-byte aligned");
+
+#define RT_GLOBAL __attribute__((address_space(1)))
+struct PassConstants {
+    const RT_GLOBAL uint32_t* textures;
+    const RT_GLOBAL uint32_t* env;
+    const RT_GLOBAL RtTriangleHot* triangles;
+    const RT_GLOBAL float4* camera_rays;
+    RT_GLOBAL float4* accum;
+    RT_GLOBAL uint32_t* output;
+    RT_GLOBAL float4* frame_light;
+    RT_GLOBAL uint4* primary;
+    RT_GLOBAL uint32_t* queue;
+    const RT_GLOBAL uint32_t* tile_order;
+    RT_GLOBAL uint32_t* tile_cost;
+    RT_GLOBAL uint32_t* sched;
+    RT_GLOBAL unsigned long long* ray_counter;
+    RT_GLOBAL unsigned long long* launch_clock;
+    uint32_t texture_width, texture_height, env_map_width, env_map_height, material_count;
+    uint32_t tex_w, tex_h, tex_layers, env_w, env_h, env_uniform, bounces;
+    uint32_t lds_mat, lds_mat_aux, lds_sph_mat;
+    uint32_t light_plane, compute_per_frame, accumulation_index, accumulate, frames, gen_rays;
+    uint32_t width, height, tiles_x, owned_tiles, rank, world_size;
+    float camera_origin[3];
+    uint32_t queue_units, queue_stripes, unit_tile_major, sched_bits;
+    uint32_t sphere_always, sphere_nodes, sphere_octant_stride, sphere_boxes_ordered;
+    float sphere_extent, sphere_rmin, sphere_rmax;
+    uint32_t tri_nodes, tri_accel, tri_octant_stride;
+};
+static_assert(sizeof(PassConstants) % 16 == 0 && sizeof(PassConstants) == 288, "pass-constants block layout");
+static_assert(kLdsTailBytes % 16 == 0, "the block and the environment line after the tail are 16-byte aligned");
+constexpr size_t kEnvLineOffset = kLdsTailBytes + sizeof(PassConstants);
 __host__ __device__ inline uint32_t env_line_texels(uint32_t env_uniform, uint32_t env_w, uint32_t env_h) {
     switch (env_uniform & 3u) {
         case 3u: return 1u;
diff --git a/rust_gpu_raytracing_amd/csrc/rt_path_common.h b/rust_gpu_raytracing_amd/csrc/rt_path_common.h
--- a/rust_gpu_raytracing_amd/csrc/rt_path_common.h
+++ b/rust_gpu_raytracing_amd/csrc/rt_path_common.h
@@ -41,6 +41,27 @@
 };
 
 __device__ __forceinline__ f3 ld3(const float4& v) { return mk(v.x, v.y, v.z); }
+
+typedef const __attribute__((address_space(3))) PassConstants LdsPassConstants;
+template <class KA>
+constexpr bool kInLds = false;
+template <>
+constexpr bool kInLds<LdsPassConstants> = true;
+template <>
+constexpr bool kInLds<__attribute__((address_space(3))) PassConstants> = true;
+template <class T>
+__device__ __forceinline__ T* plain_ptr(T* p) {
+    return p;
+}
+template <class T>
+__device__ __forceinline__ T* plain_ptr(RT_GLOBAL T* p) {
+    return (T*)p;
+}
+template <class KA>
+__device__ __forceinline__ uint32_t wave_uniform(uint32_t v) {
+    if constexpr (kInLds<KA>) return __builtin_amdgcn_readfirstlane(v);
+    return v;
+}
 
 __device__ __forceinline__ int texel_coord(float c, uint32_t size) {
     if (!(c >= 0.0f)) return 0;
@@ -252,8 +273,8 @@
     }
 }
 
-template <bool kTris, bool kAlwaysUv = false>
-__device__ __forceinline__ Hit trace_end(const SceneView& sv, const KernelArgs& ka, f3 o, f3 d, const TraceState& ts) {
+template <bool kTris, bool kAlwaysUv = false, class KA>
+__device__ __forceinline__ Hit trace_end(const SceneView& sv, const KA& ka, f3 o, f3 d, const TraceState& ts) {
     Hit h;
     h.t = kF32Max;
     h.p = mk(0.f, 0.f, 0.f);
@@ -264,7 +285,7 @@
     h.v = 0.f;
     if (kTris && ts.tri.t != kF32Max) {
         const RtObject& ob = sv.obj[ts.tri.obj];
-        const f3 fn = ld3(ka.triangles[ts.tri.tri].fn);
+        const f3 fn = ld3(plain_ptr(ka.triangles)[ts.tri.tri].fn);
         h.front_face = ts.tri.front;
         h.n = ts.tri.front ? fn : -fn;
         h.t = ts.tri.t;
@@ -335,7 +356,7 @@
         y = texel_coord(v * (float)(int32_t)ka.env_map_height, ka.env_h);
     }
     if (kLine && (ka.env_uniform & kEnvLineStaged)) {
-        const float4 c = (reinterpret_cast<const float4*>(srgb) + kLdsTailBytes / sizeof(float4))[x + y];
+        const float4 c = (reinterpret_cast<const float4*>(srgb) + kEnvLineOffset / sizeof(float4))[x + y];
         return f4{c.x, c.y, c.z, c.w};
     }
     return decode_texel(ka.env[(size_t)y * ka.env_w + (size_t)x], srgb);
@@ -356,7 +377,8 @@
     return mk(r0, r1, r2);
 }
 
-__device__ __forceinline__ f3 camera_ray(const KernelArgs& ka, const float* cam, uint32_t x, uint32_t y) {
+template <class KA>
+__device__ __forceinline__ f3 camera_ray(const KA& ka, const float* cam, uint32_t x, uint32_t y) {
     const float xc = (float)x / (float)ka.width;
     const float yc = (float)y / (float)ka.height;
     const float nx = xc * 2.0f - 1.0f;
@@ -369,15 +391,15 @@
     return mat4_mul_xyz(cam + 16, ws.x, ws.y, ws.z, 0.0f, unused);
 }
 
-__device__ __forceinline__ f3 pixel_ray(const KernelArgs& ka, const float* cam, uint32_t index, uint32_t x,
-                                        uint32_t y) {
+template <class KA>
+__device__ __forceinline__ f3 pixel_ray(const KA& ka, const float* cam, uint32_t index, uint32_t x, uint32_t y) {
     if (ka.gen_rays) return camera_ray(ka, cam, x, y);
-    const float4 cr = ka.camera_rays[index];
+    const float4 cr = plain_ptr(ka.camera_rays)[index];
     return mk(cr.x, cr.y, cr.z);
 }
 
-__device__ __forceinline__ void start_sample(const KernelArgs& ka, uint32_t index, uint32_t random_index, f3 cam,
-                                             Path& p) {
+template <class KA>
+__device__ __forceinline__ void start_sample(const KA& ka, uint32_t index, uint32_t random_index, f3 cam, Path& p) {
     p.o = mk(ka.camera_origin[0], ka.camera_origin[1], ka.camera_origin[2]);
     p.d = cam;
     p.seed = index * random_index * 326624u;
diff --git a/rust_gpu_raytracing_amd/csrc/rt_walk.h b/rust_gpu_raytracing_amd/csrc/rt_walk.h
--- a/rust_gpu_raytracing_amd/csrc/rt_walk.h
+++ b/rust_gpu_raytracing_amd/csrc/rt_walk.h
@@ -10,8 +10,8 @@
 
 namespace {
 
-template <bool kTris>
-__device__ __forceinline__ void phase_setup(const SceneView& sv, const KernelArgs& ka, f3 o, float a, uint32_t phase,
+template <bool kTris, class KA>
+__device__ __forceinline__ void phase_setup(const SceneView& sv, const KA& ka, f3 o, float a, uint32_t phase,
                                             TraceState& ts) {
     const float r = sqrt_up(dot(o, o));
     float m;
@@ -38,8 +38,9 @@
     }
 }
 
-template <bool kTris>
-__device__ __forceinline__ void trace_begin(const SceneView& sv, const KernelArgs& ka, f3 o, f3 d, TraceState& ts) {
+template <bool kTris, class KA>
+__device__ __forceinline__ void trace_begin(const SceneView& sv, const KernelArgs& ka, const KA& ca, f3 o, f3 d,
+                                            TraceState& ts) {
     if constexpr (kTris) {
         ts.inv = mk(1.0f / d.x, 1.0f / d.y, 1.0f / d.z);
     } else {
@@ -54,24 +55,29 @@
     ts.node = 0;
     ts.pending = kNoLeaf;
     uint32_t i = 0;
-    for (; i + 4u <= ka.sphere_always; i += 4u) test_sphere_group<true>(sv, i, o, d, ts.a4, ts.a2, ts.sph);
-    if (ka.sphere_always - i >= 2u) {
+    const uint32_t n_always = wave_uniform<KA>(ca.sphere_always);
+    for (; i + 4u <= n_always; i += 4u) test_sphere_group<true>(sv, i, o, d, ts.a4, ts.a2, ts.sph);
+    if (n_always - i >= 2u) {
         test_sphere_group<true>(sv, i, o, d, ts.a4, ts.a2, ts.sph);
-    } else if (ka.sphere_always - i == 1u) {
+    } else if (n_always - i == 1u) {
         float b;
         const float disc = sphere_disc(sv.sph[i], o, d, ts.a4, b);
         sphere_candidate(disc, b, ts.a2, sv.orig[i], i, ts.sph);
     }
     if constexpr (!kTris) {
         ts.phase = 1;
-    } else if (!ka.tri_accel) {
+    } else if (!wave_uniform<KA>(ca.tri_accel)) {
         ts.tri = sweep_triangles(sv, ka, o, d);
         ts.phase = 1;
     } else {
-        ts.phase = ka.tri_nodes != 0 ? 0u : 1u;
-    }
-    if (ts.phase == 1 && ka.sphere_nodes == 0) ts.phase = 2;
-    phase_setup<kTris>(sv, ka, o, a, ts.phase, ts);
+        ts.phase = ca.tri_nodes != 0 ? 0u : 1u;
+    }
+    if (ts.phase == 1 && ca.sphere_nodes == 0) ts.phase = 2;
+    phase_setup<kTris>(sv, ca, o, a, ts.phase, ts);
+}
+template <bool kTris>
+__device__ __forceinline__ void trace_begin(const SceneView& sv, const KernelArgs& ka, f3 o, f3 d, TraceState& ts) {
+    trace_begin<kTris>(sv, ka, ka, o, d, ts);
 }
 
 __device__ __forceinline__ uint32_t lane_id_here() {
```

After: 27000. 0.953x the previous value.
